# zhoubin-me/supertonic

Measured on AMD Instinct MI355X. Metric: audio-sec/sec (RTF^-1), 66M model, batch=128 per GPU, higher is better.
Workload: dtype bf16

## Files before the change

### include/stn.h

```cpp
#ifndef STN_H
#define STN_H
#include <stddef.h>
#include <stdint.h>

#include "stn_arch.h"

#ifdef __cplusplus
extern "C" {
#endif

#define STN_OK 0
#define STN_ERR_INVALID (-1)
#define STN_ERR_DEVICE (-2)
#define STN_ERR_STATE (-3)
#define STN_ERR_UNSUPPORTED (-4)
#define STN_ERR_IO (-5)

#define STN_DTYPE_F32 0
#define STN_DTYPE_BF16 1
#define STN_DTYPE_F16 2

typedef struct stn_handle stn_handle;

typedef struct stn_config {
// ... 133 lines not shown
int stn_set_loudness(stn_handle* h, int on, float target_lufs, float ceiling_dbfs);
int stn_get_loudness(const stn_handle* h, int* on, float* target_lufs, float* ceiling_dbfs);
int stn_batch_loudness(stn_handle* h, float* lufs, float* peak, float* gain);
int stn_op_loudness(stn_handle* h, int hz, int rows, int W, const float* x, const int64_t* n_or_null, float* lufs, float* peak);
int stn_kweighting_filter(int hz, double* shelf_b3, double* shelf_a3, double* hp_b3, double* hp_a3);
int stn_op_loudness_ex(stn_handle* h, int hz, int rows, int W, const float* x, const int64_t* n_or_null, int on, float target_lufs,
                       float ceiling_dbfs, int x_misalign, float* st_end, float* st_start, float* pk, float* pa, float* pb, float* lufs,
                       float* peak, float* gain, char* form, size_t form_cap);
int stn_loudness_table(int hz, float* coef10, float* mpow, size_t cap, int* hop);

int stn_batch_loudness_range(stn_handle* h, float* m_max, float* s_max, float* lra, int32_t* n_st);
int stn_batch_join_loudness_range(stn_handle* h, const stn_join* j, float* m_max, float* s_max, float* lra, int32_t* n_st);
int stn_op_loudness_range(stn_handle* h, int hz, int rows, int W, const float* x, const int64_t* n_or_null, float* m_max, float* s_max,
                          float* lra, int32_t* n_st);
int stn_loudness_range_rule(int hop, int64_t nseg, const double* seg, double* m_max, double* s_max, double* lra, int32_t* n_st);

int stn_set_silence_trim(stn_handle* h, int on, float top_db, float keep_ms, float fade_ms);
int stn_get_silence_trim(const stn_handle* h, int* on, float* top_db, float* keep_ms, float* fade_ms);
int stn_batch_silence_edges(stn_handle* h, int64_t* start, int64_t* end);
int stn_op_silence_edges(stn_handle* h, int hz, int rows, int W, const float* x, const int64_t* n_or_null, float top_db, float keep_ms,
                         int64_t* start, int64_t* end);
int stn_op_silence_trim(stn_handle* h, int hz, int rows, int W, const float* x, const int64_t* n_or_null, float top_db, float keep_ms,
                        float fade_ms, const float* gain_or_null, int enc, void* y, int64_t* start, int64_t* end);
int stn_silence_fade_window(int hz, float fade_ms, float* w, int64_t cap, int64_t* n);
int stn_dbg_batch_set_wav(stn_handle* h, const float* wav);
int64_t stn_dbg_span_uploads(const stn_handle* h);

int stn_set_pause_limit(stn_handle* h, int on, float max_pause_ms);
int stn_get_pause_limit(const stn_handle* h, int* on, float* max_pause_ms);
int stn_batch_pauses(stn_handle* h, int64_t* len, int32_t* n_cuts, int64_t* cuts_or_null, int cap_pairs);
int stn_op_pause_trim(stn_handle* h, int hz, int rows, int W, const float* x, const int64_t* n_or_null, float top_db, float keep_ms,
                      float fade_ms, float max_pause_ms, const float* gain_or_null, int enc, void* y, int64_t* start, int64_t* end,
                      int64_t* len, int32_t* n_cuts, int64_t* cuts_or_null, int cap_pairs);
int stn_pause_plan(int hz, int64_t n, const double* level, int64_t K, float top_db, float keep_ms, float max_pause_ms, int64_t* start,
                   int64_t* end, int64_t* cuts, int cap_pairs, int32_t* n_cuts);
const char* stn_pause_plan_error(void);
int stn_op_silence_edges_ex(stn_handle* h, int hz, int rows, int W, const float* x, const int64_t* n_or_null, float top_db, float keep_ms,
                            float fade_ms, float max_pause_ms, int x_misalign, float* pa, float* pb, double* lev, int64_t* start,
                            int64_t* end, int64_t* len, int32_t* n_cuts, int64_t* cuts_or_null, int cap_pairs, char* form, size_t form_cap);

int stn_set_limiter(stn_handle* h, int on, float lookahead_ms);
int stn_get_limiter(const stn_handle* h, int* on, float* lookahead_ms);
int stn_batch_limiter(stn_handle* h, float* reduction_db, int64_t* limited);
int stn_op_limiter(stn_handle* h, int hz, int rows, int W, const float* x, const int64_t* n_or_null, const float* gain_or_null,
                   float ceiling_dbfs, float lookahead_ms, float* y, float* s_or_null, float* reduction_db, int64_t* limited);
int stn_limiter_window(int hz, float lookahead_ms, float* w, int64_t cap, int64_t* n);

#define STN_PEAK_SAMPLE 0
#define STN_PEAK_TRUE 1
int stn_set_peak_mode(stn_handle* h, int mode);
int stn_get_peak_mode(const stn_handle* h);
int stn_true_peak_filter(float* taps_or_null, size_t cap, int* phases, int* taps_per_phase);
int stn_batch_true_peak(stn_handle* h, float* tp_in, float* tp_out, float* trim);
int stn_op_true_peak(stn_handle* h, int hz, int rows, int W, const float* x, const int64_t* n_or_null, const float* gain_or_null,
                     int x_misalign, float* tp, float* env_or_null, float* pk_or_null, char* form, size_t form_cap);
int stn_op_limiter_ex(stn_handle* h, int hz, int rows, int W, const float* x, const int64_t* n_or_null, const float* gain_or_null,
                      float ceiling_dbfs, float lookahead_ms, float* y, float* s_or_null, float* reduction_db, int64_t* limited,
                      int peak_mode, float* env_or_null, float* trim_or_null);

#define STN_FILT_HIGHPASS 0
#define STN_FILT_LOWPASS 1
#define STN_FILT_NOTCH 2
#define STN_FILT_PEAK 3
#define STN_FILT_LOWSHELF 4
#define STN_FILT_HIGHSHELF 5
#define STN_MAX_FILTERS 8
typedef struct stn_filter { int type; float freq_hz; float q; float gain_db; } stn_filter;
int stn_set_filters(stn_handle* h, int n, const stn_filter* f);
int stn_get_filters(const stn_handle* h, int* n, stn_filter* out);
int stn_op_filter(stn_handle* h, int hz, int rows, int W, const float* x, int n, const stn_filter* f, float* y);
int stn_op_filter_ex(stn_handle* h, int hz, int rows, int W, const float* x, int n, const stn_filter* f, int x_misalign, float* y,
                     float* st_end, float* st_start, int* guard_ok, char* form, size_t form_cap);
int stn_filter_coefs(const stn_filter* f, int rate_hz, double c[5], float c32[5]);
const char* stn_filter_error(int n, const stn_filter* f, int rate_hz);
int stn_filter_response(int n, const stn_filter* f, int rate_hz, int n_freq, const double* freq_hz, double* mag_db);
int stn_dbg_filter_geometry(int* chunk, int* wg_span, int* scan_tile_chunks, int* biquads_per_section);

typedef struct stn_compressor { float threshold_db, ratio, knee_db, attack_ms, release_ms, makeup_db; } stn_compressor;
int stn_set_compressor(stn_handle* h, int on, const stn_compressor* c);
int stn_get_compressor(const stn_handle* h, int* on, stn_compressor* out);
int stn_batch_compressor(stn_handle* h, float* max_reduction_db);
int stn_op_compressor(stn_handle* h, int hz, int rows, int W, const float* x, const stn_compressor* c, float* y);
int stn_op_compressor_ex(stn_handle* h, int hz, int rows, int W, const float* x, const stn_compressor* c, int x_misalign, int in_place,
                         float* y, float* gr_db, float* s1_end, float* s1_start, float* s2_end, float* s2_start, int* guard_ok, char* form,
                         size_t form_cap);
int stn_compressor_coefs(const stn_compressor* c, int rate_hz, double k[2], float k32[2]);
int stn_compressor_curve(const stn_compressor* c, int n, const double* in_db, double* out_db);
const char* stn_compressor_error(const stn_compressor* c, int rate_hz);

#define STN_DEESS_SPLIT 0
#define STN_DEESS_WIDE 1
typedef struct stn_deesser { float freq_hz, threshold_db, ratio, knee_db, attack_ms, release_ms, range_db; int mode; } stn_deesser;
int stn_set_deesser(stn_handle* h, int on, const stn_deesser* c);
int stn_get_deesser(const stn_handle* h, int* on, stn_deesser* out);
int stn_batch_deesser(stn_handle* h, float* max_reduction_db);
int stn_op_deesser(stn_handle* h, int hz, int rows, int W, const float* x, const stn_deesser* c, float* y);
int stn_op_deesser_ex(stn_handle* h, int hz, int rows, int W, const float* x, const stn_deesser* c, int x_misalign, int in_place, float* y,
                      float* band, float* gr_db, float* st_end, float* st_start, float* s1_end, float* s1_start, float* s2_end,
                      float* s2_start, int* guard_ok, char* form, size_t form_cap);
int stn_deesser_band(const stn_deesser* c, int rate_hz, double c10[10], float c32[10]);
int stn_deesser_coefs(const stn_deesser* c, int rate_hz, double k[2], float k32[2]);
const char* stn_deesser_error(const stn_deesser* c, int rate_hz);

typedef struct stn_expander { float threshold_db, ratio, knee_db, range_db, attack_ms, hold_ms, release_ms; } stn_expander;
int stn_set_expander(stn_handle* h, int on, const stn_expander* c);
int stn_get_expander(const stn_handle* h, int* on, stn_expander* out);
int stn_batch_expander(stn_handle* h, float* min_attenuation_db, int64_t* closed_samples);
int stn_op_expander(stn_handle* h, int hz, int rows, int W, const float* x, const stn_expander* c, float* y);
int stn_op_expander_ex(stn_handle* h, int hz, int rows, int W, const float* x, const stn_expander* c, int x_misalign, int in_place, float* y,
                       float* open_db, float* s1_end, float* s1_start, float* s2_end, float* s2_start, int* guard_ok, char* form,
                       size_t form_cap);
int stn_expander_coefs(const stn_expander* c, int rate_hz, double k[3], float k32[3], int64_t* hold_samples);
int stn_expander_curve(const stn_expander* c, int n, const double* in_db, double* out_db);
const char* stn_expander_error(const stn_expander* c, int rate_hz);

int stn_profile_enable(stn_handle* h, int on);
int stn_profile_reset(stn_handle* h);
int stn_profile_filter(stn_handle* h, const char* family_or_null);
int stn_profile_sample(stn_handle* h, int every);
int stn_launch_log_enable(stn_handle* h, int on);
int64_t stn_launch_log(stn_handle* h, char* out, size_t cap);
int stn_profile_count(stn_handle* h);
int stn_profile_get(stn_handle* h, int idx, char* name, size_t name_cap, double* total_ms, int64_t* launches,
                    double* flops, double* bytes);

int stn_dbg_xattn_hs_enable(stn_handle* h, int on);
int64_t stn_dbg_xattn_hs_stamps(stn_handle* h, unsigned long long* out, size_t cap);
int stn_dbg_fold_run_frames(const int32_t* latent_lengths, int B, int n_cu);

int stn_op_gemm(stn_handle* h, int dtype, int M, int N, int K, const float* A , const float* W ,
                const float* bias_or_null, int act , float* out );
int stn_op_gemm_ex(stn_handle* h, int dtype, int M, int N, int K, const float* A , const float* W , int mode, int act,
                   int out_dtype, int ldo, const float* bias_or_null, const float* gamma_or_null, const int32_t* len_or_null, int L,
                   const int32_t* row_b_or_null, const float* rowvec_or_null, int nseq, int nt, int tr, float* out, int64_t out_elems,
                   char* form, size_t form_cap);
int stn_dbg_gemm_form(int dtype, int M, int N, int K, int mode, int out_dtype, int ldo, int masked, int tr, char* out, size_t cap);
int stn_dbg_ffn_form(int dtype, int stage, int C, int I, int64_t M, int64_t gate_rows, int packed, int k, int max_dil, int mask,
                     int64_t min_rows, int64_t split_min_rows, int nt_hints, char* out, size_t cap);
int stn_op_gemm_bench(stn_handle* h, int dtype, int M, int N, int K, int mode, int iters, double* avg_ms);
int stn_op_gemm_phases(stn_handle* h, int dtype, int M, int N, int K, int mode, double* out6);
int stn_op_dwconv_ln(stn_handle* h, int dtype, int B, int L, int C, int k, int dil, const float* x,
                     const float* w , const float* bias, const float* ln_g, const float* ln_b, float* y);
int stn_op_dwconv_ln_ragged(stn_handle* h, int dtype, int B, int L, int C, int k, int dil, const float* x,
                            const float* w , const float* bias, const float* ln_g, const float* ln_b,
                            const int32_t* seqlen , float* y);
int stn_op_gemm_rows(stn_handle* h, int dtype, int M, int N, int K, const float* A, const float* W, const float* bias_or_null, int B,
                     const int32_t* rows, const int32_t* valid, int T, float* out, int64_t out_elems, char* form, size_t form_cap);
int stn_op_dwconv_ln_ex(stn_handle* h, int dtype, int B, int L, int C, int k, int dil, const float* x, int64_t x_rows,
                        const float* w_or_null , const float* bias_or_null, const float* ln_g, const float* ln_b,
                        const int32_t* seqlen_or_null, int packed, int ln_only, float* y, int64_t y_rows, char* form, size_t form_cap);
int stn_op_dwconv_ln_tail(stn_handle* h, int dtype, int B, int L, int C, int k, int dil, const float* x, int64_t x_rows,
                          const float* w , const float* bias, const float* ln_g, const float* ln_b, const int32_t* seqlen,
                          const float* tail , int T, int rf, float* y, int64_t y_rows, char* form, size_t form_cap);
int64_t stn_dbg_len_tables(int B, const int32_t* llen, int ve_rows, int with_pairs, int vo_form, int ccf, int T, int rf, int32_t* layout,
                           int32_t* out, int64_t out_n);
int stn_dbg_dwconv_ln_form(int dtype, int B, int L, int C, int k, int packed, char* out, size_t cap);
int stn_op_fold_ln(stn_handle* h, int dtype, int M, int C, int S, const float* part, const float* b2, const float* gamma,
                   const float* rowvec_or_null, const int32_t* row_b_or_null, int nseq, const float* ln_g, const float* ln_b, float* x,
                   float* y);
int stn_op_layout(stn_handle* h, int which, int dtype, const int32_t* p, int n_p, const float* a, int64_t a_n, const float* b, int64_t b_n,
                  const float* c, int64_t c_n, const int64_t* ids, int64_t ids_n, const int32_t* len, int packed, float* out, int64_t out_n,
                  float* out2, int64_t out2_n, int32_t* iout, int64_t iout_n);
int stn_op_attention(stn_handle* h, int dtype, int B, int Lq, int Lk, int H, int dh, const float* q, const float* k,
                     const float* v, const int32_t* qlen_or_null, const int32_t* klen_or_null, int rope_mode, float* o);
int stn_op_attention_ex(stn_handle* h, int dtype, int B, int Lq, int Lk, int H, int dh, const float* q, int64_t q_elems, int ldq,
                        int q_col, float* kv, int64_t kv_elems, int ldk, int k_col, int v_col, float* o, int64_t o_elems, int ldo,
                        const int32_t* qlen_or_null, const int32_t* klen_or_null, const int32_t* q_off_or_null,
                        const int32_t* k_off_or_null, int rope_mode, int k_rotated, int rot_groups, int rot_stride, int rot_col,
                        char* form, size_t form_cap);
int stn_op_xattn_hs(stn_handle* h, int dtype, int M, const float* xn, const float* Wq, const float* bq_or_null, const float* Wo,
                    const float* kv, int64_t kv_elems, int ldk, int k_col, int B, int L, int Lk, const int32_t* qlen,
                    const int32_t* klen_or_null, const int32_t* k_off_or_null, int rope_mode, int pairs_mode, int64_t part_stride,
                    float* part, int64_t part_elems, int32_t* pairs_out_or_null, char* form, size_t form_cap);
int stn_dbg_attn_form(int kind, int dtype, int B, int Lq, int Lk, int H, int dh, int ldq, int ldk, int misaligned, char* out, size_t cap);
int stn_op_ffn(stn_handle* h, int M, int C, int I, const float* xn , const float* W1, const float* b1, const float* W2,
               const float* b2_or_null, const float* gamma_or_null, const float* rowvec_or_null ,
               const int32_t* row_b_or_null , int nseq, float* x, int fused);
int stn_op_ffn_ex(stn_handle* h, int dtype, int M, int C, int I, const float* xn, int ldx, int64_t xn_elems, const float* W1, const float* b1,
                  const float* W2, const float* b2_or_null, const float* gamma_or_null, const int32_t* len_or_null, int L,
                  const int32_t* row_b_or_null, const float* rowvec_or_null, int rv_ld, int nseq, int mode, int split, float* x, int ldo,
                  int64_t x_elems, float* part_or_null, int64_t part_stride, int64_t part_elems, char* form, size_t form_cap);
int stn_op_ffn_bench(stn_handle* h, int M, int C, int I, int fused, int iters, double* out5);
int stn_op_fold_dwconv_ln(stn_handle* h, int B, int C, int k, int dil, int S, const int32_t* seqlen, const float* x, const float* part,
                          const float* b2_or_null, const float* gamma_or_null, const float* rowvec_or_null , const float* w ,
                          const float* bias, const float* ln_g, const float* ln_b, float* x_out, float* y);
int stn_op_fold_dwconv_ln_ex(stn_handle* h, int dtype, int B, int L, int C, int k, int dil, int S, int run_frames, const int32_t* seqlen,
                             const float* x_in, int64_t x_rows, const float* part, int64_t part_stride, int64_t part_elems,
                             const float* b2_or_null, const float* gamma_or_null, const float* rowvec_or_null, int rv_ld,
                             const float* w , const float* bias, const float* ln_g, const float* ln_b, float* x_out, int64_t x_out_rows,
                             float* y, int64_t y_rows, char* form, size_t form_cap);
int stn_dbg_fold_dwconv_ln_form(int dtype, int B, int L, int C, int k, int dil, int S, int has_rowvec, int run_frames, char* out, size_t cap);
int stn_op_block_bench(stn_handle* h, int B, int L, int C, int I, int k, int dil, int mode, int iters, double* out6);
int stn_op_randn(stn_handle* h, uint64_t seed, int B, int D, int L, const int64_t* utt_ids_or_null,
                 const int32_t* len_or_null, float* out);

const char* stn_version(void);
int stn_hip_versions(int* built, int* runtime);
int stn_device_count(void);
int stn_device_sync(int device);
int stn_ffn_fused_forms(int dtype, int C, int I);

#ifdef __cplusplus
}
#endif
#endif
```

### supertonic_amd/binding.py

```python
import ctypes
import os

import numpy as np

from .arch import StnArch

_HERE = os.path.dirname(os.path.abspath(__file__))
LIB_PATH = os.environ.get("STN_LIB") or os.path.join(_HERE, "libstn.so")
_LIB = None

F32, BF16, F16 = 0, 1, 2
_DTYPES = {"f32": F32, "fp32": F32, "float32": F32, "bf16": BF16, "f16": F16, "fp16": F16, "float16": F16, "half": F16,
           F32: F32, BF16: BF16, F16: F16}
ACT_NONE, ACT_GELU, ACT_SILU, ACT_GELU_TANH = 0, 1, 2, 3
EPI_STORE, EPI_RESID, EPI_STORE_T = 0, 1, 2
FFN_VOCODER, FFN_ESTIMATOR, FFN_TEXT = 1, 2, 4
LAYOUT_ROW_MAP, LAYOUT_NCL_TO_ROWS, LAYOUT_EULER_NCL, LAYOUT_UNPACK_ROWS, LAYOUT_EMBED, LAYOUT_MASKED_MEAN, LAYOUT_IM2COL, LAYOUT_VOCODER_IN = range(8)
LAYOUT_FILL_ROWS, LAYOUT_HS_PAIRS, LAYOUT_TRIM_LEN = 8, 9, 10
ENC_F32, ENC_PCM16, ENC_PCM24, ENC_MULAW, ENC_ALAW = 0, 1, 2, 3, 4
ENCODINGS = {"f32": ENC_F32, "pcm16": ENC_PCM16, "pcm24": ENC_PCM24, "mulaw": ENC_MULAW, "alaw": ENC_ALAW}
ENCODING_NAMES = {v: k for k, v in ENCODINGS.items()}
ENCODING_BYTES = {ENC_F32: 4, ENC_PCM16: 2, ENC_PCM24: 3, ENC_MULAW: 1, ENC_ALAW: 1}
ZERO_CODEWORD = {ENC_F32: 0, ENC_PCM16: 0, ENC_PCM24: 0, ENC_MULAW: 0xFF, ENC_ALAW: 0xD5}

# ... 367 lines not shown

class StnError(RuntimeError):
    def __init__(self, code, msg):
        super().__init__(f"stn error {code}: {msg}")
        self.code = code


class StnConfig(ctypes.Structure):
    _fields_ = [("device", ctypes.c_int32), ("dtype", ctypes.c_int32)]


_f32p = np.ctypeslib.ndpointer(np.float32, flags="C_CONTIGUOUS")
_i64p = np.ctypeslib.ndpointer(np.int64, flags="C_CONTIGUOUS")
_i32p = np.ctypeslib.ndpointer(np.int32, flags="C_CONTIGUOUS")


def runtime_info(L=None):
    import sys
    L = L or load()
    b, r = ctypes.c_int(), ctypes.c_int()
    L.stn_hip_versions(ctypes.byref(b), ctypes.byref(r))
    return {"hip_built": b.value, "hip_runtime": r.value, "torch_preloaded": "torch" in sys.modules, "lib": LIB_PATH}


def device_count():
    n = load().stn_device_count()
    if n < 0:
        raise StnError(n, "hipGetDeviceCount failed")
    return n


def device_sync(device=0):
    rc = load().stn_device_sync(int(device))
    if rc < 0:
        raise StnError(rc, "hipDeviceSynchronize failed")


def _check_runtime(L):
    import warnings
    info = runtime_info(L)
    b, r = info["hip_built"], info["hip_runtime"]
    if r > 0 and (b // 100000) != (r // 100000):
        warnings.warn(f"libstn.so was built against HIP {b // 10000000}.{b // 100000 % 100} but runs on HIP runtime {r // 10000000}.{r // 100000 % 100}"
                      + (" (PyTorch's bundled runtime was loaded first; set STN_NO_TORCH_PRELOAD=1 in processes that do not need torch)" if info["torch_preloaded"] else ""),
                      RuntimeWarning, stacklevel=3)


def load():
    global _LIB
    if _LIB is not None:
        return _LIB
    if not os.path.exists(LIB_PATH):
        raise FileNotFoundError(f"{LIB_PATH} not found: build it with `make` (hipcc --offload-arch=gfx950); "
                                "the engine has no fallback path")
    import sys
    if "torch" not in sys.modules and os.environ.get("STN_NO_TORCH_PRELOAD") != "1" and os.environ.get("STN_HOST_ONLY") != "1":
        import importlib.util
        if importlib.util.find_spec("torch") is not None:
            import torch
    L = ctypes.CDLL(LIB_PATH)
    if os.environ.get("STN_HOST_ONLY") == "1":
        _LIB = L
        return L
    vp, ci, cu64, cf = ctypes.c_void_p, ctypes.c_int, ctypes.c_uint64, ctypes.c_float
    L.stn_hip_versions.argtypes = [ctypes.POINTER(ci), ctypes.POINTER(ci)]
    L.stn_ffn_fused_forms.argtypes = [ci, ci, ci]
    L.stn_device_count.argtypes = []
    L.stn_device_sync.argtypes = [ci]
    _check_runtime(L)
    L.stn_version.restype = ctypes.c_char_p
    L.stn_create.argtypes = [ctypes.POINTER(StnConfig), ctypes.POINTER(vp)]
    L.stn_destroy.argtypes = [vp]
    L.stn_last_error.restype = ctypes.c_char_p
    L.stn_last_error.argtypes = [vp]
    L.stn_load_dir.argtypes = [vp, ctypes.c_char_p]
    L.stn_tensor_names.argtypes = [vp, ctypes.POINTER(StnArch), ctypes.c_char_p, ctypes.c_size_t]
    L.stn_load_synthetic.argtypes = [vp, ctypes.POINTER(StnArch), cu64]
    L.stn_get_arch.argtypes = [vp, ctypes.POINTER(StnArch)]
    L.stn_param_count.restype = ctypes.c_int64
    L.stn_param_count.argtypes = [vp]
    L.stn_duration.argtypes = [vp, ci, ci, _i64p, _f32p, _f32p, _f32p]
    L.stn_text_enc.argtypes = [vp, ci, ci, _i64p, _f32p, _f32p, _f32p]
    L.stn_vector_est.argtypes = [vp, ci, ci, ci] + [_f32p] * 8
    L.stn_vocoder.argtypes = [vp, ci, ci, _f32p, _f32p]
    L.stn_batch_upload.argtypes = [vp, ci, ci, _i64p, _f32p, _f32p, _f32p, vp, vp]
    L.stn_batch_set_noise.argtypes = [vp, _f32p, ci]
    L.stn_batch_run.argtypes = [vp, ci, cf, cu64]
    L.stn_set_graph_mode.argtypes = [vp, ci]
    L.stn_set_vocoder_mode.argtypes = [vp, ci]
    L.stn_set_row_layout.argtypes = [vp, ci]
    L.stn_set_fused_xattn.argtypes = [vp, ci]
    L.stn_set_shape_buckets.argtypes = [vp, ci]
    L.stn_set_duration_read.argtypes = [vp, ci]
    L.stn_set_gelu_form.argtypes = [vp, ci]
    L.stn_get_gelu_form.argtypes = [vp]
    L.stn_batch_ve_rows.argtypes = [vp]
    L.stn_batch_ve_rows.restype = ctypes.c_int64
    L.stn_batch_vo_rows.argtypes = [vp]
    L.stn_batch_vo_rows.restype = ctypes.c_int64
    L.stn_graph_replays.restype = ctypes.c_int64
    L.stn_graph_replays.argtypes = [vp]
    L.stn_graphs_cached.restype = ctypes.c_int64
    L.stn_graphs_cached.argtypes = [vp]
    L.stn_batch_dims.argtypes = [vp, ctypes.POINTER(ci), ctypes.POINTER(ci), ctypes.POINTER(ctypes.c_int64)]
    L.stn_batch_fetch.argtypes = [vp, vp, ctypes.c_size_t, vp]
    L.stn_batch_fetch_latent.argtypes = [vp, _f32p]
    L.stn_batch_fetch_pcm16.argtypes = [vp, vp, ctypes.c_size_t, vp]
    L.stn_batch_fetch_pcm16_begin.argtypes = [vp, ci]
    L.stn_batch_fetch_slot_dims.argtypes = [vp, ci, ctypes.POINTER(ci), ctypes.POINTER(ctypes.c_int64)]
    L.stn_batch_fetch_pcm16_end.argtypes = [vp, ci, ctypes.POINTER(vp), ctypes.POINTER(ctypes.c_size_t), vp]
    L.stn_host_alloc_pinned.restype = vp
    L.stn_host_alloc_pinned.argtypes = [ctypes.c_size_t]
    L.stn_host_free_pinned.argtypes = [vp]
    L.stn_batch_wav_device_ptr.argtypes = [vp, ctypes.POINTER(vp)]
    L.stn_sync.argtypes = [vp]
    L.stn_set_stream.argtypes = [vp, vp]
    L.stn_batch_copy_wav_device.argtypes = [vp, vp, ctypes.c_int64]
    L.stn_batch_copy_pcm16_device.argtypes = [vp, vp, ctypes.c_int64]
    L.stn_profile_filter.argtypes = [vp, ctypes.c_char_p]
    L.stn_profile_sample.argtypes = [vp, ci]
    L.stn_launch_log_enable.argtypes = [vp, ci]
    L.stn_dbg_xattn_hs_enable.argtypes = [vp, ci]
    L.stn_dbg_xattn_hs_stamps.argtypes = [vp, vp, ctypes.c_size_t]
    L.stn_dbg_xattn_hs_stamps.restype = ctypes.c_int64
    L.stn_dbg_fold_run_frames.argtypes = [vp, ctypes.c_int, ctypes.c_int]
    L.stn_dbg_fold_run_frames.restype = ctypes.c_int
    L.stn_dbg_gemm_form.argtypes = [ci, ci, ci, ci, ci, ci, ci, ci, ci, ctypes.c_char_p, ctypes.c_size_t]
    L.stn_dbg_gemm_form.restype = ctypes.c_int
    L.stn_dbg_attn_form.argtypes = [ci, ci, ci, ci, ci, ci, ci, ci, ci, ci, ctypes.c_char_p, ctypes.c_size_t]
    L.stn_dbg_attn_form.restype = ctypes.c_int
    L.stn_dbg_ffn_form.argtypes = [ci, ci, ci, ci, ctypes.c_int64, ctypes.c_int64, ci, ci, ci, ci, ctypes.c_int64, ctypes.c_int64, ci,
                                   ctypes.c_char_p, ctypes.c_size_t]
    L.stn_dbg_ffn_form.restype = ctypes.c_int
    L.stn_launch_log.argtypes = [vp, ctypes.c_char_p, ctypes.c_size_t]
    L.stn_launch_log.restype = ctypes.c_int64
    L.stn_profile_enable.argtypes = [vp, ci]
    L.stn_profile_reset.argtypes = [vp]
    L.stn_profile_count.argtypes = [vp]
    L.stn_profile_get.argtypes = [vp, ci, ctypes.c_char_p, ctypes.c_size_t, ctypes.POINTER(ctypes.c_double),
                                  ctypes.POINTER(ctypes.c_int64), ctypes.POINTER(ctypes.c_double),
                                  ctypes.POINTER(ctypes.c_double)]
    L.stn_op_gemm.argtypes = [vp, ci, ci, ci, ci, _f32p, _f32p, vp, ci, _f32p]
    L.stn_op_gemm_ex.argtypes = [vp, ci, ci, ci, ci, _f32p, _f32p, ci, ci, ci, ci, vp, vp, vp, ci, vp, vp, ci, ci, ci, _f32p,
                                 ctypes.c_int64, ctypes.c_char_p, ctypes.c_size_t]
    L.stn_op_gemm_bench.argtypes = [vp, ci, ci, ci, ci, ci, ci, ctypes.POINTER(ctypes.c_double)]
    L.stn_op_gemm_phases.argtypes = [vp, ci, ci, ci, ci, ci, ctypes.POINTER(ctypes.c_double)]
    L.stn_op_dwconv_ln.argtypes = [vp, ci, ci, ci, ci, ci, ci, _f32p, _f32p, _f32p, _f32p, _f32p, _f32p]
    L.stn_op_dwconv_ln_ragged.argtypes = [vp, ci, ci, ci, ci, ci, ci, _f32p, _f32p, _f32p, _f32p, _f32p, _i32p, _f32p]
    L.stn_op_attention.argtypes = [vp, ci, ci, ci, ci, ci, ci, _f32p, _f32p, _f32p, vp, vp, ci, _f32p]
    L.stn_op_gemm_rows.argtypes = [vp, ci, ci, ci, ci, _f32p, _f32p, vp, ci, _i32p, _i32p, ci, _f32p, ctypes.c_int64, ctypes.c_char_p, ctypes.c_size_t]
    L.stn_op_dwconv_ln_ex.argtypes = [vp, ci, ci, ci, ci, ci, ci, _f32p, ctypes.c_int64, vp, vp, _f32p, _f32p, vp, ci, ci, _f32p, ctypes.c_int64,
                                      ctypes.c_char_p, ctypes.c_size_t]
    L.stn_op_dwconv_ln_tail.argtypes = [vp, ci, ci, ci, ci, ci, ci, _f32p, ctypes.c_int64, _f32p, _f32p, _f32p, _f32p, _i32p, _f32p, ci, ci, _f32p,
                                        ctypes.c_int64, ctypes.c_char_p, ctypes.c_size_t]
    L.stn_dbg_resample_form.argtypes = [ci, ci, ctypes.c_int64, ctypes.c_char_p, ctypes.c_size_t]
    L.stn_dbg_resample_form.restype = ctypes.c_int
    L.stn_dbg_dwconv_ln_form.argtypes = [ci, ci, ci, ci, ci, ci, ctypes.c_char_p, ctypes.c_size_t]
    L.stn_dbg_dwconv_ln_form.restype = ctypes.c_int
    L.stn_dbg_len_tables.argtypes = [ci, _i32p, ci, ci, ci, ci, ci, ci, _i32p, ctypes.c_void_p, ctypes.c_int64]
    L.stn_dbg_len_tables.restype = ctypes.c_int64
    L.stn_op_fold_ln.argtypes = [vp, ci, ci, ci, ci, _f32p, _f32p, _f32p, vp, vp, ci, _f32p, _f32p, _f32p, _f32p]
    L.stn_op_layout.argtypes = [vp, ci, ci, _i32p, ci, vp, ctypes.c_int64, vp, ctypes.c_int64, vp, ctypes.c_int64, vp, ctypes.c_int64, vp, ci,
                                vp, ctypes.c_int64, vp, ctypes.c_int64, vp, ctypes.c_int64]
    L.stn_op_attention_ex.argtypes = [vp, ci, ci, ci, ci, ci, ci, _f32p, ctypes.c_int64, ci, ci, _f32p, ctypes.c_int64, ci, ci, ci,
                                      _f32p, ctypes.c_int64, ci, vp, vp, vp, vp, ci, ci, ci, ci, ci, ctypes.c_char_p, ctypes.c_size_t]
    L.stn_op_xattn_hs.argtypes = [vp, ci, ci, _f32p, _f32p, vp, _f32p, _f32p, ctypes.c_int64, ci, ci, ci, ci, ci, _i32p, vp, vp, ci, ci,
                                  ctypes.c_int64, _f32p, ctypes.c_int64, vp, ctypes.c_char_p, ctypes.c_size_t]
    L.stn_op_randn.argtypes = [vp, cu64, ci, ci, ci, vp, vp, _f32p]
    L.stn_op_ffn.argtypes = [vp, ci, ci, ci, _f32p, _f32p, _f32p, _f32p, vp, vp, vp, vp, ci, _f32p, ci]
    L.stn_op_ffn_ex.argtypes = [vp, ci, ci, ci, ci, _f32p, ci, ctypes.c_int64, _f32p, _f32p, _f32p, vp, vp, vp, ci, vp, vp, ci, ci, ci, ci, _f32p, ci,
                                ctypes.c_int64, vp, ctypes.c_int64, ctypes.c_int64, ctypes.c_char_p, ctypes.c_size_t]
    L.stn_op_ffn_bench.argtypes = [vp, ci, ci, ci, ci, ci, ctypes.POINTER(ctypes.c_double)]
    L.stn_set_fused_ffn.argtypes = [vp, ci]
    L.stn_set_fused_ffn_min_rows.argtypes = [vp, ctypes.c_int64, ctypes.c_int64]
    L.stn_op_fold_dwconv_ln.argtypes = [vp, ci, ci, ci, ci, ci, _i32p, _f32p, _f32p, vp, vp, vp, _f32p, _f32p, _f32p, _f32p, _f32p, _f32p]
    L.stn_op_fold_dwconv_ln_ex.argtypes = [vp, ci, ci, ci, ci, ci, ci, ci, ci, _i32p, _f32p, ctypes.c_int64, _f32p, ctypes.c_int64, ctypes.c_int64, vp, vp,
                                           vp, ci, _f32p, _f32p, _f32p, _f32p, _f32p, ctypes.c_int64, _f32p, ctypes.c_int64, ctypes.c_char_p,
                                           ctypes.c_size_t]
    L.stn_dbg_fold_dwconv_ln_form.argtypes = [ci, ci, ci, ci, ci, ci, ci, ci, ci, ctypes.c_char_p, ctypes.c_size_t]
    L.stn_dbg_fold_dwconv_ln_form.restype = ctypes.c_int
    L.stn_op_block_bench.argtypes = [vp, ci, ci, ci, ci, ci, ci, ci, ci, ctypes.POINTER(ctypes.c_double)]
    L.stn_group_create.argtypes = [ci, vp, ci, ctypes.POINTER(vp)]
    L.stn_group_destroy.argtypes = [vp]
    L.stn_group_last_error.restype = ctypes.c_char_p
    L.stn_group_last_error.argtypes = [vp]
    L.stn_group_size.argtypes = [vp]
    L.stn_group_uses_rccl.argtypes = [vp]
    L.stn_group_handle.restype = vp
    L.stn_group_handle.argtypes = [vp, ci]
    L.stn_group_load_synthetic.argtypes = [vp, ctypes.POINTER(StnArch), cu64]
    L.stn_group_load_dir.argtypes = [vp, ctypes.c_char_p]
    L.stn_group_deal.argtypes = [ci, _i32p, ci, _i32p, _i32p]
    L.stn_group_synthesize.argtypes = [vp, ci, ci, _i64p, _f32p, _f32p, _f32p, ci, cf, vp, cu64, ctypes.POINTER(ctypes.c_int64)]
    L.stn_group_fetch_pcm16.argtypes = [vp, vp, ctypes.c_size_t, vp]
    L.stn_set_output_rate.argtypes = [vp, ci]
    L.stn_get_output_rate.argtypes = [vp]
    L.stn_resample_filter.argtypes = [ci, ci, vp, ctypes.c_size_t, ctypes.POINTER(ci), ctypes.POINTER(ci)]
    L.stn_resample_error.argtypes = [ci, ci]
    L.stn_resample_error.restype = ctypes.c_char_p
    L.stn_op_resample.argtypes = [vp, ci, ci, ci, ci, _f32p, vp, vp]
    L.stn_group_set_output_rate.argtypes = [vp, ci]
    _f64p = np.ctypeslib.ndpointer(np.float64, flags="C_CONTIGUOUS")
    L.stn_set_loudness.argtypes = [vp, ci, cf, cf]
    L.stn_get_loudness.argtypes = [vp, ctypes.POINTER(ci), ctypes.POINTER(cf), ctypes.POINTER(cf)]
    L.stn_batch_loudness.argtypes = [vp, vp, vp, vp]
    L.stn_op_loudness.argtypes = [vp, ci, ci, ci, _f32p, vp, vp, vp]
    L.stn_kweighting_filter.argtypes = [ci, _f64p, _f64p, _f64p, _f64p]
    L.stn_op_loudness_ex.argtypes = [vp, ci, ci, ci, _f32p, vp, ci, cf, cf, ci, vp, vp, vp, vp, vp, vp, vp, vp, ctypes.c_char_p, ctypes.c_size_t]
    L.stn_loudness_table.argtypes = [ci, vp, vp, ctypes.c_size_t, ctypes.POINTER(ci)]
    L.stn_group_set_loudness.argtypes = [vp, ci, cf, cf]
    L.stn_batch_loudness_range.argtypes = [vp, vp, vp, vp, vp]
    L.stn_op_loudness_range.argtypes = [vp, ci, ci, ci, _f32p, vp, vp, vp, vp, vp]
    L.stn_set_silence_trim.argtypes = [vp, ci, cf, cf, cf]
    L.stn_get_silence_trim.argtypes = [vp, ctypes.POINTER(ci), ctypes.POINTER(cf), ctypes.POINTER(cf), ctypes.POINTER(cf)]
    L.stn_batch_silence_edges.argtypes = [vp, vp, vp]
    L.stn_op_silence_edges.argtypes = [vp, ci, ci, ci, _f32p, vp, cf, cf, vp, vp]
    L.stn_op_silence_trim.argtypes = [vp, ci, ci, ci, _f32p, vp, cf, cf, cf, vp, ci, vp, vp, vp]
    L.stn_silence_fade_window.argtypes = [ci, cf, vp, ctypes.c_int64, ctypes.POINTER(ctypes.c_int64)]
    L.stn_set_pause_limit.argtypes = [vp, ci, cf]
    L.stn_get_pause_limit.argtypes = [vp, ctypes.POINTER(ci), ctypes.POINTER(cf)]
    L.stn_batch_pauses.argtypes = [vp, vp, vp, vp, ci]
    L.stn_op_pause_trim.argtypes = [vp, ci, ci, ci, _f32p, vp, cf, cf, cf, cf, vp, ci, vp, vp, vp, vp, vp, vp, ci]
    L.stn_op_silence_edges_ex.argtypes = [vp, ci, ci, ci, _f32p, vp, cf, cf, cf, cf, ci, vp, vp, vp, vp, vp, vp, vp, vp, ci, ctypes.c_char_p,
                                          ctypes.c_size_t]
    L.stn_group_set_pause_limit.argtypes = [vp, ci, cf]
    L.stn_set_limiter.argtypes = [vp, ci, cf]
    L.stn_get_limiter.argtypes = [vp, ctypes.POINTER(ci), ctypes.POINTER(cf)]
    L.stn_batch_limiter.argtypes = [vp, vp, vp]
    L.stn_op_limiter.argtypes = [vp, ci, ci, ci, _f32p, vp, vp, cf, cf, vp, vp, vp, vp]
    L.stn_limiter_window.argtypes = [ci, cf, vp, ctypes.c_int64, ctypes.POINTER(ctypes.c_int64)]
    L.stn_group_set_limiter.argtypes = [vp, ci, cf]
    L.stn_set_peak_mode.argtypes = [vp, ci]
    L.stn_get_peak_mode.argtypes = [vp]
    L.stn_group_set_peak_mode.argtypes = [vp, ci]
    L.stn_true_peak_filter.argtypes = [vp, ctypes.c_size_t, ctypes.POINTER(ci), ctypes.POINTER(ci)]
    L.stn_batch_true_peak.argtypes = [vp, vp, vp, vp]
    L.stn_op_true_peak.argtypes = [vp, ci, ci, ci, _f32p, vp, vp, ci, vp, vp, vp, ctypes.c_char_p, ctypes.c_size_t]
    L.stn_op_limiter_ex.argtypes = [vp, ci, ci, ci, _f32p, vp, vp, cf, cf, vp, vp, vp, vp, ci, vp, vp]
    fp = ctypes.POINTER(StnFilter)
    L.stn_set_filters.argtypes = [vp, ci, fp]
    L.stn_get_filters.argtypes = [vp, ctypes.POINTER(ci), fp]
    L.stn_group_set_filters.argtypes = [vp, ci, fp]
    L.stn_op_filter.argtypes = [vp, ci, ci, ci, _f32p, ci, fp, _f32p]
    L.stn_op_filter_ex.argtypes = [vp, ci, ci, ci, _f32p, ci, fp, ci, _f32p, vp, vp, ctypes.POINTER(ci), ctypes.c_char_p, ctypes.c_size_t]
    L.stn_filter_error.argtypes = [ci, fp, ci]
    L.stn_filter_error.restype = ctypes.c_char_p
    L.stn_filter_coefs.argtypes = [fp, ci, _f64p, _f32p]
    L.stn_filter_response.argtypes = [ci, fp, ci, ci, _f64p, _f64p]
    L.stn_dbg_filter_geometry.argtypes = [ctypes.POINTER(ci)] * 4
    cpp = ctypes.POINTER(StnCompressor)
    L.stn_set_compressor.argtypes = [vp, ci, cpp]
    L.stn_get_compressor.argtypes = [vp, ctypes.POINTER(ci), cpp]
    L.stn_group_set_compressor.argtypes = [vp, ci, cpp]
    L.stn_batch_compressor.argtypes = [vp, vp]
    L.stn_op_compressor.argtypes = [vp, ci, ci, ci, _f32p, cpp, _f32p]
    L.stn_op_compressor_ex.argtypes = [vp, ci, ci, ci, _f32p, cpp, ci, ci, _f32p, vp, vp, vp, vp, vp, ctypes.POINTER(ci), ctypes.c_char_p, ctypes.c_size_t]
    L.stn_compressor_error.argtypes = [cpp, ci]
    L.stn_compressor_error.restype = ctypes.c_char_p
    L.stn_compressor_coefs.argtypes = [cpp, ci, _f64p, _f32p]
    L.stn_compressor_curve.argtypes = [cpp, ci, _f64p, _f64p]
    xpp = ctypes.POINTER(StnExpander)
    L.stn_set_expander.argtypes = [vp, ci, xpp]
    L.stn_get_expander.argtypes = [vp, ctypes.POINTER(ci), xpp]
    L.stn_group_set_expander.argtypes = [vp, ci, xpp]
    L.stn_batch_expander.argtypes = [vp, vp, vp]
    L.stn_op_expander.argtypes = [vp, ci, ci, ci, _f32p, xpp, _f32p]
    L.stn_op_expander_ex.argtypes = [vp, ci, ci, ci, _f32p, xpp, ci, ci, _f32p, vp, vp, vp, vp, vp, ctypes.POINTER(ci), ctypes.c_char_p, ctypes.c_size_t]
    L.stn_expander_error.argtypes = [xpp, ci]
    L.stn_expander_error.restype = ctypes.c_char_p
    L.stn_expander_coefs.argtypes = [xpp, ci, _f64p, _f32p, ctypes.POINTER(ctypes.c_int64)]
    L.stn_expander_curve.argtypes = [xpp, ci, _f64p, _f64p]
    dsp = ctypes.POINTER(StnDeesser)
    L.stn_set_deesser.argtypes = [vp, ci, dsp]
    L.stn_get_deesser.argtypes = [vp, ctypes.POINTER(ci), dsp]
    L.stn_group_set_deesser.argtypes = [vp, ci, dsp]
    L.stn_batch_deesser.argtypes = [vp, vp]
    L.stn_op_deesser.argtypes = [vp, ci, ci, ci, _f32p, dsp, _f32p]
    L.stn_op_deesser_ex.argtypes = [vp, ci, ci, ci, _f32p, dsp, ci, ci, _f32p] + [vp] * 8 + [ctypes.POINTER(ci), ctypes.c_char_p, ctypes.c_size_t]
    L.stn_deesser_error.argtypes = [dsp, ci]
    L.stn_deesser_error.restype = ctypes.c_char_p
    L.stn_deesser_band.argtypes = [dsp, ci, _f64p, _f32p]
    L.stn_deesser_coefs.argtypes = [dsp, ci, _f64p, _f32p]
    L.stn_dbg_batch_set_wav.argtypes = [vp, _f32p]
    L.stn_dbg_span_uploads.argtypes = [vp]
    L.stn_dbg_span_uploads.restype = ctypes.c_int64
    L.stn_encoding_bytes.argtypes = [ci]
    L.stn_batch_fetch_encoded.argtypes = [vp, ci, vp, ctypes.c_size_t, vp]
    L.stn_batch_copy_encoded_device.argtypes = [vp, ci, vp, ctypes.c_int64]
    L.stn_batch_fetch_encoded_begin.argtypes = [vp, ci, ci]
    L.stn_batch_fetch_encoded_end.argtypes = [vp, ci, ctypes.POINTER(vp), ctypes.POINTER(ctypes.c_size_t), vp]
    L.stn_op_encode.argtypes = [vp, ci, ci, ci, _f32p, vp]
    L.stn_set_dither.argtypes = [vp, ci, cu64]
    L.stn_get_dither.argtypes = [vp, ctypes.POINTER(cu64)]
    L.stn_group_set_dither.argtypes = [vp, ci, cu64]
    L.stn_op_encode_ex.argtypes = [vp, ci, ci, ci, _f32p, ci, vp, vp, ci, cu64, ctypes.c_int64, vp]
    L.stn_set_pitch.argtypes = [vp, cf]
    L.stn_get_pitch.argtypes = [vp, ctypes.POINTER(cf), ctypes.POINTER(ci), ctypes.POINTER(ci)]
    L.stn_group_set_pitch.argtypes = [vp, cf]
    L.stn_op_time_stretch.argtypes = [vp, ci, ci, ci, _f32p, vp, ci, ci, vp, vp, vp]
    L.stn_op_pitch.argtypes = [vp, ci, ci, ci, _f32p, vp, cf, vp]
    L.stn_set_pitch_mode.argtypes = [vp, ci]
    L.stn_get_pitch_mode.argtypes = [vp]
    L.stn_group_set_pitch_mode.argtypes = [vp, ci]
    L.stn_op_formant.argtypes = [vp, ci, ci, ci, _f32p, _f32p, vp, vp]
    L.stn_op_formant_ex.argtypes = [vp, ci, ci, ci, _f32p, _f32p, vp, vp, vp, vp, vp, vp, vp, ctypes.POINTER(ci)]
    L.stn_op_pitch_ex.argtypes = [vp, ci, ci, ci, _f32p, vp, cf, ci, vp]
# ... 1384 lines not shown
        return res, form.value.decode()

    def op_gemm_bench(self, M, N, K, mode=0, iters=20, dtype=None):
        ms = ctypes.c_double()
        self._ck(self._lib.stn_op_gemm_bench(self._h, self.dtype if dtype is None else _DTYPES[dtype], M, N, K, mode,
                                             iters, ctypes.byref(ms)))
        return ms.value

    def op_ffn(self, xn, W1, b1, W2, b2, gamma, x, rowvec=None, row_b=None, fused=True):
        M, C = xn.shape
        I = W1.shape[0]
        out = np.array(x, dtype=np.float32, order="C", copy=True)
        _, b2p = _opt(b2, np.float32)
        b2a = _opt(b2, np.float32)[0]
        ga, gp = _opt(gamma, np.float32)
        rva, rvp = _opt(rowvec, np.float32)
        rba, rbp = _opt(row_b, np.int32)
        b2p = b2a.ctypes.data if b2a is not None else None
        self._ck(self._lib.stn_op_ffn(self._h, M, C, I, _c(xn, np.float32), _c(W1, np.float32), _c(b1, np.float32), _c(W2, np.float32),
                                      b2p, gp, rvp, rbp, 0 if rva is None else rva.shape[0], out, int(fused)))
        return out

    def op_ffn_ex(self, xn, W1, b1, W2, x, mode=1, b2=None, gamma=None, len=None, L=None, row_b=None, rowvec=None, split=0, part=None,
                  part_stride=0, M=None, dtype=None):
        xn = _c(xn, np.float32)
        I, C = W1.shape
        M = xn.shape[0] if M is None else int(M)
        x_r = np.array(x, dtype=np.float32, order="C", copy=True)
        p_r = None if part is None else np.array(part, dtype=np.float32, order="C", copy=True)
        nseq = 0
        for v in (len, rowvec):
            if v is not None:
                nseq = max(nseq, np.asarray(v).shape[0])
        if row_b is not None and rowvec is None:
            nseq = max(nseq, int(np.max(row_b)) + 1)
        _b, bp = _opt(b2, np.float32)
        _g, gp = _opt(gamma, np.float32)
        _l, lp = _opt(len, np.int32)
        _r, rp = _opt(row_b, np.int32)
        _v, vp_ = _opt(rowvec, np.float32)
        form = ctypes.create_string_buffer(32)
        self._ck(self._lib.stn_op_ffn_ex(self._h, self.dtype if dtype is None else _DTYPES[dtype], M, C, I, xn.reshape(-1), xn.shape[1], xn.size,
                                         _c(W1, np.float32), _c(b1, np.float32), _c(W2, np.float32), bp, gp, lp, int(M if L is None else L), rp, vp_,
                                         C if _v is None else _v.shape[1], nseq, int(mode), int(split), x_r.reshape(-1), x_r.shape[1], x_r.size,
                                         None if p_r is None else p_r.ctypes.data, int(part_stride), 0 if p_r is None else p_r.size, form,
                                         ctypes.sizeof(form)))
        return x_r, p_r, form.value.decode()

    def op_ffn_bench(self, M, C, I, fused=True, iters=20):
        out = (ctypes.c_double * 5)()
        self._ck(self._lib.stn_op_ffn_bench(self._h, M, C, I, int(fused), iters, out))
        return dict(ms=out[0], first_stage=out[1], tile_loop=out[2], epilogue=out[3], workgroups=int(out[4]))

    def op_fold_dwconv_ln(self, seqlen, x, part, b2, gamma, rowvec, w, bias, g, b, k, dil):
        seqlen = np.ascontiguousarray(seqlen, np.int32)
        S, M, C = part.shape
        xo = np.empty((M, C), np.float32)
        y = np.empty((M, C), np.float32)
        b2a, _ = _opt(b2, np.float32)
        ga, _ = _opt(gamma, np.float32)
        rva, _ = _opt(rowvec, np.float32)
        p = lambda a: None if a is None else a.ctypes.data
        self._ck(self._lib.stn_op_fold_dwconv_ln(self._h, len(seqlen), C, k, dil, S, seqlen, _c(x, np.float32), _c(part, np.float32), p(b2a), p(ga), p(rva),
                                                 _c(w, np.float32), _c(bias, np.float32), _c(g, np.float32), _c(b, np.float32), xo, y))
        return xo, y

    def op_fold_dwconv_ln_ex(self, seqlen, L, x_in, part, part_stride, S, b2, gamma, rowvec, w, bias, g, b, dil, x_out, y, run_frames=0, dtype=None):
        seqlen = _c(seqlen, np.int32)
        x_in = _c(x_in, np.float32)
        part = _c(part, np.float32).reshape(-1)
        xo = np.array(x_out, dtype=np.float32, order="C", copy=True)
        yo = np.array(y, dtype=np.float32, order="C", copy=True)
        C = x_in.shape[1]
        w = _c(w, np.float32)
        _b2, b2p = _opt(b2, np.float32)
        _g, gp = _opt(gamma, np.float32)
        _v, vp_ = _opt(rowvec, np.float32)
        form = ctypes.create_string_buffer(96)
        self._ck(self._lib.stn_op_fold_dwconv_ln_ex(self._h, self.dtype if dtype is None else _DTYPES[dtype], len(seqlen), int(L), C, w.shape[1], int(dil),
                                                    int(S), int(run_frames), seqlen, x_in.reshape(-1), x_in.shape[0], part, int(part_stride), part.size,
                                                    b2p, gp, vp_, C if _v is None else _v.shape[1], w, _c(bias, np.float32), _c(g, np.float32),
                                                    _c(b, np.float32), xo.reshape(-1), xo.shape[0], yo.reshape(-1), yo.shape[0], form, ctypes.sizeof(form)))
        return xo, yo, form.value.decode()

    def op_block_bench(self, B, L, C, I, k, dil, mode, iters=20):
        out = (ctypes.c_double * 6)()
        self._ck(self._lib.stn_op_block_bench(self._h, B, L, C, I, k, dil, mode, iters, out))
        return dict(ms=out[0], conv_ms=out[1], fold_phase1=out[2], fold_barrier=out[3], fold_phase2=out[4], fold_span=out[5])

    def set_fused_ffn_min_rows(self, k4_rows=-1, split_rows=-1):
        self._ck(self._lib.stn_set_fused_ffn_min_rows(self._h, int(k4_rows), int(split_rows)))

    def op_gemm_phases(self, M, N, K, mode=0, dtype=None):
        out = (ctypes.c_double * 6)()
        self._ck(self._lib.stn_op_gemm_phases(self._h, self.dtype if dtype is None else _DTYPES[dtype], M, N, K, mode, out))
        return dict(first_stage=out[0], k_loop=out[1], epilogue=out[2], grid_span=out[3], entry_spread=out[4], workgroups=int(out[5]))

    def op_dwconv_ln(self, x, w, bias, g, b, dil, dtype=None, seqlen=None):
        B, L, C = x.shape
        k = w.shape[1]
        y = np.empty((B, L, C), np.float32)
        if seqlen is not None:
            self._ck(self._lib.stn_op_dwconv_ln_ragged(self._h, self.dtype if dtype is None else _DTYPES[dtype], B, L, C, k,
                                                       dil, _c(x, np.float32), _c(w, np.float32), _c(bias, np.float32),
                                                       _c(g, np.float32), _c(b, np.float32), _c(seqlen, np.int32), y))
            return y
        self._ck(self._lib.stn_op_dwconv_ln(self._h, self.dtype if dtype is None else _DTYPES[dtype], B, L, C, k, dil,
                                            _c(x, np.float32), _c(w, np.float32), _c(bias, np.float32),
                                            _c(g, np.float32), _c(b, np.float32), y))
        return y

    def op_gemm_rows(self, A, W, out, rows, valid, T, bias=None, dtype=None):
        A = _c(A, np.float32)
        W = _c(W, np.float32)
        rows = _c(rows, np.int32)
        valid = _c(valid, np.int32)
        o_r = np.array(out, dtype=np.float32, order="C", copy=True)
        _b, bp = _opt(bias, np.float32)
        form = ctypes.create_string_buffer(96)
        self._ck(self._lib.stn_op_gemm_rows(self._h, self.dtype if dtype is None else _DTYPES[dtype], A.shape[0], W.shape[0], A.shape[1],
                                            A.reshape(-1), W.reshape(-1), bp, len(rows), rows, valid, int(T), o_r.reshape(-1), o_r.size, form,
                                            ctypes.sizeof(form)))
        return o_r, form.value.decode()

    def op_dwconv_ln_ex(self, x, w, bias, g, b, dil, out, B, L, seqlen=None, packed=False, ln_only=False, dtype=None):
        x = _c(x, np.float32)
        o_r = np.array(out, dtype=np.float32, order="C", copy=True)
        C = x.shape[1]
        _w, wp = _opt(w, np.float32)
        _b, bp = _opt(bias, np.float32)
        _l, lp = _opt(seqlen, np.int32)
        form = ctypes.create_string_buffer(32)
        self._ck(self._lib.stn_op_dwconv_ln_ex(self._h, self.dtype if dtype is None else _DTYPES[dtype], int(B), int(L), C,
                                               1 if _w is None else _w.shape[1], int(dil), x.reshape(-1), x.shape[0], wp, bp, _c(g, np.float32),
                                               _c(b, np.float32), lp, int(bool(packed)), int(bool(ln_only)), o_r.reshape(-1), o_r.shape[0], form,
                                               ctypes.sizeof(form)))
        return o_r, form.value.decode()

    def op_dwconv_ln_tail(self, x, w, bias, g, b, dil, out, L, seqlen, tail, T, dtype=None):
        x = _c(x, np.float32)
        tail = _c(tail, np.float32)
        o_r = np.array(out, dtype=np.float32, order="C", copy=True)
        C = x.shape[1]
        w = _c(w, np.float32)
        seqlen = _c(seqlen, np.int32)
        assert tail.ndim == 2 and tail.shape[1] == C and tail.shape[0] >= 1
        form = ctypes.create_string_buffer(32)
        self._ck(self._lib.stn_op_dwconv_ln_tail(self._h, self.dtype if dtype is None else _DTYPES[dtype], len(seqlen), int(L), C, w.shape[1],
                                                 int(dil), x.reshape(-1), x.shape[0], w, _c(bias, np.float32), _c(g, np.float32),
                                                 _c(b, np.float32), seqlen, tail.reshape(-1), int(T), tail.shape[0] - 1, o_r.reshape(-1),
                                                 o_r.shape[0], form, ctypes.sizeof(form)))
        return o_r, form.value.decode()

    def op_fold_ln(self, x, part, b2, gamma, g, b, rowvec=None, row_b=None, dtype=None):
        x_r = np.array(x, dtype=np.float32, order="C", copy=True)
        M, C = x_r.shape
        part = _c(part, np.float32)
        y = np.empty((M, C), np.float32)
        _v, vp_ = _opt(rowvec, np.float32)
        _r, rp = _opt(row_b, np.int32)
        self._ck(self._lib.stn_op_fold_ln(self._h, self.dtype if dtype is None else _DTYPES[dtype], M, C, part.shape[0], part.reshape(-1),
                                          _c(b2, np.float32), _c(gamma, np.float32), vp_, rp, 0 if _v is None else _v.shape[0],
                                          _c(g, np.float32), _c(b, np.float32), x_r, y))
        return x_r, y

    def op_layout(self, which, p, a=None, b=None, c=None, ids=None, length=None, packed=False, out=None, out2=None, iout=None, dtype="f32"):
        def f32(v):
            return (None, None, 0) if v is None else (lambda arr: (arr, arr.ctypes.data, arr.size))(_c(v, np.float32))
        pa = _c(p, np.int32)
        _a, ap, an = f32(a)
        _b, bp, bn = f32(b)
        _cc, cp, cn = f32(c)
        _i, ip = _opt(ids, np.int64)
        _l, lp = _opt(length, np.int32)
        o1 = None if out is None else np.array(out, dtype=np.float32, order="C", copy=True)
        o2 = None if out2 is None else np.array(out2, dtype=np.float32, order="C", copy=True)
        io = None if iout is None else np.array(iout, dtype=np.int32, order="C", copy=True)
        ptr = lambda v: (None, 0) if v is None else (v.ctypes.data, v.size)
        self._ck(self._lib.stn_op_layout(self._h, int(which), _DTYPES[dtype], pa, len(pa), ap, an, bp, bn, cp, cn, ip, 0 if _i is None else _i.size,
                                         lp, int(bool(packed)), *ptr(o1), *ptr(o2), *ptr(io)))
        return o1, o2, io

    def op_attention(self, q, k, v, H, qlen=None, klen=None, rope_mode=-1, dtype=None):
        B, Lq, C = q.shape
        Lk = k.shape[1]
        o = np.empty((B, Lq, C), np.float32)
        _q, qp = _opt(qlen, np.int32)
        _k, kp = _opt(klen, np.int32)
        self._ck(self._lib.stn_op_attention(self._h, self.dtype if dtype is None else _DTYPES[dtype], B, Lq, Lk, H,
                                            C // H, _c(q, np.float32), _c(k, np.float32), _c(v, np.float32), qp, kp,
                                            rope_mode, o))
        return o

    def op_attention_ex(self, q, kv, out, B, Lq, Lk, H, dh, q_col=0, k_col=0, v_col=None, qlen=None, klen=None, q_off=None, k_off=None,
                        rope_mode=-1, k_rotated=False, rot_groups=1, rot_stride=0, rot_col=None, dtype=None):
        q = _c(q, np.float32)
        kv_r = np.array(kv, dtype=np.float32, order="C", copy=True)
        o_r = np.array(out, dtype=np.float32, order="C", copy=True)
        _a, qlp = _opt(qlen, np.int32)
        _b, klp = _opt(klen, np.int32)
        _d, qop = _opt(q_off, np.int32)
        _e, kop = _opt(k_off, np.int32)
        form = ctypes.create_string_buffer(64)
        self._ck(self._lib.stn_op_attention_ex(self._h, self.dtype if dtype is None else _DTYPES[dtype], int(B), int(Lq), int(Lk), int(H), int(dh),
                                               q.reshape(-1), q.size, q.shape[1], int(q_col), kv_r.reshape(-1), kv_r.size, kv_r.shape[1],
                                               int(k_col), int(k_col + H * dh if v_col is None else v_col), o_r.reshape(-1), o_r.size,
                                               o_r.shape[1], qlp, klp, qop, kop, int(rope_mode), int(bool(k_rotated)), int(rot_groups),
                                               int(rot_stride), int(k_col if rot_col is None else rot_col), form, ctypes.sizeof(form)))
        return o_r, kv_r, form.value.decode()

    def op_xattn_hs(self, xn, Wq, bq, Wo, kv, part, part_stride, B, L, Lk, qlen, k_col=0, klen=None, k_off=None, rope_mode=-1,
                    pairs=False, dtype=None):
        xn = _c(xn, np.float32)
        kv = _c(kv, np.float32)
        part_r = np.array(part, dtype=np.float32, order="C", copy=True).reshape(-1)
        _b, bqp = _opt(bq, np.float32)
        _k, klp = _opt(klen, np.int32)
        _o, kop = _opt(k_off, np.int32)
        pr = np.full(2 * ((B + 1) // 2), -7, np.int32) if pairs else None
        form = ctypes.create_string_buffer(64)
        self._ck(self._lib.stn_op_xattn_hs(self._h, self.dtype if dtype is None else _DTYPES[dtype], xn.shape[0], xn.reshape(-1),
                                           _c(Wq, np.float32), bqp, _c(Wo, np.float32), kv.reshape(-1), kv.size, kv.shape[1], int(k_col),
                                           int(B), int(L), int(Lk), _c(qlen, np.int32), klp, kop, int(rope_mode), int(bool(pairs)),
                                           int(part_stride), part_r, part_r.size, None if pr is None else pr.ctypes.data, form,
                                           ctypes.sizeof(form)))
        return part_r, pr, form.value.decode()

    def op_randn(self, seed, B, D, L, utt_ids=None, length=None):
        out = np.empty((B, D, L), np.float32)
        _u, up = _opt(utt_ids, np.int64)
        _l, lp = _opt(length, np.int32)
        self._ck(self._lib.stn_op_randn(self._h, seed, B, D, L, up, lp, out))
        return out


def pinned_array(shape, dtype):
    L = load()
    dt = np.dtype(dtype)
    n = int(np.prod(shape)) * dt.itemsize
    p = L.stn_host_alloc_pinned(n)
    if not p:
        raise MemoryError("stn_host_alloc_pinned failed")
    buf = (ctypes.c_char * n).from_address(p)
    arr = np.frombuffer(buf, dtype=dt).reshape(shape)
    import weakref
    weakref.finalize(buf, L.stn_host_free_pinned, ctypes.c_void_p(p))
    return arr
```

### supertonic_amd/csrc/api.cpp

```cpp
#include "../../include/stn.h"

#include <algorithm>
#include <complex>
#include <cstdio>
#include <cstring>
#include <fstream>
#include <string>

#include "engine.hpp"
#include "host/json_min.hpp"
#include "host/graph_bind.hpp"
#include "host/onnx_reader.hpp"

#include <map>
#include <sstream>

struct stn_handle {
    stn::Engine* eng = nullptr;
    std::string err;
    std::vector<std::pair<std::string, stn::KernelStat>> prof;
};

static thread_local std::string g_create_err;

// ... 799 lines not shown
}
int stn_batch_loudness_range(stn_handle* h, float* m_max, float* s_max, float* lra, int32_t* n_st) {
    STN_TRY(h, { need_batch(h); h->eng->batch_loudness_range(m_max, s_max, lra, n_st); })
}
int stn_batch_join_loudness_range(stn_handle* h, const stn_join* j, float* m_max, float* s_max, float* lra, int32_t* n_st) {
    STN_TRY(h, { need(j != nullptr, "join is null"); need_batch(h); h->eng->batch_join_loudness_range(j, m_max, s_max, lra, n_st); })
}
int stn_op_loudness_range(stn_handle* h, int hz, int rows, int W, const float* x, const int64_t* n, float* m_max, float* s_max, float* lra,
                          int32_t* n_st) {
    STN_TRY(h, { need(rows > 0 && rows <= 65535 && W > 0 && x, "stn_op_loudness_range: bad argument (1 <= rows <= 65535, W >= 1, x)");
                 h->eng->op_loudness_range(hz, rows, W, x, n, m_max, s_max, lra, n_st); })
}
int stn_op_join(stn_handle* h, int hz, int rows, int W, const float* x, const int64_t* n, const stn_join* j, int enc, int loudness_on, float target_lufs,
                float ceiling_dbfs, void* y, float* prog_lufs, float* prog_peak, float* prog_gain) {
    STN_TRY(h, { need(rows > 0 && rows <= 65535 && W > 0 && x && n && j && y, "stn_op_join: bad argument (1 <= rows <= 65535, W >= 1, x, n, j and y)");
                 h->eng->op_join(hz, rows, W, x, n, j, enc, loudness_on != 0, target_lufs, ceiling_dbfs, y, prog_lufs, prog_peak, prog_gain); })
}
int stn_batch_copy_wav_device(stn_handle* h, void* dst, int64_t stride) {
    STN_TRY(h, { need(dst != nullptr, "dst is null"); h->eng->batch_copy_wav_device(static_cast<float*>(dst), stride); })
}

int stn_profile_enable(stn_handle* h, int on) { STN_TRY(h, { h->eng->profile_enable(on != 0); }) }
int stn_launch_log_enable(stn_handle* h, int on) { STN_TRY(h, { h->eng->launch_log_enable(on != 0); }) }
int64_t stn_launch_log(stn_handle* h, char* out, size_t cap) {
    if (!h) return STN_ERR_INVALID;
    try {
        const std::string s = h->eng->launch_log();
        if (out && cap > s.size()) std::memcpy(out, s.c_str(), s.size() + 1);
        return (int64_t)s.size();
    } catch (const std::exception& e) { h->err = e.what(); return STN_ERR_STATE; }
}
int stn_dbg_xattn_hs_enable(stn_handle* h, int on) { STN_TRY(h, { h->eng->hs_stamps_enable(on != 0); }) }
int stn_dbg_fold_run_frames(const int32_t* latent_lengths, int B, int n_cu) {
    if (!latent_lengths || B < 1 || n_cu < 1) return STN_ERR_INVALID;
    return stn::fold_run_frames(latent_lengths, B, n_cu);
}
int64_t stn_dbg_xattn_hs_stamps(stn_handle* h, unsigned long long* out, size_t cap) {
    if (!h) return STN_ERR_INVALID;
    try { return h->eng->hs_stamps_fetch(out, cap); } catch (const std::exception& e) { h->err = e.what(); return STN_ERR_STATE; }
}
int stn_profile_sample(stn_handle* h, int every) { STN_TRY(h, { h->eng->profile_sample(every); }) }
int stn_profile_filter(stn_handle* h, const char* fam) { STN_TRY(h, { h->eng->profile_filter(fam ? fam : ""); }) }
int stn_profile_reset(stn_handle* h) { STN_TRY(h, { h->eng->profile_reset(); h->prof.clear(); }) }
int stn_profile_count(stn_handle* h) {
    if (!h) return STN_ERR_INVALID;
    try { h->prof = h->eng->profile_collect(); } catch (const std::exception& e) { h->err = e.what(); return STN_ERR_DEVICE; }
    return (int)h->prof.size();
}
int stn_profile_get(stn_handle* h, int idx, char* name, size_t cap, double* ms, int64_t* launches, double* flops, double* bytes) {
    if (!h || idx < 0 || idx >= (int)h->prof.size()) return STN_ERR_INVALID;
    const auto& p = h->prof[idx];
    if (name && cap) { std::snprintf(name, cap, "%s", p.first.c_str()); }
    if (ms) *ms = p.second.ms;
    if (launches) *launches = p.second.launches;
    if (flops) *flops = p.second.flops;
    if (bytes) *bytes = p.second.bytes;
    return STN_OK;
}

int stn_op_gemm(stn_handle* h, int dtype, int M, int N, int K, const float* A, const float* W, const float* bias, int act, float* out) {
    STN_TRY(h, { need(M > 0 && N > 0 && K > 0 && A && W && out, "stn_op_gemm: bad argument");
                 need(K % (dtype != STN_DTYPE_F32 ? 8 : 4) == 0, "stn_op_gemm: K must be a multiple of 8 (bf16) / 4 (f32)");
                 h->eng->op_gemm(dtype, M, N, K, A, W, bias, act, out); })
}
int stn_op_gemm_ex(stn_handle* h, int dtype, int M, int N, int K, const float* A, const float* W, int mode, int act, int out_dtype, int ldo,
                   const float* bias, const float* gamma, const int32_t* len, int L, const int32_t* row_b, const float* rowvec, int nseq, int nt,
                   int tr, float* out, int64_t out_elems, char* form, size_t form_cap) {
    STN_TRY(h, { need(M > 0 && N > 0 && K > 0 && A && W && out && L >= 1, "stn_op_gemm_ex: bad argument");
                 need(dtype == STN_DTYPE_F32 || dtype == STN_DTYPE_BF16 || dtype == STN_DTYPE_F16, "stn_op_gemm_ex: unknown dtype");
                 need(K % (dtype != STN_DTYPE_F32 ? 8 : 4) == 0, "stn_op_gemm_ex: K must be a multiple of 8 (16-bit) / 4 (f32)");
                 need(mode == stn::EPI_STORE || mode == stn::EPI_RESID || mode == stn::EPI_STORE_T, "stn_op_gemm_ex: mode must be 0, 1 or 2");
                 need(act >= stn::ACT_NONE && act <= stn::ACT_GELU_TANH, "stn_op_gemm_ex: unknown activation");
                 need(out_dtype == STN_DTYPE_F32 || (mode == stn::EPI_STORE && out_dtype == dtype), "stn_op_gemm_ex: out_dtype must be f32 or the engine's dtype (store only)");
                 need(nt == 0 || nt == 1, "stn_op_gemm_ex: nt must be 0 or 1");
                 need(tr >= -1 && tr <= 1, "stn_op_gemm_ex: tr must be -1, 0 or 1");
                 need(!(len && row_b), "stn_op_gemm_ex: len and row_b exclude each other");
                 const int64_t seqs = ((int64_t)M + L - 1) / L;
                 if (mode == stn::EPI_STORE_T) {
                     need(!row_b && nseq >= seqs && out_elems >= seqs * N * L, "stn_op_gemm_ex: mode 2 needs nseq >= ceil(M/L), out_elems >= ceil(M/L)*N*L, no row_b");
                 } else {
                     need(ldo >= N && out_elems >= (int64_t)M * ldo, "stn_op_gemm_ex: needs ldo >= N and out_elems >= M*ldo");
                 }
                 if (len || (rowvec && !row_b)) need(nseq >= seqs, "stn_op_gemm_ex: len / rowvec by m / L need nseq >= ceil(M/L)");
                 if (rowvec || len || row_b) need(nseq > 0, "stn_op_gemm_ex: nseq must be > 0");
                 if (len) for (int b = 0; b < nseq; ++b) need(len[b] >= 0 && len[b] <= L, "stn_op_gemm_ex: len out of [0, L]");
                 if (row_b) for (int m = 0; m < M; ++m) need(row_b[m] >= 0 && row_b[m] < nseq, "stn_op_gemm_ex: row_b out of [0, nseq)");
                 const std::string f = h->eng->op_gemm_ex(dtype, M, N, K, A, W, mode, act, out_dtype, ldo, bias, gamma, len, L, row_b, rowvec,
                                                          nseq, nt, tr, out, out_elems);
                 if (form && form_cap) std::snprintf(form, form_cap, "%s", f.c_str()); })
}
int stn_dbg_gemm_form(int dtype, int M, int N, int K, int mode, int out_dtype, int ldo, int masked, int tr, char* out, size_t cap) {
    if (M < 1 || N < 1 || K < 1 || (dtype != STN_DTYPE_F32 && dtype != STN_DTYPE_BF16 && dtype != STN_DTYPE_F16) || tr < -1 || tr > 1)
        return STN_ERR_INVALID;
    static const int dummy_len[4] = {};
    stn::Epilogue e;
    e.mode = mode; e.out_dtype = out_dtype; e.ldo = ldo; e.len = masked ? dummy_len : nullptr; e.tr_force = tr;
    std::string f;
    try { f = stn::gemm_form(dtype, M, N, K, K, K, e, nullptr, nullptr).str(); } catch (const std::exception&) { return STN_ERR_INVALID; }
    if (out && cap > f.size()) std::memcpy(out, f.c_str(), f.size() + 1);
    return (int)f.size();
}
int stn_dbg_ffn_form(int dtype, int stage, int C, int I, int64_t M, int64_t gate_rows, int packed, int k, int max_dil, int mask,
                     int64_t min_rows, int64_t split_min_rows, int nt_hints, char* out, size_t cap) {
    if (C < 1 || I < 1 || M < 1 || k < 1 || max_dil < 1 || (stage != stn::FFN_VOCODER && stage != stn::FFN_ESTIMATOR && stage != stn::FFN_TEXT) ||
        (dtype != STN_DTYPE_F32 && dtype != STN_DTYPE_BF16 && dtype != STN_DTYPE_F16))
        return STN_ERR_INVALID;
    const std::string f = stn::ffn_form(dtype, stage, C, I, M, gate_rows, packed != 0, k, max_dil, mask, min_rows, split_min_rows, nt_hints != 0).str();
    if (out && cap > f.size()) std::memcpy(out, f.c_str(), f.size() + 1);
    return (int)f.size();
}
int stn_op_gemm_bench(stn_handle* h, int dtype, int M, int N, int K, int mode, int iters, double* avg_ms) {
    STN_TRY(h, { need(M > 0 && N > 0 && K > 0 && iters > 0 && avg_ms, "stn_op_gemm_bench: bad argument");
                 need(K % (dtype != STN_DTYPE_F32 ? 8 : 4) == 0, "K must be a multiple of 8 (bf16) / 4 (f32)");
                 *avg_ms = h->eng->op_gemm_bench(dtype, M, N, K, mode, iters); })
}
int stn_op_gemm_phases(stn_handle* h, int dtype, int M, int N, int K, int mode, double* out6) {
    STN_TRY(h, { need(M > 0 && N > 0 && K > 0 && out6, "stn_op_gemm_phases: bad argument");
                 need(K % (dtype != STN_DTYPE_F32 ? 8 : 4) == 0, "K must be a multiple of 8 (bf16) / 4 (f32)");
                 h->eng->op_gemm_phases(dtype, M, N, K, mode, out6); })
}
int stn_op_dwconv_ln(stn_handle* h, int dtype, int B, int L, int C, int k, int dil, const float* x, const float* w,
                     const float* bias, const float* g, const float* b, float* y) {
    STN_TRY(h, { need(B > 0 && L > 0 && C > 0 && C % 4 == 0 && C <= 1024 && k > 0 && (k & 1) && dil > 0 && x && w && bias && g && b && y,
                      "stn_op_dwconv_ln: bad argument");
                 h->eng->op_dwconv_ln(dtype, B, L, C, k, dil, x, w, bias, g, b, y); })
}
int stn_op_dwconv_ln_ragged(stn_handle* h, int dtype, int B, int L, int C, int k, int dil, const float* x, const float* w,
                            const float* bias, const float* g, const float* b, const int32_t* seqlen, float* y) {
    STN_TRY(h, { need(B > 0 && L > 0 && C > 0 && C % 4 == 0 && C <= 1024 && k > 0 && (k & 1) && dil > 0 && x && w && bias && g && b && y && seqlen,
                      "stn_op_dwconv_ln_ragged: bad argument");
                 for (int i = 0; i < B; ++i) need(seqlen[i] >= 0 && seqlen[i] <= L, "stn_op_dwconv_ln_ragged: seqlen out of [0, L]");
                 h->eng->op_dwconv_ln(dtype, B, L, C, k, dil, x, w, bias, g, b, y, seqlen); })
}
static void gemm_rows_checked(stn_handle* h, int dtype, int M, int N, int K, const float* A, const float* W, const float* bias, int B,
                              const int32_t* rows, const int32_t* valid, int T, float* out, int64_t out_elems, char* form, size_t form_cap) {
    need(M > 0 && N > 0 && K > 0 && A && W && out && rows && valid && B > 0 && B <= 1024 && T > 0, "stn_op_gemm_rows: bad argument");
    need(dtype == STN_DTYPE_F32 || dtype == STN_DTYPE_BF16 || dtype == STN_DTYPE_F16, "stn_op_gemm_rows: unknown dtype");
    need(K % (dtype != STN_DTYPE_F32 ? 8 : 4) == 0, "stn_op_gemm_rows: K must be a multiple of 8 (16-bit) / 4 (f32)");
    int64_t tot = 0;
    for (int b = 0; b < B; ++b) {
        need(rows[b] >= 0 && rows[b] <= T && valid[b] >= 0 && valid[b] <= rows[b], "stn_op_gemm_rows: needs 0 <= valid[b] <= rows[b] <= T");
        tot += rows[b];
    }
    need(tot <= M && out_elems >= (int64_t)B * T * N, "stn_op_gemm_rows: needs sum rows <= M and out_elems >= B*T*N");
    const std::string f = h->eng->op_gemm_rows(dtype, M, N, K, A, W, bias, B, rows, valid, T, out, out_elems);
    if (form && form_cap) std::snprintf(form, form_cap, "%s", f.c_str());
}
int stn_op_gemm_rows(stn_handle* h, int dtype, int M, int N, int K, const float* A, const float* W, const float* bias, int B, const int32_t* rows,
                     const int32_t* valid, int T, float* out, int64_t out_elems, char* form, size_t form_cap) {
    STN_TRY(h, gemm_rows_checked(h, dtype, M, N, K, A, W, bias, B, rows, valid, T, out, out_elems, form, form_cap))
}
static void dwconv_ln_ex_checked(stn_handle* h, int dtype, int B, int L, int C, int k, int dil, const float* x, int64_t x_rows, const float* w,
                                 const float* bias, const float* g, const float* b, const int32_t* seqlen, int packed, int ln_only, float* y,
                                 int64_t y_rows, char* form, size_t form_cap) {
    need(B > 0 && L > 0 && C > 0 && C % 4 == 0 && C <= 1024 && k > 0 && (k & 1) && dil > 0 && x && g && b && y && x_rows > 0 && y_rows > 0,
         "stn_op_dwconv_ln_ex: bad argument");
    need(dtype == STN_DTYPE_F32 || dtype == STN_DTYPE_BF16 || dtype == STN_DTYPE_F16, "stn_op_dwconv_ln_ex: unknown dtype");
    need(ln_only || (w && bias), "stn_op_dwconv_ln_ex: the conv needs w and bias");
    need(!(packed && ln_only), "stn_op_dwconv_ln_ex: ln_only takes no packed layout");
    need(!packed || (seqlen && B <= 1024), "stn_op_dwconv_ln_ex: packed rows need seqlen and B <= 1024");
    int64_t rows = (int64_t)B * L;
    if (seqlen && !ln_only) {
        int64_t tot = 0;
        for (int i = 0; i < B; ++i) { need(seqlen[i] >= 0 && seqlen[i] <= L, "stn_op_dwconv_ln_ex: seqlen out of [0, L]"); tot += seqlen[i]; }
        if (packed) rows = tot;
    }
    need(x_rows >= rows && y_rows >= rows, "stn_op_dwconv_ln_ex: x / y hold fewer rows than the launch addresses");
    const std::string f = h->eng->op_dwconv_ln_ex(dtype, B, L, C, k, dil, x, x_rows, w, bias, g, b, ln_only ? nullptr : seqlen, packed, ln_only, y, y_rows);
    if (form && form_cap) std::snprintf(form, form_cap, "%s", f.c_str());
}
int stn_op_dwconv_ln_ex(stn_handle* h, int dtype, int B, int L, int C, int k, int dil, const float* x, int64_t x_rows, const float* w,
                        const float* bias, const float* g, const float* b, const int32_t* seqlen, int packed, int ln_only, float* y,
                        int64_t y_rows, char* form, size_t form_cap) {
    STN_TRY(h, dwconv_ln_ex_checked(h, dtype, B, L, C, k, dil, x, x_rows, w, bias, g, b, seqlen, packed, ln_only, y, y_rows, form, form_cap))
}
static void dwconv_ln_tail_checked(stn_handle* h, int dtype, int B, int L, int C, int k, int dil, const float* x, int64_t x_rows, const float* w,
                                   const float* bias, const float* g, const float* b, const int32_t* seqlen, const float* tail, int T, int rf,
                                   float* y, int64_t y_rows, char* form, size_t form_cap) {
    need(B > 0 && B <= 1024 && L > 0 && C > 0 && C % 4 == 0 && C <= 512 && (k == 5 || k == 7) && dil > 0 && x && w && bias && g && b && y && seqlen &&
             x_rows > 0 && y_rows > 0,
         "stn_op_dwconv_ln_tail: bad argument");
    need(dtype == STN_DTYPE_F32 || dtype == STN_DTYPE_BF16 || dtype == STN_DTYPE_F16, "stn_op_dwconv_ln_tail: unknown dtype");
    need(tail && rf >= 0 && T >= L, "stn_op_dwconv_ln_tail: needs a tail table of rf + 1 >= 1 rows and T >= L");
    int64_t rows = 0;
    for (int i = 0; i < B; ++i) { need(seqlen[i] >= 0 && seqlen[i] <= L, "stn_op_dwconv_ln_tail: seqlen out of [0, L]"); rows += seqlen[i]; }
    need(x_rows >= rows && y_rows >= rows, "stn_op_dwconv_ln_tail: x / y hold fewer rows than the launch addresses");
    const std::string f = h->eng->op_dwconv_ln_ex(dtype, B, L, C, k, dil, x, x_rows, w, bias, g, b, seqlen, 1, 0, y, y_rows, tail, T, rf);
    if (form && form_cap) std::snprintf(form, form_cap, "%s", f.c_str());
}
int stn_op_dwconv_ln_tail(stn_handle* h, int dtype, int B, int L, int C, int k, int dil, const float* x, int64_t x_rows, const float* w,
                          const float* bias, const float* g, const float* b, const int32_t* seqlen, const float* tail, int T, int rf, float* y,
                          int64_t y_rows, char* form, size_t form_cap) {
    STN_TRY(h, dwconv_ln_tail_checked(h, dtype, B, L, C, k, dil, x, x_rows, w, bias, g, b, seqlen, tail, T, rf, y, y_rows, form, form_cap))
}
int64_t stn_dbg_len_tables(int B, const int32_t* llen, int ve_rows, int with_pairs, int vo_form, int ccf, int T, int rf, int32_t* layout,
                           int32_t* out, int64_t out_n) {
    if (B < 1 || B > 1024 || !llen || ve_rows < 0 || vo_form < stn::LEN_VO_NONE || vo_form > stn::LEN_VO_SCALED || ccf < 1 || T < 0 || rf < 0) return STN_ERR_INVALID;
    int64_t tot = 0;
    for (int b = 0; b < B; ++b) {
        if (llen[b] < 0 || llen[b] > (1 << 20)) return STN_ERR_INVALID;
        tot += llen[b];
    }
    if (ve_rows > 0 && tot > ve_rows) return STN_ERR_INVALID;
    if (with_pairs && ve_rows == 0) return STN_ERR_INVALID;
    const stn::LenTables t = stn::len_tables_layout(B, ve_rows, with_pairs != 0, vo_form);
    if (layout) {
        const int v[9] = {t.seed, t.llen, t.ve_off, t.ve_row_b, t.pairs, t.vo_n, t.vo_valid, t.vo_off, t.total};
        std::memcpy(layout, v, sizeof v);
    }
    if (out) {
        if (out_n < t.total) return STN_ERR_INVALID;
        stn::len_tables_build(t, llen, B, ve_rows, with_pairs != 0, vo_form, ccf, T, rf, out);
    }
    return t.total;
}
int stn_dbg_dwconv_ln_form(int dtype, int B, int L, int C, int k, int packed, char* out, size_t cap) {
    if (B < 1 || L < 1 || C < 1 || k < 1 || !(k & 1) || (dtype != STN_DTYPE_F32 && dtype != STN_DTYPE_BF16 && dtype != STN_DTYPE_F16)) return STN_ERR_INVALID;
    std::string f;
    try { f = stn::dwconv_ln_form(dtype, B, L, C, k, packed != 0).str(); } catch (const std::exception&) { return STN_ERR_INVALID; }
    if (out && cap > f.size()) std::memcpy(out, f.c_str(), f.size() + 1);
    return (int)f.size();
}
int stn_op_fold_ln(stn_handle* h, int dtype, int M, int C, int S, const float* part, const float* b2, const float* gamma, const float* rowvec,
                   const int32_t* row_b, int nseq, const float* g, const float* b, float* x, float* y) {
    STN_TRY(h, { need(M > 0 && C > 0 && C % 4 == 0 && C <= 1024 && (S == 4 || S == 8 || S == 12 || S == 24) && part && b2 && gamma && g && b && x && y,
                      "stn_op_fold_ln: bad argument");
                 need(dtype == STN_DTYPE_BF16 || dtype == STN_DTYPE_F16, "stn_op_fold_ln: a 16-bit format needed");
                 need(!rowvec || nseq > 0, "stn_op_fold_ln: rowvec needs nseq > 0");
                 if (rowvec && row_b) for (int m = 0; m < M; ++m) need(row_b[m] >= 0 && row_b[m] < nseq, "stn_op_fold_ln: row_b out of range");
                 h->eng->op_fold_ln(dtype, M, C, S, part, b2, gamma, rowvec, row_b, nseq, g, b, x, y); })
}
int stn_op_layout(stn_handle* h, int which, int dtype, const int32_t* p, int n_p, const float* a, int64_t a_n, const float* b, int64_t b_n,
                  const float* c, int64_t c_n, const int64_t* ids, int64_t ids_n, const int32_t* len, int packed, float* out, int64_t out_n,
                  float* out2, int64_t out2_n, int32_t* iout, int64_t iout_n) {
    static const int n_params[11] = {3, 4, 5, 3, 4, 3, 6, 6, 5, 1, 5};
    STN_TRY(h, { need(which >= 0 && which < 11 && p && n_p == n_params[which], "stn_op_layout: unknown kernel or parameter count");
                 need(dtype == STN_DTYPE_F32 || dtype == STN_DTYPE_BF16 || dtype == STN_DTYPE_F16, "stn_op_layout: unknown dtype");
                 need(a_n >= 0 && b_n >= 0 && c_n >= 0 && ids_n >= 0 && out_n >= 0 && out2_n >= 0 && iout_n >= 0 && (a || !a_n) && (b || !b_n) && (c || !c_n) &&
                          (ids || !ids_n) && (out || !out_n) && (out2 || !out2_n) && (iout || !iout_n),
                      "stn_op_layout: a buffer without a pointer");
                 h->eng->op_layout(which, dtype, p, a, a_n, b, b_n, c, c_n, ids, ids_n, len, packed, out, out_n, out2, out2_n, iout, iout_n); })
}
int stn_op_attention(stn_handle* h, int dtype, int B, int Lq, int Lk, int H, int dh, const float* q, const float* k,
                     const float* v, const int32_t* qlen, const int32_t* klen, int rope_mode, float* o) {
    STN_TRY(h, { need(B > 0 && Lq > 0 && Lk > 0 && H > 0 && dh >= 8 && dh % 8 == 0 && dh <= 96 && q && k && v && o,
                      "stn_op_attention: bad argument");
                 h->eng->op_attention(dtype, B, Lq, Lk, H, dh, q, k, v, qlen, klen, rope_mode, o); })
}
static void attention_ex_checked(stn_handle* h, int dtype, int B, int Lq, int Lk, int H, int dh, const float* q, int64_t q_elems, int ldq,
                                 int q_col, float* kv, int64_t kv_elems, int ldk, int k_col, int v_col, float* o, int64_t o_elems, int ldo,
                                 const int32_t* qlen, const int32_t* klen, const int32_t* q_off, const int32_t* k_off, int rope_mode,
                                 int k_rotated, int rot_groups, int rot_stride, int rot_col, char* form, size_t form_cap) {
    need(B > 0 && Lq > 0 && Lk > 0 && H > 0 && dh >= 8 && dh % 8 == 0 && dh <= 96 && q && kv && o, "stn_op_attention_ex: bad argument");
    need(dtype == STN_DTYPE_F32 || dtype == STN_DTYPE_BF16 || dtype == STN_DTYPE_F16, "stn_op_attention_ex: unknown dtype");
    need(rope_mode >= -1 && rope_mode <= 1, "stn_op_attention_ex: rope_mode must be -1, 0 or 1");
    const int64_t C = (int64_t)H * dh;
    need(ldq > 0 && ldk > 0 && ldo >= C && q_col >= 0 && k_col >= 0 && v_col >= 0 && q_col + C <= ldq && k_col + C <= ldk && v_col + C <= ldk,
         "stn_op_attention_ex: the heads must lie inside the rows (col + H*dh <= ld, ldo >= H*dh)");
    need((q_off == nullptr || qlen) && (k_off == nullptr || klen), "stn_op_attention_ex: packed rows need their lengths");
    const int64_t qrows = q_elems / ldq, krows = kv_elems / ldk, orows = o_elems / ldo;
    for (int b = 0; b < B; ++b) {
        need(!qlen || qlen[b] >= 0, "stn_op_attention_ex: qlen < 0");
        need(!klen || klen[b] >= 0, "stn_op_attention_ex: klen < 0");
        if (q_off)
            need(qlen[b] <= Lq && q_off[b] >= 0 && (int64_t)q_off[b] + qlen[b] <= std::min(qrows, orows),
                 "stn_op_attention_ex: packed query rows outside q / o (or qlen > Lq)");
        if (k_off) need(k_off[b] >= 0 && (int64_t)k_off[b] + std::min(klen[b], Lk) <= krows, "stn_op_attention_ex: packed key rows outside kv");
    }
    if (!q_off) need((int64_t)B * Lq <= std::min(qrows, orows), "stn_op_attention_ex: q / o hold fewer than B*Lq rows");
    if (!k_off) need((int64_t)B * Lk <= krows, "stn_op_attention_ex: kv holds fewer than B*Lk rows");
    if (k_rotated)
        need(rot_groups >= 1 && rot_stride >= 0 && rot_col >= 0 && rot_col + (int64_t)(rot_groups - 1) * rot_stride + C <= ldk,
             "stn_op_attention_ex: the rotated groups must lie inside the kv rows");
    const std::string f = h->eng->op_attention_ex(dtype, B, Lq, Lk, H, dh, q, q_elems, ldq, q_col, kv, kv_elems, ldk, k_col, v_col, o, o_elems,
                                                  ldo, qlen, klen, q_off, k_off, rope_mode, k_rotated, rot_groups, rot_stride, rot_col);
    if (form && form_cap) std::snprintf(form, form_cap, "%s", f.c_str());
}
int stn_op_attention_ex(stn_handle* h, int dtype, int B, int Lq, int Lk, int H, int dh, const float* q, int64_t q_elems, int ldq,
                        int q_col, float* kv, int64_t kv_elems, int ldk, int k_col, int v_col, float* o, int64_t o_elems, int ldo,
                        const int32_t* qlen, const int32_t* klen, const int32_t* q_off, const int32_t* k_off, int rope_mode, int k_rotated,
                        int rot_groups, int rot_stride, int rot_col, char* form, size_t form_cap) {
    STN_TRY(h, attention_ex_checked(h, dtype, B, Lq, Lk, H, dh, q, q_elems, ldq, q_col, kv, kv_elems, ldk, k_col, v_col, o, o_elems, ldo,
                                    qlen, klen, q_off, k_off, rope_mode, k_rotated, rot_groups, rot_stride, rot_col, form, form_cap))
}
static void xattn_hs_checked(stn_handle* h, int dtype, int M, const float* xn, const float* Wq, const float* bq, const float* Wo, const float* kv,
                             int64_t kv_elems, int ldk, int k_col, int B, int L, int Lk, const int32_t* qlen, const int32_t* klen,
                             const int32_t* k_off, int rope_mode, int pairs_mode, int64_t part_stride, float* part, int64_t part_elems,
                             int32_t* pairs_out, char* form, size_t form_cap) {
    const int C = 384;
    need(M > 0 && B > 0 && B <= 1024 && L > 0 && Lk > 0 && xn && Wq && Wo && kv && qlen && part, "stn_op_xattn_hs: bad argument");
    need(stn::xattn_hs_supported(dtype, C, 4, L, Lk, ldk), "stn_op_xattn_hs: unsupported dtype or shape (xattn_hs_supported)");
    need(rope_mode >= -1 && rope_mode <= 1 && (pairs_mode == 0 || pairs_mode == 1), "stn_op_xattn_hs: rope_mode -1..1, pairs_mode 0 or 1");
    need(k_col >= 0 && k_col % 8 == 0 && k_col + 2 * C <= ldk, "stn_op_xattn_hs: K and V (k_col .. k_col + 768) must lie inside the rows, k_col % 8 == 0");
    need(k_off == nullptr || klen, "stn_op_xattn_hs: packed keys need klen");
    need(part_stride >= (int64_t)M * C && part_elems >= 3 * part_stride + (int64_t)M * C,
         "stn_op_xattn_hs: part must hold 4 heads of M*384 values part_stride apart");
    int64_t rows = 0;
    const int64_t krows = kv_elems / ldk;
    for (int b = 0; b < B; ++b) {
        need(qlen[b] >= 0 && qlen[b] <= L, "stn_op_xattn_hs: qlen out of [0, L]");
        rows += qlen[b];
        need(!klen || klen[b] >= 0, "stn_op_xattn_hs: klen < 0");
        if (k_off) need(k_off[b] >= 0 && (int64_t)k_off[b] + std::min(klen[b], Lk) <= krows, "stn_op_xattn_hs: packed key rows outside kv");
    }
    need(rows <= M, "stn_op_xattn_hs: sum qlen > M");
    if (!k_off) need((int64_t)B * Lk <= krows, "stn_op_xattn_hs: kv holds fewer than B*Lk rows");
    const std::string f = h->eng->op_xattn_hs(dtype, M, xn, Wq, bq, Wo, kv, kv_elems, ldk, k_col, B, L, Lk, qlen, klen, k_off, rope_mode,
                                              pairs_mode, part_stride, part, part_elems, pairs_out);
    if (form && form_cap) std::snprintf(form, form_cap, "%s", f.c_str());
}
int stn_op_xattn_hs(stn_handle* h, int dtype, int M, const float* xn, const float* Wq, const float* bq, const float* Wo, const float* kv,
                    int64_t kv_elems, int ldk, int k_col, int B, int L, int Lk, const int32_t* qlen, const int32_t* klen, const int32_t* k_off,
                    int rope_mode, int pairs_mode, int64_t part_stride, float* part, int64_t part_elems, int32_t* pairs_out, char* form,
                    size_t form_cap) {
    STN_TRY(h, xattn_hs_checked(h, dtype, M, xn, Wq, bq, Wo, kv, kv_elems, ldk, k_col, B, L, Lk, qlen, klen, k_off, rope_mode, pairs_mode,
                                part_stride, part, part_elems, pairs_out, form, form_cap))
}
int stn_dbg_attn_form(int kind, int dtype, int B, int Lq, int Lk, int H, int dh, int ldq, int ldk, int misaligned, char* out, size_t cap) {
    if (B < 1 || Lq < 1 || Lk < 1 || H < 1 || (dtype != STN_DTYPE_F32 && dtype != STN_DTYPE_BF16 && dtype != STN_DTYPE_F16) || (kind != 0 && kind != 1))
        return STN_ERR_INVALID;
    std::string f;
    try {
        if (kind == 0) {
            auto ptr = [&](int bit) { return reinterpret_cast<const void*>((uintptr_t)(misaligned & bit ? 4 : 0)); };
            f = stn::attn_form(dtype, B, Lq, Lk, H, dh, ldq, ldk, ptr(1), ptr(2), ptr(4)).str();
        } else {
            f = stn::xattn_hs_form(dtype, H * dh, H, B, Lq, Lk, ldk).str();
        }
    } catch (const std::exception&) { return STN_ERR_INVALID; }
    if (out && cap > f.size()) std::memcpy(out, f.c_str(), f.size() + 1);
    return (int)f.size();
}
int stn_op_ffn(stn_handle* h, int M, int C, int I, const float* xn, const float* W1, const float* b1, const float* W2, const float* b2,
               const float* gamma, const float* rowvec, const int32_t* row_b, int nseq, float* x, int fused) {
    STN_TRY(h, { need(M > 0 && C > 0 && I > 0 && C % 8 == 0 && I % 8 == 0 && xn && W1 && b1 && W2 && x, "stn_op_ffn: bad argument");
                 need(!rowvec || nseq > 0, "stn_op_ffn: rowvec needs nseq > 0");
                 if (rowvec && row_b) for (int m = 0; m < M; ++m) need(row_b[m] >= 0 && row_b[m] < nseq, "stn_op_ffn: row_b out of range");
                 need(fused >= 0 && fused <= 2, "stn_op_ffn: mode must be 0 (two launches), 1 (K4) or 2 (K4-split + fold)");
                 h->eng->op_ffn(M, C, I, xn, W1, b1, W2, b2, gamma, rowvec, row_b, nseq, x, fused); })
}
static void ffn_ex_checked(stn_handle* h, int dtype, int M, int C, int I, const float* xn, int ldx, int64_t xn_elems, const float* W1, const float* b1,
                           const float* W2, const float* b2, const float* gamma, const int32_t* len, int L, const int32_t* row_b, const float* rowvec,
                           int rv_ld, int nseq, int mode, int split, float* x, int ldo, int64_t x_elems, float* part, int64_t part_stride,
                           int64_t part_elems, char* form, size_t form_cap) {
    need(M > 0 && C > 0 && I > 0 && C % 8 == 0 && I % 8 == 0 && xn && W1 && b1 && W2 && x && L >= 1, "stn_op_ffn_ex: bad argument");
    need((dtype == STN_DTYPE_BF16 || dtype == STN_DTYPE_F16) && dtype == h->eng->dtype(), "stn_op_ffn_ex: dtype must be the 16-bit format of the engine");
// ... 91 lines not shown
```

### supertonic_amd/csrc/engine.hpp

```cpp
#pragma once
#include <cmath>
#include <hip/hip_runtime.h>

#include <algorithm>
#include <cstdint>
#include <functional>
#include <initializer_list>
#include <iterator>
#include <stdexcept>
#include <string>
#include <unordered_map>
#include <vector>

#include "../../include/stn_arch.h"
#include "host/len_tables.hpp"
#include "host/join_plan.hpp"
#include "host/pause_plan.hpp"
#include "host/formant.hpp"
#include "host/pitch.hpp"
#include "kernels.hpp"

namespace stn {

#define STN_HIP(expr)                                                                                          \
// ... 279 lines not shown
    struct FormantProbe {
        float *ax = nullptr, *cy = nullptr;
        double *g = nullptr, *ex = nullptr, *ey = nullptr;
        bool guard_ok = false;
    };
    void op_formant(int hz, int rows, int W, const float* x, const float* y, const int64_t* n, float* out, FormantProbe* probe = nullptr);
    void op_pitch_ex(int hz, int rows, int W, const float* x, const int64_t* n, float semitones, int mode, float* y);
    void op_encode_ex(int enc, int rows, int W, const float* x, int x_misalign, const float* gain, const int64_t* row_id, int mode, uint64_t seed,
                      int64_t dst_stride, void* y);
    JoinPlan batch_join_plan(const stn_join* j);
    void batch_fetch_joined(const stn_join* j, int enc, void* dst, size_t capacity_bytes, int64_t* prog_len, float* prog_dur);
    void batch_fetch_joined_begin(int slot, const stn_join* j, int enc);
    void batch_copy_joined_device(const stn_join* j, int enc, void* dst, int64_t dst_stride);
    void batch_join_loudness(const stn_join* j, float* lufs, float* peak, float* gain);
    void op_join(int hz, int rows, int W, const float* x, const int64_t* n, const stn_join* j, int enc, bool loudness_on, float target_lufs,
                 float ceiling_dbfs, void* y, float* prog_lufs, float* prog_peak, float* prog_gain);

    void set_output_rate(int hz);
    int output_rate() const { return resample_on() ? out_hz_ : a_.sample_rate; }
    bool resample_on() const { return out_hz_ != 0 && out_hz_ != a_.sample_rate; }
    int64_t out_len(int64_t W) const;
    void op_resample(int in_hz, int out_hz, int rows, int W, const float* x, float* y, int16_t* pcm);

    void set_loudness(bool on, float target_lufs, float ceiling_dbfs);
    bool loudness_on() const { return lo_on_; }
    void get_loudness(int* on, float* target_lufs, float* ceiling_dbfs) const;
    void batch_loudness(float* lufs, float* peak, float* gain);
    void op_loudness(int hz, int rows, int W, const float* x, const int64_t* n, float* lufs, float* peak);
    struct LoProbe {
        int x_misalign = 0;
        float *st_end = nullptr, *st_start = nullptr, *pk = nullptr, *pa = nullptr, *pb = nullptr;
        const char* form = "";
    };
    void op_loudness_ex(int hz, int rows, int W, const float* x, const int64_t* n, bool on, float target, float ceiling, LoProbe& probe,
                        float* lufs, float* peak, float* gain);
    void batch_loudness_range(float* m_max, float* s_max, float* lra, int32_t* n_st);
    void batch_join_loudness_range(const stn_join* j, float* m_max, float* s_max, float* lra, int32_t* n_st);
    void op_loudness_range(int hz, int rows, int W, const float* x, const int64_t* n, float* m_max, float* s_max, float* lra, int32_t* n_st);

    void set_silence_trim(bool on, float top_db, float keep_ms, float fade_ms);
    bool silence_trim_on() const { return st_on_; }
    void get_silence_trim(int* on, float* top_db, float* keep_ms, float* fade_ms) const;
    void batch_silence_edges(int64_t* start, int64_t* end);
    void op_silence_edges(int hz, int rows, int W, const float* x, const int64_t* n, float top_db, float keep_ms, int64_t* start, int64_t* end);
    void op_silence_trim(int hz, int rows, int W, const float* x, const int64_t* n, float top_db, float keep_ms, float fade_ms, const float* gain,
                         int enc, void* y, int64_t* start, int64_t* end);
    void set_pause_limit(bool on, float max_pause_ms);
    bool pause_limit_active() const { return pl_on_ && st_on_; }
    void get_pause_limit(int* on, float* max_pause_ms) const;
    void batch_pauses(int64_t* len, int32_t* n_cuts, int64_t* cuts, int cap_pairs);
    void op_pause_trim(int hz, int rows, int W, const float* x, const int64_t* n, float top_db, float keep_ms, float fade_ms, float max_pause_ms,
                       const float* gain, int enc, void* y, int64_t* start, int64_t* end, int64_t* len, int32_t* n_cuts, int64_t* cuts, int cap_pairs);
    struct EdProbe {
        int x_misalign = 0;
        float *pa = nullptr, *pb = nullptr;
        double* lev = nullptr;
        const char* form = "";
    };
    void op_silence_edges_ex(int hz, int rows, int W, const float* x, const int64_t* n, float top_db, float keep_ms, float fade_ms, float max_pause_ms,
                             EdProbe& probe, int64_t* start, int64_t* end, int64_t* len, int32_t* n_cuts, int64_t* cuts, int cap_pairs);
    void dbg_batch_set_wav(const float* wav);
    int64_t span_uploads() const { return sp_uploads_; }

    void set_limiter(bool on, float lookahead_ms);
    bool limiter_active() const { return lm_on_ && lo_on_; }
    void get_limiter(int* on, float* lookahead_ms) const;
    void batch_limiter(float* reduction_db, int64_t* limited);
    void op_limiter(int hz, int rows, int W, const float* x, const int64_t* n, const float* gain, float ceiling_dbfs, float lookahead_ms, float* y,
                    float* s, float* reduction_db, int64_t* limited);
    void op_limiter_ex(int hz, int rows, int W, const float* x, const int64_t* n, const float* gain, float ceiling_dbfs, float lookahead_ms, float* y,
                       float* s, float* reduction_db, int64_t* limited, int peak_mode, float* env, float* trim);

    void set_peak_mode(int mode);
    int peak_mode() const { return pk_true_ ? 1 : 0; }
    void batch_true_peak(float* tp_in, float* tp_out, float* trim);
    const char* op_true_peak(int hz, int rows, int W, const float* x, const int64_t* n, const float* gain, int x_misalign, float* tp, float* env,
                             float* pk);

    void set_filters(int n, const stn_filter* f);
    bool filter_on() const { return !fl_set_.empty(); }
    const std::vector<stn_filter>& filters() const { return fl_set_; }
    struct FlProbe {
        int x_misalign = 0;
        float *st_end = nullptr, *st_start = nullptr;
        bool guard_ok = false;
        const char* form = "";
    };
    void op_filter(int hz, int rows, int W, const float* x, int n, const stn_filter* f, float* y, FlProbe* probe);

    void set_compressor(bool on, const stn_compressor* c);
    bool compressor_on() const { return cp_.on; }
    const stn_compressor& compressor() const { return cp_.set; }
    void batch_compressor(float* max_reduction_db);
    struct CpProbe {
        int x_misalign = 0, in_place = 0;
        float *gr = nullptr, *s1_end = nullptr, *s1_start = nullptr, *s2_end = nullptr, *s2_start = nullptr;
        bool guard_ok = false;
        const char* form = "";
    };
    void op_compressor(int hz, int rows, int W, const float* x, const stn_compressor& c, float* y, CpProbe* probe);

    void set_deesser(bool on, const stn_deesser* c);
    bool deesser_on() const { return ds_.on; }
    const stn_deesser& deesser() const { return ds_.set; }
    void batch_deesser(float* max_reduction_db);
    struct DsProbe {
        int x_misalign = 0, in_place = 0;
        float *band = nullptr, *gr = nullptr, *st_end = nullptr, *st_start = nullptr;
        float *s1_end = nullptr, *s1_start = nullptr, *s2_end = nullptr, *s2_start = nullptr;
        bool guard_ok = false;
        const char* form = "";
    };
    void op_deesser(int hz, int rows, int W, const float* x, const stn_deesser& c, float* y, DsProbe* probe);

    void set_expander(bool on, const stn_expander* c);
    bool expander_on() const { return xp_.on; }
    const stn_expander& expander() const { return xp_.set; }
    void batch_expander(float* min_attenuation_db, int64_t* closed_samples);
    struct XpProbe {
        int x_misalign = 0, in_place = 0;
        float *open = nullptr, *s1_end = nullptr, *s1_start = nullptr, *s2_end = nullptr, *s2_start = nullptr;
        bool guard_ok = false;
        const char* form = "";
    };
    void op_expander(int hz, int rows, int W, const float* x, const stn_expander& c, float* y, XpProbe* probe);

    void profile_enable(bool on) { if (on != prof_on_) profile_reset(); prof_on_ = on; }
    void launch_log_enable(bool on);
    std::string launch_log() const;
    void profile_sample(int every) { prof_every_ = every < 1 ? 1 : every; prof_seen_ = 0; }
    void profile_filter(const std::string& family) { if (family != prof_filter_) profile_reset(); prof_filter_ = family; }
    void profile_reset();
    std::vector<std::pair<std::string, KernelStat>> profile_collect();

    void op_gemm(int dtype, int M, int N, int K, const float* A, const float* W, const float* bias, int act, float* out);
    std::string op_gemm_ex(int dtype, int M, int N, int K, const float* A, const float* W, int mode, int act, int out_dtype, int ldo,
                           const float* bias, const float* gamma, const int* len, int L, const int* row_b, const float* rowvec, int nseq,
                           int nt, int tr, float* out, int64_t out_elems);
    std::string op_attention_ex(int dtype, int B, int Lq, int Lk, int H, int dh, const float* q, int64_t q_elems, int ldq, int q_col,
                                float* kv, int64_t kv_elems, int ldk, int k_col, int v_col, float* o, int64_t o_elems, int ldo,
                                const int* qlen, const int* klen, const int* q_off, const int* k_off, int rope_mode, int k_rotated,
                                int rot_groups, int rot_stride, int rot_col);
    std::string op_xattn_hs(int dtype, int M, const float* xn, const float* Wq, const float* bq, const float* Wo, const float* kv,
                            int64_t kv_elems, int ldk, int k_col, int B, int L, int Lk, const int* qlen, const int* klen, const int* k_off,
                            int rope_mode, int pairs_mode, int64_t part_stride, float* part, int64_t part_elems, int* pairs_out);
    void op_attention(int dtype, int B, int Lq, int Lk, int H, int dh, const float* q, const float* k, const float* v,
                      const int* qlen, const int* klen, int rope_mode, float* o);
    std::string op_gemm_rows(int dtype, int M, int N, int K, const float* A, const float* W, const float* bias, int B, const int* rows,
                             const int* valid, int T, float* out, int64_t out_elems);
    void op_dwconv_ln(int dtype, int B, int L, int C, int k, int dil, const float* x, const float* w, const float* bias,
                      const float* g, const float* b, float* y, const int* seqlen = nullptr );
    std::string op_dwconv_ln_ex(int dtype, int B, int L, int C, int k, int dil, const float* x, int64_t x_rows, const float* w, const float* bias,
                                const float* g, const float* b, const int* seqlen, int packed, int ln_only, float* y, int64_t y_rows,
                                const float* tail = nullptr, int T = 0, int rf = 0);
    void op_fold_ln(int dtype, int M, int C, int S, const float* part, const float* b2, const float* gamma, const float* rowvec, const int* row_b,
                    int nseq, const float* g, const float* b, float* x, float* y);
    void op_layout(int which, int dtype, const int* p, const float* a, int64_t a_n, const float* b, int64_t b_n, const float* c, int64_t c_n,
                   const int64_t* ids, int64_t ids_n, const int* len, int packed, float* out, int64_t out_n, float* out2, int64_t out2_n, int* iout,
                   int64_t iout_n);
    double op_gemm_bench(int dtype, int M, int N, int K, int mode, int iters);
    void op_gemm_phases(int dtype, int M, int N, int K, int mode, double* out6);
    void op_randn(uint64_t seed, int B, int D, int L, const int64_t* utt_ids, const int* len, float* out);
    void op_ffn(int M, int C, int I, const float* xn, const float* W1, const float* b1, const float* W2, const float* b2, const float* gamma,
                const float* rowvec , const int* row_b , int nseq, float* x, int mode);
    std::string op_ffn_ex(int M, int C, int I, const float* xn, int ldx, int64_t xn_elems, const float* W1, const float* b1, const float* W2,
                          const float* b2, const float* gamma, const int* len, int L, const int* row_b, const float* rowvec, int rv_ld, int nseq,
                          int mode, int split, float* x, int ldo, int64_t x_elems, float* part, int64_t part_stride, int64_t part_elems);
    void op_fold_dwconv_ln(int B, int C, int k, int dil, int S, const int* seqlen, const float* x, const float* part, const float* b2,
                           const float* gamma, const float* rowvec , const float* w , const float* bias,
                           const float* g, const float* b, float* x_out, float* y);
    std::string op_fold_dwconv_ln_ex(int dtype, int B, int L, int C, int k, int dil, int S, int run_frames, const int* seqlen, const float* x_in,
                                     int64_t x_rows, const float* part, int64_t part_stride, int64_t part_elems, const float* b2, const float* gamma,
                                     const float* rowvec, int rv_ld, const float* w, const float* bias, const float* g, const float* b, float* x_out,
                                     int64_t x_out_rows, float* y, int64_t y_rows);
    void op_ffn_bench(int M, int C, int I, int mode, int iters, double* out5);
    void op_block_bench(int B, int L, int C, int I, int k, int dil, int mode, int iters, double* out6);

    Arena& arena() { return ar_; }

   private:
    DevTensor& tensor(const std::string& name);
    const float* vecf(const std::string& name) { return tensor(name).f32; }
    Linear linear(const std::string& prefix);
    LNorm lnorm(const std::string& prefix);
    ConvNeXt convnext_w(const std::string& prefix);
    Attn attn_w(const std::string& prefix, bool self);
    void free_weights();
    using RawSource = std::function<std::vector<float>(const std::string& name, int kind, int rows, int cols, float gain)>;
    void load_weights(const stn_arch& a, const RawSource& src, std::vector<std::string>* names_only);

    size_t act_bytes(int64_t n) const { return (size_t)n * (is_half(dt_) ? 2 : 4); }
    void* act_alloc(int64_t n) { return ar_.alloc(act_bytes(n)); }
    float* f32_alloc(int64_t n) { return static_cast<float*>(ar_.alloc((size_t)n * 4)); }
    void gemm(const char* tag, int dt, const void* A, int lda, const Linear& w, int M, Epilogue e);
    struct FoldState {
        float* x = nullptr;
        float* x_alt = nullptr;
        void* part = nullptr;
        int64_t part_stride = 0;
        bool pending = false;
        FoldArgs fold;
    };
    FfnForm ffn_plan(int stage, int C, int I, int64_t M, int64_t gate_rows, bool packed, int k, int max_dil) const {
        return ffn_form(dt_, stage, C, I, M, gate_rows, packed, k, max_dil, fused_ffn_, ffn_min_rows_, ffn_split_min_rows_, nt_hints_);
    }
    FoldArgs ffn_launch(const FfnForm& f, int C, const FfnArgs& a, const Linear& w1, const Linear& w2);
    static FoldArgs ffn_pending(const FfnForm& f, const FfnArgs& a) {
        return FoldArgs{a.part, f.split, a.part_stride, a.b2, a.gamma, a.rowvec, a.rv_ld, a.row_b};
    }
    struct FfnOp { FfnForm f; Linear w1, w2; FfnArgs a; };
    FfnOp op_ffn_setup(const char* op, int mode, int M, int C, int I, const float* W1, const float* W2, int split = 0);
    void convnext(const ConvNeXt& p, const FfnForm& f, float* x, int B, int L, int C, int hid, int k, int dil, const int* len,
                  const int* conv_len = nullptr, const float* rowvec = nullptr, int rv_ld = 0, const Ragged* rg = nullptr, FoldState* fs = nullptr,
                  const DwconvTail& tl = DwconvTail() );
    void fold_layernorm(FoldState& fs, int64_t M, int C, const LNorm& ln, void* xn, const char* tag);
    void attn_block(const Attn& p, float* x, int B, int Lq, int C, int H, const void* ctx, int Lk, const int* qlen,
                    const int* klen, int rope_mode, bool self, const Ragged* qrg = nullptr);
    void* to_act(const float* src, int64_t n);

    struct ProfSpan { std::string tag; hipEvent_t a, b; double flops, bytes; };
    void prof_begin(const char* tag, double flops, double bytes);
    void prof_end();
    class StageSpan {
       public:
        StageSpan(Engine& e, const char* stage, const char* tag, double flops, double bytes) : e_(e), prev_(e.stage_) {
            e_.stage_ = stage;
            begin(tag, flops, bytes);
        }
        ~StageSpan() { end(); e_.stage_ = prev_; }
        StageSpan(const StageSpan&) = delete;
        StageSpan& operator=(const StageSpan&) = delete;
        void next(const char* tag, double flops, double bytes) { end(); begin(tag, flops, bytes); }

       private:
        void begin(const char* tag, double flops, double bytes) { if ((begun_ = e_.prof_on_)) e_.prof_begin(tag, flops, bytes); }
        void end() { if (begun_) e_.prof_end(); begun_ = false; }
        Engine& e_;
        const char* prev_;
        bool begun_ = false;
    };

    int device_, dt_;
    int n_cu_ = 256;
    hipStream_t s_ = nullptr, own_s_ = nullptr;
    const char* stage_ = "";
    std::string prof_filter_;
    std::string log_family_;
    int prof_every_ = 1;
    uint64_t prof_seen_ = 0;
    bool prof_active_ = false;
    stn_arch a_{};
    bool loaded_ = false;
    int64_t params_ = 0;
    std::unordered_map<std::string, DevTensor> w_;
    std::vector<void*> owned_;
    Arena ar_;
    Batch bt_;
    std::vector<void*> batch_owned_;
    std::vector<void*> batch_retired_;
    template <typename T> void ensure(T*& p, size_t& cap, size_t need);
    std::vector<float> reported_dur_;
    uint64_t drains_ = 0;
    std::vector<int64_t> out_spans(int64_t W, int hz) const;
    struct BatchSpans {
        RowSpans dev;
        std::vector<int64_t> host;
        uint64_t seq = 0, drains = ~0ull; int hz = 0; int64_t W = 0;
    };
    const BatchSpans& batch_spans(int hz, int64_t W);
    BatchSpans sp_[2];
    DevBuf sp_buf_;
    int64_t sp_uploads_ = 0;
    RowSpans op_spans(int rows, int W, std::vector<int64_t> n);
    std::vector<int64_t> op_sp_;
    void enqueue_after_duration(int total_step, const std::function<void()>& take_text_rows);
    struct GraphKey {
        int B = 0, Lt = 0, L = 0, steps = 0; bool noise = false, ragged = false; int xattn = 0; int ffn = 0; int rows = 0, vrows = 0, trows = 0; int vform = 0;
        uint64_t gen = 0, wgen = 0; const void* p0 = nullptr; const void* p1 = nullptr; const void* pin = nullptr; hipStream_t s = nullptr;
        bool operator==(const GraphKey& o) const {
            return B == o.B && Lt == o.Lt && L == o.L && steps == o.steps && noise == o.noise && ragged == o.ragged && xattn == o.xattn && ffn == o.ffn &&
                   rows == o.rows && vrows == o.vrows && vform == o.vform && trows == o.trows && gen == o.gen && wgen == o.wgen && p0 == o.p0 && p1 == o.p1 && pin == o.pin && s == o.s;
        }
    };
    struct GraphEntry { GraphKey key; hipGraph_t graph = nullptr, graph2 = nullptr; hipGraphExec_t exec = nullptr, exec2 = nullptr; uint64_t last_use = 0; };
    static constexpr size_t kGraphCache = 8, kWarmKeys = 16;
    std::vector<GraphEntry> graphs_;
    std::vector<GraphKey> warm_keys_;
    uint64_t graph_clock_ = 0, wgen_ = 0;
    void drop_graphs();
    bool graph_on_ = true;
    bool vo_ragged_ = false;
    bool packed_ve_ = true;
    bool nt_hints_ = true;
    hipStream_t dp_s_ = nullptr, te_s_ = nullptr;
    Arena dp_ar_, te_ar_;
    hipEvent_t ev_te_ = nullptr, ev_copied_ = nullptr, ev_dp_ = nullptr;
    std::function<void()> text_gate_;
    bool copied_valid_ = false;
    int64_t ffn_min_rows_ = 18432;
    int64_t ffn_split_min_rows_ = 1;
    int fused_ffn_ = 9;
    bool shape_buckets_ = false;
    bool dur_read_always_ = false;
    int gelu_act_ = ACT_GELU;
    int fused_xattn_ = 1;
    int64_t last_ve_rows_ = 0, last_vo_rows_ = 0;
    struct VoConsts {
// ... 190 lines not shown
```

### supertonic_amd/csrc/engine_ops.cpp

```cpp
#include "engine.hpp"
#include "engine_internal.hpp"

#include <algorithm>
#include <cmath>
#include <cstdio>
#include <cstring>

namespace stn {
using detail::up;

void Engine::op_gemm(int dtype, int M, int N, int K, const float* A, const float* W, const float* bias, int act, float* out) {
    STN_HIP(hipSetDevice(device_));
    ar_.reset();
    float* dA = up(ar_, s_, A, (size_t)M * K);
    float* dW = up(ar_, s_, W, (size_t)N * K);
    float* dB = bias ? up(ar_, s_, bias, (size_t)N) : nullptr;
    float* dO = f32_alloc((size_t)M * N);
    const void* pa = dA;
    const void* pw = dW;
    if (is_half(dtype)) {
        void* a16 = ar_.alloc((size_t)M * K * 2);
        void* w16 = ar_.alloc((size_t)N * K * 2);
        launch_cast(s_, dtype, dA, (int64_t)M * K, a16);
        launch_cast(s_, dtype, dW, (int64_t)N * K, w16);
// ... 382 lines not shown
    STN_HIP(hipEventRecord(a, s_));
    for (int i = 0; i < iters; ++i) run(nullptr);
    STN_HIP(hipEventRecord(b, s_));
    STN_HIP(hipEventSynchronize(b));
    float ms = 0.f;
    STN_HIP(hipEventElapsedTime(&ms, a, b));
    (void)hipEventDestroy(a); (void)hipEventDestroy(b);
    out5[0] = ms / iters;
    if (op.f.kind != FFN_GEMMS) {
        STN_HIP(hipMemsetAsync(ts, 0, sizeof(unsigned long long) * 4 * (size_t)nwg, s_));
        run(ts);
        std::vector<unsigned long long> h((size_t)4 * nwg);
        STN_HIP(hipMemcpyAsync(h.data(), ts, sizeof(unsigned long long) * h.size(), hipMemcpyDeviceToHost, s_));
        sync();
        double s1 = 0, s2 = 0, s3 = 0;
        int live = 0;
        for (int w = 0; w < nwg; ++w) {
            if (!h[4 * w + 3]) continue;
            ++live;
            s1 += (double)(h[4 * w + 1] - h[4 * w]); s2 += (double)(h[4 * w + 2] - h[4 * w + 1]); s3 += (double)(h[4 * w + 3] - h[4 * w + 2]);
        }
        if (live) { out5[1] = s1 / live; out5[2] = s2 / live; out5[3] = s3 / live; }
        out5[4] = live;
    }
    STN_HIP(hipGetLastError());
    sync();
}

void Engine::op_fold_dwconv_ln(int B, int C, int k, int dil, int S, const int* seqlen, const float* x, const float* part, const float* b2,
                               const float* gamma, const float* rowvec, const float* w, const float* bias, const float* g, const float* b,
                               float* x_out, float* y) {
    if (!is_half(dt_)) throw std::invalid_argument("op_fold_dwconv_ln: 16-bit engines only");
    int L = 0;
    int64_t M = 0;
    for (int i = 0; i < B; ++i) { M += seqlen[i]; L = std::max(L, seqlen[i]); }
    std::fill(x_out, x_out + M * C, 0.f);
    std::fill(y, y + M * C, 0.f);
    op_fold_dwconv_ln_ex(dt_, B, L, C, k, dil, S, 0, seqlen, x, M, part, M * C, M * C * S, b2, gamma, rowvec, C, w, bias, g, b, x_out, M, y, M);
}

void Engine::op_block_bench(int B, int L, int C, int I, int k, int dil, int mode, int iters, double* out2) {
    STN_HIP(hipSetDevice(device_));
    ar_.reset();
    for (int i = 0; i < 6; ++i) out2[i] = 0.0;
    const int64_t M = (int64_t)B * L;
    float* wr = f32_alloc((int64_t)I * C);
    launch_randn_masked(s_, 12, nullptr, 1, I, C, nullptr, wr);
    launch_scale(s_, wr, I * C, 0.05f);
    FfnOp op = op_ffn_setup("op_block_bench", mode, (int)M, C, I, wr, wr);
    std::vector<int> len(B, L), off(B + 1);
    for (int i = 0; i <= B; ++i) off[i] = i * L;
    const int* dlen = up(ar_, s_, len.data(), (size_t)B);
    const int* doff = up(ar_, s_, off.data(), (size_t)B + 1);
    float* xa = f32_alloc(M * C);
    float* xb = f32_alloc(M * C);
    launch_randn_masked(s_, 11, nullptr, 1, (int)M, C, nullptr, xa);
    float* d_b1 = f32_alloc(I);
    float* d_b2 = f32_alloc(C);
    float* d_g = f32_alloc(C);
    float* d_one = f32_alloc(C);
    float* dwt = f32_alloc((int64_t)k * C);
    launch_fill(s_, d_b1, I, 0.01f); launch_fill(s_, d_b2, C, 0.01f); launch_fill(s_, d_g, C, 0.01f); launch_fill(s_, d_one, C, 1.f);
    launch_fill(s_, dwt, k * C, 1.f / k);
    void* xn = act_alloc(M * C);
    op.a.xn = xn; op.a.b1 = d_b1; op.a.b2 = d_b2; op.a.gamma = d_g;
    const bool split = op.f.kind == FFN_K4_SPLIT;
    if (split) STN_HIP(hipMemsetAsync(op.a.part, 0, (size_t)op.a.part_stride * op.f.split * 2, s_));
    FoldArgs fo = ffn_pending(op.f, op.a);
    auto conv = [&]() {
        if (split) { launch_fold_dwconv_ln(s_, dt_, xa, xb, B, L, C, fo, dwt, d_b2, k, dil, d_one, d_b2, 1e-6f, xn, dlen, doff); std::swap(xa, xb); }
        else launch_dwconv_ln(s_, dt_, xa, B, L, C, dwt, d_b2, k, dil, d_one, d_b2, 1e-6f, xn, dlen, doff);
    };
    auto block = [&]() { conv(); op.a.x = xa; ffn_launch(op.f, C, op.a, op.w1, op.w2); };
    hipEvent_t a, b;
    STN_HIP(hipEventCreate(&a)); STN_HIP(hipEventCreate(&b));
    for (int which = 0; which < 2; ++which) {
        for (int i = 0; i < 3; ++i) { if (which) conv(); else block(); }
        STN_HIP(hipEventRecord(a, s_));
        for (int i = 0; i < iters; ++i) { if (which) conv(); else block(); }
        STN_HIP(hipEventRecord(b, s_));
        STN_HIP(hipEventSynchronize(b));
        float ms = 0.f;
        STN_HIP(hipEventElapsedTime(&ms, a, b));
        out2[which] = ms / iters;
    }
    (void)hipEventDestroy(a); (void)hipEventDestroy(b);
    if (split) {
        const int nwg = B * ((L + 7) / 8);
        unsigned long long* ts = static_cast<unsigned long long*>(ar_.alloc(sizeof(unsigned long long) * 4 * (size_t)nwg));
        STN_HIP(hipMemsetAsync(ts, 0, sizeof(unsigned long long) * 4 * (size_t)nwg, s_));
        fo.ts = ts;
        conv();
        fo.ts = nullptr;
        std::vector<unsigned long long> h((size_t)4 * nwg);
        STN_HIP(hipMemcpyAsync(h.data(), ts, sizeof(unsigned long long) * h.size(), hipMemcpyDeviceToHost, s_));
        sync();
        double p1 = 0, p2 = 0, p3 = 0; int live = 0;
        unsigned long long tmin = ~0ull, tmax = 0;
        for (int w = 0; w < nwg; ++w) {
            if (!h[4 * w + 3]) continue;
            ++live;
            p1 += (double)(h[4 * w + 1] - h[4 * w]); p2 += (double)(h[4 * w + 2] - h[4 * w + 1]); p3 += (double)(h[4 * w + 3] - h[4 * w + 2]);
            tmin = std::min(tmin, h[4 * w]); tmax = std::max(tmax, h[4 * w + 3]);
        }
        if (live) { out2[2] = p1 / live; out2[3] = p2 / live; out2[4] = p3 / live; out2[5] = (double)(tmax - tmin); }
    }
    STN_HIP(hipGetLastError());
    sync();
}

static void down_as(Arena& ar, hipStream_t s, int dtype, const void* d, float* h, size_t n) {
    const float* src = static_cast<const float*>(d);
    if (is_half(dtype)) {
        float* w = static_cast<float*>(ar.alloc(n * 4));
        launch_half_to_f32(s, dtype, d, (int64_t)n, w);
        src = w;
    }
    STN_HIP(hipMemcpyAsync(h, src, n * 4, hipMemcpyDeviceToHost, s));
}

std::string Engine::op_ffn_ex(int M, int C, int I, const float* xn, int ldx, int64_t xn_elems, const float* W1, const float* b1, const float* W2,
                              const float* b2, const float* gamma, const int* len, int L, const int* row_b, const float* rowvec, int rv_ld, int nseq,
                              int mode, int split, float* x, int ldo, int64_t x_elems, float* part, int64_t part_stride, int64_t part_elems) {
    STN_HIP(hipSetDevice(device_));
    ar_.reset();
    float* d_w1 = up(ar_, s_, W1, (size_t)I * C);
    float* d_w2 = up(ar_, s_, W2, (size_t)C * I);
    FfnOp op = op_ffn_setup("op_ffn_ex", mode, M, C, I, d_w1, d_w2, split);
    FfnArgs& fa = op.a;
    fa.xn = up_as(ar_, s_, dt_, xn, (size_t)xn_elems); fa.ldx = ldx;
    float* d_x = up(ar_, s_, x, (size_t)x_elems);
    fa.x = d_x; fa.ldo = ldo;
    fa.b1 = up(ar_, s_, b1, (size_t)I);
    fa.b2 = b2 ? up(ar_, s_, b2, (size_t)C) : nullptr;
    fa.gamma = gamma ? up(ar_, s_, gamma, (size_t)C) : nullptr;
    fa.rowvec = rowvec ? up(ar_, s_, rowvec, (size_t)nseq * rv_ld) : nullptr; fa.rv_ld = rv_ld;
    fa.row_b = row_b ? up(ar_, s_, row_b, (size_t)M) : nullptr;
    fa.len = len ? up(ar_, s_, len, (size_t)nseq) : nullptr; fa.L = L;
    void* d_part = nullptr;
    if (op.f.kind == FFN_K4_SPLIT) {
        d_part = up_as(ar_, s_, dt_, part, (size_t)part_elems);
        fa.part = d_part; fa.part_stride = part_stride;
    }
    ffn_launch(op.f, C, fa, op.w1, op.w2);
    STN_HIP(hipGetLastError());
    STN_HIP(hipMemcpyAsync(x, d_x, sizeof(float) * (size_t)x_elems, hipMemcpyDeviceToHost, s_));
    if (d_part) down_as(ar_, s_, dt_, d_part, part, (size_t)part_elems);
    sync();
    return op.f.str();
}

std::string Engine::op_dwconv_ln_ex(int dtype, int B, int L, int C, int k, int dil, const float* x, int64_t x_rows, const float* w,
                                    const float* bias, const float* g, const float* b, const int* seqlen, int packed, int ln_only, float* y,
                                    int64_t y_rows, const float* tail, int T, int rf) {
    STN_HIP(hipSetDevice(device_));
    ar_.reset();
    const int* dlen = seqlen ? up(ar_, s_, seqlen, (size_t)B) : nullptr;
    float* dx = up(ar_, s_, x, (size_t)x_rows * C);
    float* dg = up(ar_, s_, g, (size_t)C);
    float* dbt = up(ar_, s_, b, (size_t)C);
    void* dy = up_as(ar_, s_, dtype, y, (size_t)y_rows * C);
    std::string form = "layernorm";
    if (ln_only) {
        launch_layernorm(s_, dtype, dx, (int64_t)B * L, C, dg, dbt, 1e-6f, dy);
    } else {
        std::vector<float> wt((size_t)C * k);
        for (int c = 0; c < C; ++c) for (int j = 0; j < k; ++j) wt[(size_t)j * C + c] = w[(size_t)c * k + j];
        float* dw = up(ar_, s_, wt.data(), wt.size());
        float* db = up(ar_, s_, bias, (size_t)C);
        int* off = nullptr;
        if (packed) {
            off = static_cast<int*>(ar_.alloc(sizeof(int) * (size_t)(B + 1)));
            launch_row_map(s_, dlen, B, off, nullptr);
        }
        DwconvTail tl;
        if (tail) { tl.tail = up(ar_, s_, tail, (size_t)(rf + 1) * C); tl.T = T; tl.rf = rf; }
        form = dwconv_ln_form(dtype, B, L, C, k, packed != 0).str();
        launch_dwconv_ln(s_, dtype, dx, B, L, C, dw, db, k, dil, dg, dbt, 1e-6f, dy, dlen, off, tl);
    }
    STN_HIP(hipGetLastError());
    down_as(ar_, s_, dtype, dy, y, (size_t)y_rows * C);
    sync();
    return form;
}

void Engine::op_fold_ln(int dtype, int M, int C, int S, const float* part, const float* b2, const float* gamma, const float* rowvec,
                        const int* row_b, int nseq, const float* g, const float* b, float* x, float* y) {
    STN_HIP(hipSetDevice(device_));
    ar_.reset();
    const size_t n = (size_t)M * C;
    FoldArgs fo;
    fo.part = up_as(ar_, s_, dtype, part, n * S); fo.S = S; fo.part_stride = (int64_t)n;
    fo.b2 = up(ar_, s_, b2, (size_t)C); fo.gamma = up(ar_, s_, gamma, (size_t)C);
    fo.rowvec = rowvec ? up(ar_, s_, rowvec, (size_t)nseq * C) : nullptr; fo.rv_ld = C;
    fo.row_b = (rowvec && row_b) ? up(ar_, s_, row_b, (size_t)M) : nullptr;
    float* dx = up(ar_, s_, x, n);
    float* dg = up(ar_, s_, g, (size_t)C);
    float* dbt = up(ar_, s_, b, (size_t)C);
    void* dy = ar_.alloc(n * 2);
    launch_fold_ln(s_, dtype, dx, M, C, fo, dg, dbt, 1e-6f, dy);
    STN_HIP(hipGetLastError());
    STN_HIP(hipMemcpyAsync(x, dx, n * 4, hipMemcpyDeviceToHost, s_));
    down_as(ar_, s_, dtype, dy, y, n);
    sync();
}

std::string Engine::op_fold_dwconv_ln_ex(int dtype, int B, int L, int C, int k, int dil, int S, int run_frames, const int* seqlen, const float* x_in,
                                         int64_t x_rows, const float* part, int64_t part_stride, int64_t part_elems, const float* b2, const float* gamma,
                                         const float* rowvec, int rv_ld, const float* w, const float* bias, const float* g, const float* b, float* x_out,
                                         int64_t x_out_rows, float* y, int64_t y_rows) {
    STN_HIP(hipSetDevice(device_));
    ar_.reset();
    std::vector<float> wt((size_t)C * k);
    for (int c = 0; c < C; ++c) for (int j = 0; j < k; ++j) wt[(size_t)j * C + c] = w[(size_t)c * k + j];
    const int* dlen = up(ar_, s_, seqlen, (size_t)B);
    int* doff = static_cast<int*>(ar_.alloc(sizeof(int) * (size_t)(B + 1)));
    launch_row_map(s_, dlen, B, doff, nullptr);
    float* dx = up(ar_, s_, x_in, (size_t)x_rows * C);
    float* dxo = up(ar_, s_, x_out, (size_t)x_out_rows * C);
    void* dy = up_as(ar_, s_, dtype, y, (size_t)y_rows * C);
    float* dw = up(ar_, s_, wt.data(), wt.size());
    float* db = up(ar_, s_, bias, (size_t)C);
    float* dg = up(ar_, s_, g, (size_t)C);
    float* dbt = up(ar_, s_, b, (size_t)C);
    FoldArgs fo;
    fo.part = up_as(ar_, s_, dtype, part, (size_t)part_elems); fo.S = S; fo.part_stride = part_stride;
    if (b2) fo.b2 = up(ar_, s_, b2, (size_t)C);
    else { float* z = f32_alloc(C); launch_fill(s_, z, C, 0.f); fo.b2 = z; }
    if (gamma) fo.gamma = up(ar_, s_, gamma, (size_t)C);
    else { float* o = f32_alloc(C); launch_fill(s_, o, C, 1.f); fo.gamma = o; }
    fo.rowvec = rowvec ? up(ar_, s_, rowvec, (size_t)B * rv_ld) : nullptr; fo.rv_ld = rowvec ? rv_ld : C;
    fo.run_frames = run_frames;
    const std::string form = fold_dwconv_ln_form(dtype, B, L, C, k, dil, S, rowvec != nullptr, run_frames).str();
    launch_fold_dwconv_ln(s_, dtype, dx, dxo, B, L, C, fo, dw, db, k, dil, dg, dbt, 1e-6f, dy, dlen, doff);
    STN_HIP(hipGetLastError());
    STN_HIP(hipMemcpyAsync(x_out, dxo, sizeof(float) * (size_t)x_out_rows * C, hipMemcpyDeviceToHost, s_));
    down_as(ar_, s_, dtype, dy, y, (size_t)y_rows * C);
    sync();
    return form;
}

void Engine::op_layout(int which, int dtype, const int* p, const float* a, int64_t a_n, const float* b, int64_t b_n, const float* c, int64_t c_n,
                       const int64_t* ids, int64_t ids_n, const int* len, int packed, float* out, int64_t out_n, float* out2, int64_t out2_n,
                       int* iout, int64_t iout_n) {
    STN_HIP(hipSetDevice(device_));
    ar_.reset();
    auto need = [](bool ok, const char* what) { if (!ok) throw std::invalid_argument(std::string("stn_op_layout: ") + what); };
    auto rows_needed = [&](int B, int rows_per_seq) -> int64_t {
        if (!packed) return (int64_t)B * rows_per_seq;
        int64_t t = 0;
        for (int i = 0; i < B; ++i) t += len[i];
        return t;
    };
    auto check_len = [&](int B, int hi, bool required) {
        need(B > 0 && B <= 1024, "1 <= B <= 1024");
        need(len || !(required || packed), "lengths needed");
        if (len) for (int i = 0; i < B; ++i) need(len[i] >= 0 && len[i] <= hi, "a length outside [0, rows per sequence]");
    };
    auto row_off = [&](const int* dlen, int B) -> int* {
        if (!packed) return nullptr;
        int* off = static_cast<int*>(ar_.alloc(sizeof(int) * (size_t)(B + 1)));
        launch_row_map(s_, dlen, B, off, nullptr);
        return off;
    };
    switch (which) {
    case 0: {
        const int B = p[0], rows_padded = p[1], with_b = p[2];
        need(B > 0 && len && iout && rows_padded >= 0, "row_map: B > 0, lengths and iout needed");
        if (B > 1024) { launch_row_map(s_, nullptr, B, nullptr, nullptr); return; }
        int64_t tot = 0;
        for (int i = 0; i < B; ++i) { need(len[i] >= 0 && len[i] < (1 << 20), "row_map: length out of range"); tot += len[i]; }
        need(iout_n >= B + 1 + (with_b ? std::max<int64_t>(tot, rows_padded) : 0), "row_map: iout too small");
        const int* dlen = up(ar_, s_, len, (size_t)B);
        int* d = up(ar_, s_, iout, (size_t)iout_n);
        launch_row_map(s_, dlen, B, d, with_b ? d + B + 1 : nullptr, rows_padded);
        STN_HIP(hipMemcpyAsync(iout, d, (size_t)iout_n * 4, hipMemcpyDeviceToHost, s_));
        break;
    }
    case 1: {
        const int B = p[0], C = p[1], L = p[2], ldo = p[3];
        need(C > 0 && L > 0 && ldo >= C && a && out, "ncl_to_rows: bad shape");
        check_len(B, L, false);
        need(a_n >= (int64_t)B * C * L && out_n >= rows_needed(B, L) * ldo, "ncl_to_rows: buffer too small");
        const int* dlen = len ? up(ar_, s_, len, (size_t)B) : nullptr;
        float* da = up(ar_, s_, a, (size_t)a_n);
        void* d = up_as(ar_, s_, dtype, out, (size_t)out_n);
        launch_ncl_to_rows(s_, dtype, da, B, C, L, d, ldo, dlen, row_off(dlen, B));
        down_as(ar_, s_, dtype, d, out, (size_t)out_n);
        break;
    }
    case 2: {
        const int B = p[0], D = p[1], L = p[2], with_z = p[3], ldz = p[4];
        need(D > 0 && L > 0 && a && b && c && out && (!with_z || (out2 && ldz >= D)), "euler_ncl: bad shape");
        check_len(B, L, false);
        const int64_t vr = rows_needed(B, L);
        need(a_n >= (int64_t)B * D * L && out_n >= (int64_t)B * D * L && c_n >= B && b_n >= vr * D && (!with_z || out2_n >= vr * ldz), "euler_ncl: buffer too small");
        const int* dlen = len ? up(ar_, s_, len, (size_t)B) : nullptr;
        float* dp = up(ar_, s_, a, (size_t)a_n);
        float* dv = up(ar_, s_, b, (size_t)b_n);
        float* ddt = up(ar_, s_, c, (size_t)c_n);
        float* d = up(ar_, s_, out, (size_t)out_n);
        void* dz = with_z ? up_as(ar_, s_, dtype, out2, (size_t)out2_n) : nullptr;
        launch_euler_ncl(s_, dp, dv, ddt, dlen, B, D, L, d, row_off(dlen, B), dz, dtype, ldz);
        STN_HIP(hipMemcpyAsync(out, d, (size_t)out_n * 4, hipMemcpyDeviceToHost, s_));
        if (dz) down_as(ar_, s_, dtype, dz, out2, (size_t)out2_n);
        break;
    }
    case 3: {
        const int B = p[0], T = p[1], W = p[2];
        need(T > 0 && W > 0 && W % 4 == 0 && a && out, "unpack_rows: bad shape");
        packed = 1;
        check_len(B, T, true);
        need(a_n >= rows_needed(B, T) * W && a_n > 0 && out_n >= (int64_t)B * T * W, "unpack_rows: buffer too small");
        const int* dlen = up(ar_, s_, len, (size_t)B);
        float* da = up(ar_, s_, a, (size_t)a_n);
        float* d = up(ar_, s_, out, (size_t)out_n);
        launch_unpack_rows(s_, da, dlen, row_off(dlen, B), B, T, W, d);
        STN_HIP(hipMemcpyAsync(out, d, (size_t)out_n * 4, hipMemcpyDeviceToHost, s_));
        break;
    }
    case 4: {
        const int vocab = p[0], B = p[1], L = p[2], C = p[3];
        need(vocab > 0 && L > 0 && C > 0 && C % 4 == 0 && ids && a && out, "embed: bad shape");
        check_len(B, L, true);
        need(ids_n >= (int64_t)B * L && a_n >= (int64_t)vocab * C && out_n >= rows_needed(B, L) * C, "embed: buffer too small");
        const int* dlen = up(ar_, s_, len, (size_t)B);
        int64_t* di = up(ar_, s_, ids, (size_t)ids_n);
        float* da = up(ar_, s_, a, (size_t)a_n);
        float* d = up(ar_, s_, out, (size_t)out_n);
        launch_embed(s_, di, da, vocab, B, L, C, dlen, d, row_off(dlen, B));
        STN_HIP(hipMemcpyAsync(out, d, (size_t)out_n * 4, hipMemcpyDeviceToHost, s_));
// ... 95 lines not shown
```

### supertonic_amd/csrc/kernels.hpp

```cpp
#pragma once
#include <hip/hip_runtime.h>
#include <hip/hip_ext.h>
#include <stdint.h>
#include <stdio.h>
#include <stdlib.h>

#include <stdexcept>
#include <type_traits>
#include <utility>
#include <vector>
#include <string>

#include "dither.hpp"

namespace stn {

struct LaunchEvents { hipEvent_t start = nullptr, stop = nullptr; };
inline thread_local LaunchEvents g_launch_ev;
struct LaunchLog {
    bool on = false;
    const char* family = "-";
    std::vector<std::pair<std::string, const char*>> entries;
    void add(const char* kexpr) { if (entries.size() < 200000) entries.emplace_back(family, kexpr); }
};
// ... 3 lines not shown
        if (::stn::g_launch_log.on) ::stn::g_launch_log.add(#kernel);                                                   \
        if (::stn::g_launch_ev.start) {                                                                                 \
            const ::stn::LaunchEvents ev_ = ::stn::g_launch_ev;                                                         \
            ::stn::g_launch_ev = ::stn::LaunchEvents{};                                                                 \
            hipExtLaunchKernelGGL(kernel, grid, block, lds, stream, ev_.start, ev_.stop, 0, __VA_ARGS__);               \
        } else {                                                                                                        \
            hipLaunchKernelGGL(kernel, grid, block, lds, stream, __VA_ARGS__);                                          \
        }                                                                                                               \
    } while (0)

struct PerDeviceOnce {
    bool done[64] = {};
    bool need() { int d = 0; (void)hipGetDevice(&d); d &= 63; if (done[d]) return false; done[d] = true; return true; }
};

inline void stn_check_hip(hipError_t e, const char* what) {
    if (e != hipSuccess) throw std::runtime_error(std::string("HIP error: ") + what + " failed: " + hipGetErrorString(e));
}


enum DType : int { F32 = 0, BF16 = 1, F16 = 2 };
__host__ __device__ inline bool is_half(int dt) { return dt == BF16 || dt == F16; }
typedef _Float16 f16_t;
template <typename Fn>
inline void with_out_type(int dtype, Fn&& fn) {
    if (dtype == F16) fn(static_cast<f16_t*>(nullptr));
    else if (dtype == BF16) fn(static_cast<uint16_t*>(nullptr));
    else fn(static_cast<float*>(nullptr));
}
template <typename Fn>
inline void with_half_type(int dtype, Fn&& fn) {
    if (dtype == F16) fn(static_cast<f16_t*>(nullptr));
    else fn(static_cast<uint16_t*>(nullptr));
}
enum ActFn : int { ACT_NONE = 0, ACT_GELU = 1, ACT_SILU = 2, ACT_GELU_TANH = 3 };

enum EpiMode : int {
    EPI_STORE = 0,
    EPI_RESID = 1,
    EPI_STORE_T = 2,
};

struct Epilogue {
    int mode = EPI_STORE;
    int act = ACT_NONE;
    int out_dtype = F32;
    const float* bias = nullptr;
    void* out = nullptr;
    int ldo = 0;
    const float* gamma = nullptr;
    float* resid = nullptr;
    const int* len = nullptr;
    int L = 1;
    const int* row_b = nullptr;
    const float* rowvec = nullptr;
    int rv_ld = 0;
    const int* map_off = nullptr;
    const int* map_valid = nullptr;
    int map_B = 0, map_T = 0;
    int ksplit = 1;
    int nt = 0;
    int tr_epilogue = 0;
    int tr_force = -1;
    unsigned long long* ts = nullptr;
};

enum GemmKernel : int { GK_TILED = 0, GK_RING_VEC = 1, GK_RING = 2, GK_REG = 3 };
enum GemmEpiForm : int { GE_LANE = 0, GE_SLAB = 1, GE_TR = 2 };
constexpr int GEMM_CFG_F32_64 = 19, GEMM_CFG_F32_128 = 20;
struct GemmForm {
    int dtype = F32, mode = EPI_STORE;
    int kernel = GK_REG;
    int cfg = 0;
    int bm = 128, bn = 128, wm = 2, wn = 2, nstage = 2, ks = 64, esz = 2;
    int epi = GE_LANE;
    int tr_epilogue = 0;
    int split = 1;
    std::string str() const;
};
GemmForm gemm_form(int dtype, int M, int N, int K, int lda, int ldw, const Epilogue& e, const void* A, const void* W, bool allow_split = true);
void launch_gemm_form(hipStream_t s, const GemmForm& f, const void* A, int lda, const void* W, int ldw, int M, int N, int K,
                      const Epilogue& e, float* workspace);
bool gemm_form_maps_rows(const GemmForm& f);
void launch_gemm(hipStream_t s, int dtype, const void* A, int lda, const void* W, int ldw, int M, int N, int K,
                 const Epilogue& e);
int gemm_splitk_factor(int dtype, int M, int N, int K, const Epilogue& e);
void launch_gemm_splitk(hipStream_t s, int dtype, const void* A, int lda, const void* W, int ldw, int M, int N, int K, const Epilogue& e,
                        int S, float* workspace);

struct FfnArgs {
    const void* xn = nullptr; int ldx = 0;
    const void* wseq = nullptr;
    const float* b1 = nullptr;
    const float* b2 = nullptr;
    const float* gamma = nullptr;
    float* x = nullptr; int ldo = 0;
    int M = 0, I = 0;
    const int* row_b = nullptr;
    const float* rowvec = nullptr; int rv_ld = 0;
    const int* len = nullptr; int L = 1;
    unsigned long long* ts = nullptr;
    int split = 1;
    void* part = nullptr;
    int64_t part_stride = 0;
};
bool ffn_fused_supported(int dtype, int C, int I);
int ffn_split_factor(int dtype, int C, int I);
constexpr int FFN_SPLITS[] = {4, 8, 12};
bool ffn_split_valid(int dtype, int C, int I, int S);
int ffn_split_choose(int dtype, int C, int I, int64_t M);
inline int64_t ffn_split_rows(int64_t M) { return (M + 127) / 128 * 128; }
enum FfnKind : int { FFN_GEMMS = 0, FFN_K4 = 1, FFN_K4_SPLIT = 2 };
enum FfnStage : int { FFN_VOCODER = 1, FFN_ESTIMATOR = 2, FFN_TEXT = 4 };
struct FfnForm {
    int kind = FFN_GEMMS, split = 1;
    bool nt = false;
    std::string str() const;
};
FfnForm ffn_form(int dtype, int stage, int C, int I, int64_t M, int64_t gate_rows, bool packed, int k, int max_dil, int mask, int64_t min_rows,
                 int64_t split_min_rows, bool nt_hints);
__host__ __device__ constexpr inline int ffn_lds_side_offset(int C, int I) { return (4 * C * 64 + (I + 2 * C) * 4 + 1023) & ~1023; }
__host__ __device__ constexpr inline bool ffn_lds_has_side(int C) { return C == 384; }
void launch_ffn_fused(hipStream_t s, int dtype, int C, const FfnArgs& a);
struct FoldArgs {
    const void* part = nullptr; int S = 0; int64_t part_stride = 0;
    const float* b2 = nullptr;
    const float* gamma = nullptr;
    const float* rowvec = nullptr; int rv_ld = 0;
    const int* row_b = nullptr;
    unsigned long long* ts = nullptr;
    int run_frames = 0;
};
int fold_run_frames(const int* lengths, int B, int n_cu);
void launch_fold_ln(hipStream_t s, int act_dtype, float* x, int64_t M, int C, const FoldArgs& f, const float* g, const float* b, float eps, void* y);
bool fold_dwconv_ln_supported(int C, int k, int dil);
struct FoldDwconvLnForm {
    int act_dtype = BF16, K = 5, nslot = 3, S = 4, U = 1, run = 32, cps = 1;
    bool rv = false;
    unsigned grid = 0;
    size_t lds = 0;
    std::string str() const;
};
FoldDwconvLnForm fold_dwconv_ln_form(int act_dtype, int B, int L, int C, int k, int dil, int S, bool has_rowvec, int run_frames);
void launch_fold_dwconv_ln(hipStream_t s, int act_dtype, const float* x_in, float* x_out, int B, int L, int C, const FoldArgs& f, const float* w_t,
                           const float* bias, int k, int dil, const float* ln_g, const float* ln_b, float eps, void* y, const int* seqlen,
                           const int* row_off);
void launch_repack_frag_acc(hipStream_t s, const void* W, int N, int K, void* Wf);
void launch_ffn_pack(hipStream_t s, const void* W1, const void* W2, int C, int I, void* tmp, void* wseq, int S = 1);

struct DwconvTail {
    const float* tail = nullptr;
    int T = 0, rf = 0;
};
void launch_dwconv_ln(hipStream_t s, int out_dtype, const float* x, int B, int L, int C, const float* w_t,
                      const float* bias, int k, int dil, const float* ln_g, const float* ln_b, float eps, void* y,
                      const int* seqlen = nullptr, const int* row_off = nullptr, const DwconvTail& tl = DwconvTail());
enum DwconvLnKernel : int { DW_V3 = 0, DW_V2 = 1, DW_GENERIC = 2 };
struct DwconvLnForm {
    int out_dtype = F32;
    int kernel = DW_GENERIC;
    int K = 0, R = 1;
    bool occ4 = false;
    std::string str() const;
};
DwconvLnForm dwconv_ln_form(int out_dtype, int B, int L, int C, int k, bool packed);
bool dwconv_ln_supports_packed(int C, int k);
void launch_row_map(hipStream_t s, const int* len, int B, int* row_off , int* row_b ,
                    int rows_padded = 0 );
constexpr int LN_NI = 4;
void check_ln_shape(int C);
void launch_layernorm(hipStream_t s, int out_dtype, const float* x, int64_t M, int C, const float* g, const float* b,
                      float eps, void* y);

enum AttnVec : int { ATTN_VEC_Q = 1, ATTN_VEC_K = 2, ATTN_VEC_V = 4 };
struct AttnForm {
    int dtype = F32;
    bool mfma = false;
    int dh = 0;
    int kc = 0, nch = 0;
    int tpr = 8, vec = 0;
    size_t lds = 0;
    std::string str() const;
};
AttnForm attn_form(int dtype, int B, int Lq, int Lk, int H, int dh, int ldq, int ldk, const void* q, const void* k, const void* v);
void launch_attention(hipStream_t s, int dtype, const void* q, int ldq, const void* k, const void* v, int ldk, void* o,
                      int ldo, int B, int Lq, int Lk, int H, int dh, const int* qlen, const int* klen, int rope_mode,
                      float rope_base, float rope_gamma, bool k_rotated = false,
                      const int* q_off = nullptr ,
                      const int* k_off = nullptr );
void launch_repack_frag(hipStream_t s, const void* W, int N, int K, void* Wf);
bool xattn_hs_supported(int dtype, int C, int H, int L, int Lk, int ldk);
void launch_xattn_hs(hipStream_t s, int dtype, const void* xn, int64_t M, const void* WqF, const float* bq, const void* kp, const void* vp, int ldk,
                     const void* WoA, void* part, int64_t part_stride, int B, int L, int Lk, const int* qlen, const int* klen,
                     const int* q_off, const int* k_off, int rope_mode, float rope_base, float rope_gamma, unsigned long long* ts = nullptr,
                     const int* pairs = nullptr );
struct XattnHsForm {
    bool f16 = false;
    int U = 1, kc = 32;
    size_t lds = 0;
    std::string str() const;
};
XattnHsForm xattn_hs_form(int dtype, int C, int H, int B, int L, int Lk, int ldk);
void launch_xattn_hs_pairs(hipStream_t s, const int* qlen, int B, int* pairs);
void launch_rope_rows(hipStream_t s, int dtype, void* x, int ld, int B, int L, const int* len, int groups, int group_stride,
                      int H, int dh, int rope_mode, float rope_base, float rope_gamma, const int* row_off = nullptr );

void launch_embed(hipStream_t s, const int64_t* ids, const float* emb, int vocab, int B, int L, int C, const int* len,
                  float* x, const int* row_off = nullptr );
void launch_mask_to_len(hipStream_t s, const float* mask, int B, int L, int* len);
void launch_ncl_to_rows(hipStream_t s, int out_dtype, const float* in, int B, int C, int L, void* out, int ld_out = 0,
                        const int* len = nullptr, const int* row_off = nullptr );
void launch_euler_ncl(hipStream_t s, const float* prev, const float* v, const float* dt, const int* len, int B, int D, int L, float* out,
                      const int* row_off = nullptr , void* z_rows = nullptr, int z_dtype = 0, int ldz = 0);
void launch_cast(hipStream_t s, int out_dtype, const float* in, int64_t n, void* out);
void launch_add_rowvec(hipStream_t s, float* x, const float* v, int ldv, int B, int L, int C, const int* len);
void launch_time_embed(hipStream_t s, const float* cur, const float* tot, int B, int dim, float scale, float* te);
void launch_scale_len(hipStream_t s, const int* len, int B, int factor, int* out);
void launch_vocoder_in(hipStream_t s, const float* latent, int B, int L, int ld, int ccf, const float* w ,
                       const float* bias, int C, int k, float* x, const int* seqlen = nullptr);
void launch_vocoder_im2col(hipStream_t s, int out_dtype, const float* latent, int B, int L, int ld, int ccf, int k, int kp, void* cols,
                           const int* seqlen = nullptr ,
                           const int* row_off = nullptr );
void launch_fill_rows(hipStream_t s, const int* valid, int B, int T, int W, int rf, const float* quiet, const float* edge, float* dst);
void launch_unpack_rows(hipStream_t s, const float* src, const int* len, const int* row_off, int B, int T, int W, float* dst);
void launch_trim_len(hipStream_t s, const int* len, int B, int ccf, int T, int rf, int* n_out, int* valid_out, bool tail_form = false);
void launch_unpack_rows_quiet(hipStream_t s, const float* src, const int* valid, const int* row_off, int B, int T, int W, int rf,
                              const float* quiet, const float* edge, float* dst);
void launch_masked_mean(hipStream_t s, int in_dtype, const void* x, int B, int L, int C, const int* len, float* pooled,
                        const int* row_off = nullptr );
void launch_softplus(hipStream_t s, float* x, int n);
void launch_scale(hipStream_t s, float* x, int n, float mul);
void launch_randn_masked(hipStream_t s, uint64_t seed, const int64_t* utt_ids, int B, int D, int L, const int* len,
                         float* xt, const unsigned long long* seed_dev = nullptr );
void launch_mask_ncl(hipStream_t s, float* x, int B, int D, int L, const int* len);
void launch_reciprocal(hipStream_t s, const float* in, int n, float* out);
void launch_bf16_to_f32(hipStream_t s, const uint16_t* in, int64_t n, float* out);
void launch_half_to_f32(hipStream_t s, int in_dtype, const void* in, int64_t n, float* out);
void launch_fill(hipStream_t s, float* x, int n, float v);
void launch_step_counters(hipStream_t s, float* tot , float* cur , float* dt , int B, int steps);
enum OutEnc : int { ENC_F32 = 0, ENC_PCM16 = 1, ENC_PCM24 = 2, ENC_MULAW = 3, ENC_ALAW = 4 };
constexpr int enc_bytes(int enc) {
    return enc == ENC_F32 ? 4 : enc == ENC_PCM16 ? 2 : enc == ENC_PCM24 ? 3 : (enc == ENC_MULAW || enc == ENC_ALAW) ? 1 : 0;
}
template <typename Fn>
inline void with_enc(int enc, const char* who, Fn&& fn) {
    switch (enc) {
        case ENC_F32: fn(std::integral_constant<int, ENC_F32>{}); break;
        case ENC_PCM16: fn(std::integral_constant<int, ENC_PCM16>{}); break;
        case ENC_PCM24: fn(std::integral_constant<int, ENC_PCM24>{}); break;
        case ENC_MULAW: fn(std::integral_constant<int, ENC_MULAW>{}); break;
        case ENC_ALAW: fn(std::integral_constant<int, ENC_ALAW>{}); break;
        default: throw std::invalid_argument(std::string(who) + ": unknown encoding " + std::to_string(enc));
    }
}
struct Dither {
    int mode = DITHER_OFF; uint64_t seed = 0; unsigned kind = DITHER_ROW; const int64_t* ids = nullptr;
    const int64_t* lim = nullptr; int64_t lim_stride = 1;
};
void launch_store_rows(hipStream_t s, const float* x, int64_t rows, int64_t W, const float* g, int enc, void* y, int64_t dst_stride, const Dither& d = {});
struct JoinSeg { int64_t dst, len, row; };
struct JoinProg { int64_t len; int32_t first, count; };
void launch_join_rows(hipStream_t s, const float* x, int64_t src_stride, const JoinSeg* seg, const JoinProg* prog, int G, int64_t Wj, const float* g,
                      int enc, void* y, int64_t dst_stride, const Dither& d = {});
struct JoinSegT { int64_t dst, len, row, src; int32_t fin, fout; };
void launch_join_trim_rows(hipStream_t s, const float* x, int64_t src_stride, const JoinSegT* seg, const JoinProg* prog, int G, int64_t Wj,
                           const float* g, const float* fade, int enc, void* y, int64_t dst_stride, const Dither& d = {});

constexpr int ED_CHUNK = 32;
constexpr int ED_WG = 256;
__host__ __device__ inline int64_t ed_chunks(int64_t W) { return (W + ED_CHUNK - 1) / ED_CHUNK; }
inline int edges_frame(int hz) { return (hz + 50) / 100; }
inline int64_t edges_frames(int64_t W, int hz) { const int F = edges_frame(hz); return (W + F - 1) / F; }
void launch_edges_frames(hipStream_t s, const float* x, int64_t rows, int64_t W, const int64_t* n, int hz, float* pa, float* pb);
void launch_edges_rows(hipStream_t s, int64_t rows, int64_t W, const int64_t* n, int hz, double top_db, int64_t keep, int64_t fd, const float* pa,
                       const float* pb, double* lev, int64_t* edges, JoinSegT* seg, JoinProg* prog);
const char* edges_staging_form(const float* x, int64_t W);
constexpr int PZ_MAX_CUTS = 255;
void launch_pause_rows(hipStream_t s, int64_t rows, int64_t W, const int64_t* n, int hz, double top_db, int64_t fd, int64_t Mp, int S, const double* lev,
                       const int64_t* edges, JoinSegT* seg, JoinProg* prog, int64_t* cuts);

struct ResampleTable {
    int in_hz = 0, out_hz = 0;
    int P = 0, Q = 0, T = 0, off = 0;
    std::vector<float> taps;
    float* dev = nullptr;
};
constexpr int RESAMPLE_MIN_HZ = 8000, RESAMPLE_MAX_HZ = 192000, RESAMPLE_MAX_P = 640;
inline int64_t resample_out_len(int64_t W, int P, int Q) { return (W * P + Q - 1) / Q; }
std::string resample_design(int in_hz, int out_hz, ResampleTable& f);
void resample_design_pq(int P, int Q, int in_hz, int out_hz, ResampleTable& f);
double bessel_i0(double x);
void launch_resample(hipStream_t s, const float* x, int64_t rows, int64_t W, const ResampleTable& f, int enc, void* y, int64_t dst_stride, int64_t cap = 0);
struct ResampleForm {
    int G = 1;
    bool lds = true;
    int64_t lds_bytes = 0;
    int64_t grid_x = 0;
    std::string str() const;
};
ResampleForm resample_form(int64_t W, const ResampleTable& f);

void launch_pitch_search(hipStream_t s, const float* x, int64_t rows, int64_t W, const int64_t* n, int H, int64_t M, int a, int b, int* delta, float* score);
void launch_pitch_ola(hipStream_t s, const float* x, int64_t rows, int64_t W, const int64_t* n, int H, int64_t M, int64_t Ws, int a, int b, const int* delta,
                      const float* win, float* y);

void launch_formant_lpc(hipStream_t s, const float* x, const float* y, int64_t rows, int64_t W, const int64_t* n, int H, int64_t F, int p, const float* win,
                        const double* lagw, float* ax, float* cy, double* g, double* ex, double* ey);
void launch_formant_filter(hipStream_t s, const float* y, int64_t rows, int64_t W, const int64_t* n, int H, int64_t F, int p, const float* win,
                           const float* ax, const float* cy, float* out);
// ... 92 lines not shown
```

### supertonic_amd/csrc/kernels_dwconv_ln.hip

```cpp
#include "kernels.hpp"
#include "kernels_dev.hpp"
#include "dev_env.hpp"

#include <type_traits>
#include <stdio.h>
#include <stdlib.h>

namespace stn {

template <typename OutT, bool CONV>
__global__ __launch_bounds__(256) void dwconv_ln_kernel(const float* __restrict__ x, int64_t M, int L, int C,
                                                        const float* __restrict__ w_t, const float* __restrict__ bias,
                                                        int k, int dil, const float* __restrict__ g,
                                                        const float* __restrict__ bt, float eps, OutT* __restrict__ y,
                                                        const int* __restrict__ seqlen) {
    const int lane = threadIdx.x & 63;
    const int64_t row = (int64_t)blockIdx.x * 4 + (threadIdx.x >> 6);
    if (row >= M) return;
    const int Lv = (CONV && seqlen) ? seqlen[row / L] : L;
    const bool live = !(CONV && (int)(row % L) >= Lv);
    const int C4 = C >> 2;
    const float4* x4 = reinterpret_cast<const float4*>(x);
    float4 h[LN_NI];
    if (CONV) {
        const int t = (int)(row % L);
        const int64_t base = row - t;
        const int half = (k - 1) >> 1;
        const float4* w4 = reinterpret_cast<const float4*>(w_t);
        const float4* b4 = reinterpret_cast<const float4*>(bias);
#pragma unroll
        for (int i = 0; i < LN_NI; ++i) {
            const int c4 = lane + 64 * i;
            h[i] = make_float4(0.f, 0.f, 0.f, 0.f);
            if (c4 < C4) {
                float4 a = b4[c4];
                for (int j = 0; j < k; ++j) {
                    const int tt = t + (j - half) * dil;
                    if (tt >= 0 && tt < Lv) {
                        const float4 xv = x4[(base + tt) * C4 + c4];
                        const float4 wv = w4[(int64_t)j * C4 + c4];
                        a.x = fmaf(wv.x, xv.x, a.x); a.y = fmaf(wv.y, xv.y, a.y);
                        a.z = fmaf(wv.z, xv.z, a.z); a.w = fmaf(wv.w, xv.w, a.w);
                    }
                }
                h[i] = a;
            }
        }
    } else {
#pragma unroll
        for (int i = 0; i < LN_NI; ++i) {
            const int c4 = lane + 64 * i;
            h[i] = make_float4(0.f, 0.f, 0.f, 0.f);
            if (c4 < C4) h[i] = x4[row * C4 + c4];
        }
    }
    float s = 0.f;
#pragma unroll
    for (int i = 0; i < LN_NI; ++i) s += (h[i].x + h[i].y) + (h[i].z + h[i].w);
    const float mean = wave_sum(s) / (float)C;
    float v = 0.f;
#pragma unroll
    for (int i = 0; i < LN_NI; ++i) {
        if (lane + 64 * i < C4) {
            const float dx = h[i].x - mean, dy = h[i].y - mean, dz = h[i].z - mean, dw = h[i].w - mean;
            v += (dx * dx + dy * dy) + (dz * dz + dw * dw);
        }
    }
    const float rstd = rsqrtf(wave_sum(v) / (float)C + eps);
    const float4* g4 = reinterpret_cast<const float4*>(g);
    const float4* bt4 = reinterpret_cast<const float4*>(bt);
#pragma unroll
    for (int i = 0; i < LN_NI; ++i) {
        const int c4 = lane + 64 * i;
        if (c4 < C4) {
            const float4 gg = g4[c4], bb = bt4[c4];
            store4(y + row * C + c4 * 4, live ? (h[i].x - mean) * rstd * gg.x + bb.x : 0.f, live ? (h[i].y - mean) * rstd * gg.y + bb.y : 0.f,
                   live ? (h[i].z - mean) * rstd * gg.z + bb.z : 0.f, live ? (h[i].w - mean) * rstd * gg.w + bb.w : 0.f);
        }
    }
}

template <typename OutT, int K, int R>
__global__ __launch_bounds__(256) void dwconv_ln_v2_kernel(const float* __restrict__ x, int64_t M, int L, int C,
                                                           const float* __restrict__ w_t, const float* __restrict__ bias,
                                                           int dil, const float* __restrict__ g,
                                                           const float* __restrict__ bt, float eps, OutT* __restrict__ y,
                                                           const int* __restrict__ seqlen) {
    const int lane = threadIdx.x & 63;
    const int64_t r0 = ((int64_t)blockIdx.x * 4 + (threadIdx.x >> 6)) * R;
    if (r0 >= M) return;
    const int C4 = C >> 2;
    constexpr int HALF = (K - 1) / 2;
    const float4* x4 = reinterpret_cast<const float4*>(x);
    const float4* w4 = reinterpret_cast<const float4*>(w_t);
    const float4* b4 = reinterpret_cast<const float4*>(bias);
    int tpos[R], lv[R];
    int64_t base[R];
    bool rowok[R];
#pragma unroll
    for (int r = 0; r < R; ++r) {
        const int64_t row = r0 + r < M ? r0 + r : M - 1;
        tpos[r] = (int)(row % L);
        base[r] = row - tpos[r];
        lv[r] = seqlen ? seqlen[row / L] : L;
        rowok[r] = r0 + r < M;
    }
    float4 h[R][2];
#pragma unroll
    for (int i = 0; i < 2; ++i) {
        const int c4 = lane + 64 * i;
        const bool act = c4 < C4;
        const int cc = act ? c4 : 0;
        float4 xv[R][K];
        float4 wv[K];
#pragma unroll
        for (int j = 0; j < K; ++j) wv[j] = w4[(int64_t)j * C4 + cc];
#pragma unroll
        for (int r = 0; r < R; ++r)
#pragma unroll
            for (int j = 0; j < K; ++j) {
                const int tt = tpos[r] + (j - HALF) * dil;
                const int tc = tt < 0 ? 0 : (tt >= L ? L - 1 : tt);
                xv[r][j] = x4[(base[r] + tc) * C4 + cc];
            }
        const float4 bv = b4[cc];
#pragma unroll
        for (int r = 0; r < R; ++r) {
            float4 a = bv;
#pragma unroll
            for (int j = 0; j < K; ++j) {
                const int tt = tpos[r] + (j - HALF) * dil;
                const bool keep = tt >= 0 && tt < lv[r];
                const float4 v = keep ? xv[r][j] : make_float4(0.f, 0.f, 0.f, 0.f);
                a.x = fmaf(wv[j].x, v.x, a.x); a.y = fmaf(wv[j].y, v.y, a.y);
                a.z = fmaf(wv[j].z, v.z, a.z); a.w = fmaf(wv[j].w, v.w, a.w);
            }
            h[r][i] = act ? a : make_float4(0.f, 0.f, 0.f, 0.f);
        }
    }
    const float4* g4 = reinterpret_cast<const float4*>(g);
    const float4* bt4 = reinterpret_cast<const float4*>(bt);
#pragma unroll
    for (int r = 0; r < R; ++r) {
        float s = (h[r][0].x + h[r][0].y) + (h[r][0].z + h[r][0].w) + (h[r][1].x + h[r][1].y) + (h[r][1].z + h[r][1].w);
        const float mean = wave_sum(s) / (float)C;
        float v = 0.f;
#pragma unroll
        for (int i = 0; i < 2; ++i)
            if (lane + 64 * i < C4) {
                const float dx = h[r][i].x - mean, dy = h[r][i].y - mean, dz = h[r][i].z - mean, dw = h[r][i].w - mean;
                v += (dx * dx + dy * dy) + (dz * dz + dw * dw);
            }
        const float rstd = rsqrtf(wave_sum(v) / (float)C + eps);
        if (!rowok[r]) continue;
        const bool live = tpos[r] < lv[r];
#pragma unroll
        for (int i = 0; i < 2; ++i) {
            const int c4 = lane + 64 * i;
            if (c4 < C4) {
                const float4 gg = g4[c4], bb = bt4[c4];
                store4(y + (r0 + r) * C + c4 * 4, live ? (h[r][i].x - mean) * rstd * gg.x + bb.x : 0.f, live ? (h[r][i].y - mean) * rstd * gg.y + bb.y : 0.f,
                       live ? (h[r][i].z - mean) * rstd * gg.z + bb.z : 0.f, live ? (h[r][i].w - mean) * rstd * gg.w + bb.w : 0.f);
            }
        }
    }
}

template <typename OutT, int K, int R, bool TAIL = false>
__device__ __forceinline__ void dwconv_ln_v3_body(const float* __restrict__ x, int nseq, int L, int C,
                                                           const float* __restrict__ w_t, const float* __restrict__ bias,
                                                           int dil, int wps , const float* __restrict__ g,
                                                           const float* __restrict__ bt, float eps, OutT* __restrict__ y,
                                                           const int* __restrict__ seqlen, const int* __restrict__ row_off, int xcd_runs,
                                                           const float* __restrict__ tail = nullptr, int T = 0, int rf = 0) {
    const int lane = threadIdx.x & 63;
    int bid = blockIdx.x;
    if (xcd_runs) {
        const int nb = gridDim.x, q = nb >> 3, rr = nb & 7, xcd = bid & 7, idx = bid >> 3;
        bid = xcd * q + (xcd < rr ? xcd : rr) + idx;
    }
    const int64_t wid = (int64_t)bid * 4 + (threadIdx.x >> 6);
    if (wid >= (int64_t)nseq * wps) return;
    const int b = (int)(wid / wps), rem = (int)(wid % wps);
    const int t0 = (rem / dil) * (R * dil) + (rem % dil);
    const int Lv = seqlen ? seqlen[b] : L;
    constexpr int HALF = (K - 1) / 2, NWIN = R + K - 1;
    const int C4 = C >> 2;
    const int64_t row0 = row_off ? (int64_t)row_off[b] : (int64_t)b * L;
    if (t0 >= Lv) {
        if (row_off) return;
#pragma unroll
        for (int r = 0; r < R; ++r) {
            const int t = t0 + r * dil;
            if (t >= L) break;
#pragma unroll
            for (int i = 0; i < 2; ++i)
                if (lane + 64 * i < C4) store4(y + (row0 + t) * C + (lane + 64 * i) * 4, 0.f, 0.f, 0.f, 0.f);
        }
        return;
    }
    const float4* x4 = reinterpret_cast<const float4*>(x) + row0 * C4;
    const float4* w4 = reinterpret_cast<const float4*>(w_t);
    const float4* b4 = reinterpret_cast<const float4*>(bias);
    float4 h[R][2];
#pragma unroll
    for (int i = 0; i < 2; ++i) {
        const int c4 = lane + 64 * i;
        const bool act = c4 < C4;
        const int cc = act ? c4 : 0;
        float4 win[NWIN], wv[K];
#pragma unroll
        for (int j = 0; j < K; ++j) wv[j] = w4[(int64_t)j * C4 + cc];
#pragma unroll
        for (int q = 0; q < NWIN; ++q) {
            const int tt = t0 + (q - HALF) * dil;
            const int hi_ = row_off ? Lv : L;
            const int tc = tt < 0 ? 0 : (tt >= hi_ ? hi_ - 1 : tt);
            if constexpr (TAIL) {
                const float4* src = x4 + (int64_t)tc * C4;
                bool keep = tt >= 0 && tt < Lv;
                if (tt >= Lv && tt < T) {
                    const int j = T - 1 - tt;
                    src = reinterpret_cast<const float4*>(tail) + (int64_t)(j < rf ? j : rf) * C4;
                    keep = true;
                }
                const float4 v = src[cc];
                win[q] = keep ? v : make_float4(0.f, 0.f, 0.f, 0.f);
            } else {
                const float4 v = x4[(int64_t)tc * C4 + cc];
                win[q] = (tt >= 0 && tt < Lv) ? v : make_float4(0.f, 0.f, 0.f, 0.f);
            }
        }
        const float4 bv = b4[cc];
#pragma unroll
        for (int r = 0; r < R; ++r) {
            float4 a = bv;
#pragma unroll
            for (int j = 0; j < K; ++j) {
                a.x = fmaf(wv[j].x, win[r + j].x, a.x); a.y = fmaf(wv[j].y, win[r + j].y, a.y);
                a.z = fmaf(wv[j].z, win[r + j].z, a.z); a.w = fmaf(wv[j].w, win[r + j].w, a.w);
            }
            h[r][i] = act ? a : make_float4(0.f, 0.f, 0.f, 0.f);
        }
    }
    const float4* g4 = reinterpret_cast<const float4*>(g);
    const float4* bt4 = reinterpret_cast<const float4*>(bt);
    float4 gg[2], bb[2];
#pragma unroll
    for (int i = 0; i < 2; ++i) {
        const int c4 = lane + 64 * i;
        gg[i] = g4[c4 < C4 ? c4 : 0];
        bb[i] = bt4[c4 < C4 ? c4 : 0];
    }
#pragma unroll
    for (int r = 0; r < R; ++r) {
        const int t = t0 + r * dil;
        const float s = (h[r][0].x + h[r][0].y) + (h[r][0].z + h[r][0].w) + (h[r][1].x + h[r][1].y) + (h[r][1].z + h[r][1].w);
        const float mean = wave_sum(s) / (float)C;
        float v = 0.f;
#pragma unroll
        for (int i = 0; i < 2; ++i)
            if (lane + 64 * i < C4) {
                const float dx = h[r][i].x - mean, dy = h[r][i].y - mean, dz = h[r][i].z - mean, dw = h[r][i].w - mean;
                v += (dx * dx + dy * dy) + (dz * dz + dw * dw);
            }
        const float rstd = rsqrtf(wave_sum(v) / (float)C + eps);
        if (t >= L) continue;
        if (t >= Lv) {
            if (row_off) continue;
#pragma unroll
            for (int i = 0; i < 2; ++i)
                if (lane + 64 * i < C4) store4(y + (row0 + t) * C + (lane + 64 * i) * 4, 0.f, 0.f, 0.f, 0.f);
            continue;
        }
#pragma unroll
        for (int i = 0; i < 2; ++i) {
            const int c4 = lane + 64 * i;
            if (c4 < C4)
                store4(y + (row0 + t) * C + c4 * 4, (h[r][i].x - mean) * rstd * gg[i].x + bb[i].x,
                       (h[r][i].y - mean) * rstd * gg[i].y + bb[i].y, (h[r][i].z - mean) * rstd * gg[i].z + bb[i].z,
                       (h[r][i].w - mean) * rstd * gg[i].w + bb[i].w);
        }
    }
}

template <typename OutT, int K, int R>
__global__ __launch_bounds__(256) void dwconv_ln_v3_kernel(const float* __restrict__ x, int nseq, int L, int C, const float* __restrict__ w_t,
                                                           const float* __restrict__ bias, int dil, int wps, const float* __restrict__ g, const float* __restrict__ bt,
                                                           float eps, OutT* __restrict__ y, const int* __restrict__ seqlen, const int* __restrict__ row_off, int xcd_runs) {
    dwconv_ln_v3_body<OutT, K, R>(x, nseq, L, C, w_t, bias, dil, wps, g, bt, eps, y, seqlen, row_off, xcd_runs);
}
template <typename OutT, int K, int R>
__global__ __launch_bounds__(256) __attribute__((amdgpu_waves_per_eu(4, 4))) void dwconv_ln_v3_occ4_kernel(
    const float* __restrict__ x, int nseq, int L, int C, const float* __restrict__ w_t, const float* __restrict__ bias, int dil, int wps,
    const float* __restrict__ g, const float* __restrict__ bt, float eps, OutT* __restrict__ y, const int* __restrict__ seqlen,
    const int* __restrict__ row_off, int xcd_runs) {
    dwconv_ln_v3_body<OutT, K, R>(x, nseq, L, C, w_t, bias, dil, wps, g, bt, eps, y, seqlen, row_off, xcd_runs);
}

template <typename OutT, int K, int R>
__global__ __launch_bounds__(256) void dwconv_ln_v3_tail_kernel(const float* __restrict__ x, int nseq, int L, int C, const float* __restrict__ w_t,
                                                                const float* __restrict__ bias, int dil, int wps, const float* __restrict__ g,
                                                                const float* __restrict__ bt, float eps, OutT* __restrict__ y,
                                                                const int* __restrict__ seqlen, const int* __restrict__ row_off, int xcd_runs,
                                                                const float* __restrict__ tail, int T, int rf) {
    dwconv_ln_v3_body<OutT, K, R, true>(x, nseq, L, C, w_t, bias, dil, wps, g, bt, eps, y, seqlen, row_off, xcd_runs, tail, T, rf);
}
template <typename OutT, int K, int R>
__global__ __launch_bounds__(256) __attribute__((amdgpu_waves_per_eu(4, 4))) void dwconv_ln_v3_tail_occ4_kernel(
    const float* __restrict__ x, int nseq, int L, int C, const float* __restrict__ w_t, const float* __restrict__ bias, int dil, int wps,
    const float* __restrict__ g, const float* __restrict__ bt, float eps, OutT* __restrict__ y, const int* __restrict__ seqlen,
    const int* __restrict__ row_off, int xcd_runs, const float* __restrict__ tail, int T, int rf) {
    dwconv_ln_v3_body<OutT, K, R, true>(x, nseq, L, C, w_t, bias, dil, wps, g, bt, eps, y, seqlen, row_off, xcd_runs, tail, T, rf);
}

template <typename OutT, int K, int R>
static void launch_dwconv_ln_v3_kr(hipStream_t s, bool occ4, const float* x, int nseq, int L, int C, const float* w_t, const float* bias,
                                   int dil, const float* g, const float* b, float eps, OutT* y, const int* seqlen, const int* row_off,
                                   const DwconvTail& tl) {
    const int wps = ((L + R * dil - 1) / (R * dil)) * dil;
    const int64_t nw = (int64_t)nseq * wps;
    static const int xcd_runs = [] { const char* e = stn::dev_env("STN_DWCONV_XCD"); return e ? atoi(e) : 1; }();
    if (tl.tail) {
        if constexpr (K == 7 && R == 4 && !std::is_same<OutT, f16_t>::value) {
            if (occ4) {
                STN_KLAUNCH((dwconv_ln_v3_tail_occ4_kernel<OutT, K, R>), dim3((unsigned)((nw + 3) / 4)), dim3(256), 0, s, x, nseq, L, C, w_t, bias,
                                   dil, wps, g, b, eps, y, seqlen, row_off, xcd_runs, tl.tail, tl.T, tl.rf);
                return;
            }
        }
        if (occ4) throw std::logic_error("dwconv_ln: no occ4 kernel for this form");
        STN_KLAUNCH((dwconv_ln_v3_tail_kernel<OutT, K, R>), dim3((unsigned)((nw + 3) / 4)), dim3(256), 0, s, x, nseq, L, C, w_t, bias,
                           dil, wps, g, b, eps, y, seqlen, row_off, xcd_runs, tl.tail, tl.T, tl.rf);
        return;
    }
    if constexpr (K == 7 && R == 4 && !std::is_same<OutT, f16_t>::value) {
        if (occ4) {
            STN_KLAUNCH((dwconv_ln_v3_occ4_kernel<OutT, K, R>), dim3((unsigned)((nw + 3) / 4)), dim3(256), 0, s, x, nseq, L, C, w_t, bias,
                               dil, wps, g, b, eps, y, seqlen, row_off, xcd_runs);
            return;
        }
    }
    if (occ4) throw std::logic_error("dwconv_ln: no occ4 kernel for this form");
    STN_KLAUNCH((dwconv_ln_v3_kernel<OutT, K, R>), dim3((unsigned)((nw + 3) / 4)), dim3(256), 0, s, x, nseq, L, C, w_t, bias,
                       dil, wps, g, b, eps, y, seqlen, row_off, xcd_runs);
}

void check_ln_shape(int C) {
    if (C % 4 || C > 4 * 64 * LN_NI) { char m_[256]; snprintf(m_, sizeof m_, "LayerNorm width %d unsupported (C %% 4 == 0, C <= 1024)", C); throw std::invalid_argument(m_); }
}

bool dwconv_ln_supports_packed(int C, int k) { return C <= 512 && C % 4 == 0 && (k == 5 || k == 7); }

std::string DwconvLnForm::str() const {
    if (kernel == DW_GENERIC) return "generic";
    char m_[32];
    if (kernel == DW_V2) snprintf(m_, sizeof m_, "v2<%d>", K);
    else snprintf(m_, sizeof m_, "%s<%d,%d>", occ4 ? "v3occ4" : "v3", K, R);
    return m_;
}

DwconvLnForm dwconv_ln_form(int out_dtype, int B, int L, int C, int k, bool packed) {
    check_ln_shape(C);
    if (packed && !dwconv_ln_supports_packed(C, k)) throw std::invalid_argument("packed dwconv_ln needs lengths, C <= 512, k in {5,7}");
    DwconvLnForm f;
    f.out_dtype = out_dtype == BF16 || out_dtype == F16 ? out_dtype : F32;
    f.K = k;
    if (C > 512 || (k != 5 && k != 7)) return f;
    const int64_t M = (int64_t)B * L;
    f.kernel = DW_V3;
    if (M >= 32768) {
        f.R = k == 5 ? 8 : 4;
    } else if (M >= 4096) {
        f.R = k == 5 ? (M < 16384 ? 2 : 4) : 4;
    } else if (packed) {
        f.R = k == 5 ? (M < 1024 ? 2 : 4) : 4;
    } else {
        f.kernel = DW_V2;
        f.R = 2;
    }
    f.occ4 = f.kernel == DW_V3 && f.K == 7 && f.R == 4 && f.out_dtype != F16;
    return f;
}

template <typename OutT>
static void launch_dwconv_ln_t(hipStream_t s, const DwconvLnForm& f, const float* x, int B, int L, int C, const float* w_t, const float* bias,
                               int k, int dil, const float* g, const float* b, float eps, OutT* y, const int* seqlen, const int* row_off,
                               const DwconvTail& tl) {
    const int64_t M = (int64_t)B * L;
    if (f.kernel == DW_V3) {
        if (f.K == 5 && f.R == 2) launch_dwconv_ln_v3_kr<OutT, 5, 2>(s, f.occ4, x, B, L, C, w_t, bias, dil, g, b, eps, y, seqlen, row_off, tl);
        else if (f.K == 5 && f.R == 4) launch_dwconv_ln_v3_kr<OutT, 5, 4>(s, f.occ4, x, B, L, C, w_t, bias, dil, g, b, eps, y, seqlen, row_off, tl);
        else if (f.K == 5 && f.R == 8) launch_dwconv_ln_v3_kr<OutT, 5, 8>(s, f.occ4, x, B, L, C, w_t, bias, dil, g, b, eps, y, seqlen, row_off, tl);
        else if (f.K == 7 && f.R == 4) launch_dwconv_ln_v3_kr<OutT, 7, 4>(s, f.occ4, x, B, L, C, w_t, bias, dil, g, b, eps, y, seqlen, row_off, tl);
        else throw std::logic_error("dwconv_ln: no v3 kernel for form " + f.str());
    } else if (f.kernel == DW_V2) {
        constexpr int R = 2;
        const dim3 grid((unsigned)((M + 4 * R - 1) / (4 * R)));
        if (f.K == 5) STN_KLAUNCH((dwconv_ln_v2_kernel<OutT, 5, R>), grid, dim3(256), 0, s, x, M, L, C, w_t, bias, dil, g, b, eps, y, seqlen);
        else if (f.K == 7) STN_KLAUNCH((dwconv_ln_v2_kernel<OutT, 7, R>), grid, dim3(256), 0, s, x, M, L, C, w_t, bias, dil, g, b, eps, y, seqlen);
        else throw std::logic_error("dwconv_ln: no v2 kernel for form " + f.str());
    } else {
        const dim3 grid((unsigned)((M + 3) / 4));
        STN_KLAUNCH((dwconv_ln_kernel<OutT, true>), grid, dim3(256), 0, s, x, M, L, C, w_t, bias, k, dil, g, b, eps, y, seqlen);
    }
}

void launch_dwconv_ln(hipStream_t s, int out_dtype, const float* x, int B, int L, int C, const float* w_t,
                      const float* bias, int k, int dil, const float* ln_g, const float* ln_b, float eps, void* y,
                      const int* seqlen, const int* row_off, const DwconvTail& tl) {
    check_ln_shape(C);
    if ((int64_t)B * L == 0) return;
    if (row_off && !seqlen) { throw std::invalid_argument("packed dwconv_ln needs lengths, C <= 512, k in {5,7}"); }
    if (tl.tail && (!row_off || tl.T < L || tl.rf < 0)) { throw std::invalid_argument("dwconv_ln: a tail table needs packed rows, T >= L and rf >= 0"); }
    const DwconvLnForm f = dwconv_ln_form(out_dtype, B, L, C, k, row_off != nullptr);
    with_out_type(f.out_dtype, [&](auto* tag) {
        using T = std::remove_pointer_t<decltype(tag)>;
        launch_dwconv_ln_t(s, f, x, B, L, C, w_t, bias, k, dil, ln_g, ln_b, eps, static_cast<T*>(y), seqlen, row_off, tl);
    });
}

void launch_layernorm(hipStream_t s, int out_dtype, const float* x, int64_t M, int C, const float* g, const float* b,
                      float eps, void* y) {
    check_ln_shape(C);
    if (M == 0) return;
    const dim3 grid((unsigned)((M + 3) / 4));
    with_out_type(out_dtype, [&](auto* tag) {
        using T = std::remove_pointer_t<decltype(tag)>;
        STN_KLAUNCH((dwconv_ln_kernel<T, false>), grid, dim3(256), 0, s, x, M, 1, C, nullptr, nullptr, 1, 1, g, b, eps, static_cast<T*>(y),
                    static_cast<const int*>(nullptr));
    });
}

}
```

Before: 48050.

## Make v3 dwconv+LN kernels grid-stride with LDS-staged weights and capped grid

```diff
diff --git a/include/stn.h b/include/stn.h
--- a/include/stn.h
+++ b/include/stn.h
@@ -309,6 +309,10 @@
 int stn_op_dwconv_ln_tail(stn_handle* h, int dtype, int B, int L, int C, int k, int dil, const float* x, int64_t x_rows,
                           const float* w , const float* bias, const float* ln_g, const float* ln_b, const int32_t* seqlen,
                           const float* tail , int T, int rf, float* y, int64_t y_rows, char* form, size_t form_cap);
+int stn_op_dwconv_ln_walk(stn_handle* h, int dtype, int B, int L, int C, int k, int dil, const float* x, int64_t x_rows,
+                          const float* w , const float* bias, const float* ln_g, const float* ln_b, const int32_t* seqlen_or_null,
+                          int packed, const float* tail_or_null , int T, int rf, int grid_cap, float* y, int64_t y_rows,
+                          char* form, size_t form_cap);
 int64_t stn_dbg_len_tables(int B, const int32_t* llen, int ve_rows, int with_pairs, int vo_form, int ccf, int T, int rf, int32_t* layout,
                            int32_t* out, int64_t out_n);
 int stn_dbg_dwconv_ln_form(int dtype, int B, int L, int C, int k, int packed, char* out, size_t cap);
diff --git a/supertonic_amd/binding.py b/supertonic_amd/binding.py
--- a/supertonic_amd/binding.py
+++ b/supertonic_amd/binding.py
@@ -543,6 +543,8 @@
     L.stn_op_dwconv_ln_ex.argtypes = [vp, ci, ci, ci, ci, ci, ci, _f32p, ctypes.c_int64, vp, vp, _f32p, _f32p, vp, ci, ci, _f32p, ctypes.c_int64,
                                       ctypes.c_char_p, ctypes.c_size_t]
     L.stn_op_dwconv_ln_tail.argtypes = [vp, ci, ci, ci, ci, ci, ci, _f32p, ctypes.c_int64, _f32p, _f32p, _f32p, _f32p, _i32p, _f32p, ci, ci, _f32p,
+                                        ctypes.c_int64, ctypes.c_char_p, ctypes.c_size_t]
+    L.stn_op_dwconv_ln_walk.argtypes = [vp, ci, ci, ci, ci, ci, ci, _f32p, ctypes.c_int64, _f32p, _f32p, _f32p, _f32p, vp, ci, vp, ci, ci, ci, _f32p,
                                         ctypes.c_int64, ctypes.c_char_p, ctypes.c_size_t]
     L.stn_dbg_resample_form.argtypes = [ci, ci, ctypes.c_int64, ctypes.c_char_p, ctypes.c_size_t]
     L.stn_dbg_resample_form.restype = ctypes.c_int
@@ -2233,6 +2235,21 @@
                                                  o_r.shape[0], form, ctypes.sizeof(form)))
         return o_r, form.value.decode()
 
+    def op_dwconv_ln_walk(self, x, w, bias, g, b, dil, out, B, L, grid_cap, seqlen=None, packed=False, tail=None, T=0, dtype=None):
+        x = _c(x, np.float32)
+        o_r = np.array(out, dtype=np.float32, order="C", copy=True)
+        C = x.shape[1]
+        w = _c(w, np.float32)
+        _l, lp = _opt(seqlen, np.int32)
+        _t, tp = _opt(None if tail is None else np.asarray(tail).reshape(-1), np.float32)
+        rf = 0 if tail is None else np.asarray(tail).shape[0] - 1
+        form = ctypes.create_string_buffer(32)
+        self._ck(self._lib.stn_op_dwconv_ln_walk(self._h, self.dtype if dtype is None else _DTYPES[dtype], int(B), int(L), C, w.shape[1], int(dil),
+                                                 x.reshape(-1), x.shape[0], w, _c(bias, np.float32), _c(g, np.float32), _c(b, np.float32), lp,
+                                                 int(bool(packed)), tp, int(T), int(rf), int(grid_cap), o_r.reshape(-1), o_r.shape[0], form,
+                                                 ctypes.sizeof(form)))
+        return o_r, form.value.decode()
+
     def op_fold_ln(self, x, part, b2, gamma, g, b, rowvec=None, row_b=None, dtype=None):
         x_r = np.array(x, dtype=np.float32, order="C", copy=True)
         M, C = x_r.shape
diff --git a/supertonic_amd/csrc/api.cpp b/supertonic_amd/csrc/api.cpp
--- a/supertonic_amd/csrc/api.cpp
+++ b/supertonic_amd/csrc/api.cpp
@@ -975,7 +975,7 @@
 }
 static void dwconv_ln_ex_checked(stn_handle* h, int dtype, int B, int L, int C, int k, int dil, const float* x, int64_t x_rows, const float* w,
                                  const float* bias, const float* g, const float* b, const int32_t* seqlen, int packed, int ln_only, float* y,
-                                 int64_t y_rows, char* form, size_t form_cap) {
+                                 int64_t y_rows, char* form, size_t form_cap, int grid_cap = 0) {
     need(B > 0 && L > 0 && C > 0 && C % 4 == 0 && C <= 1024 && k > 0 && (k & 1) && dil > 0 && x && g && b && y && x_rows > 0 && y_rows > 0,
          "stn_op_dwconv_ln_ex: bad argument");
     need(dtype == STN_DTYPE_F32 || dtype == STN_DTYPE_BF16 || dtype == STN_DTYPE_F16, "stn_op_dwconv_ln_ex: unknown dtype");
@@ -989,7 +989,7 @@
         if (packed) rows = tot;
     }
     need(x_rows >= rows && y_rows >= rows, "stn_op_dwconv_ln_ex: x / y hold fewer rows than the launch addresses");
-    const std::string f = h->eng->op_dwconv_ln_ex(dtype, B, L, C, k, dil, x, x_rows, w, bias, g, b, ln_only ? nullptr : seqlen, packed, ln_only, y, y_rows);
+    const std::string f = h->eng->op_dwconv_ln_ex(dtype, B, L, C, k, dil, x, x_rows, w, bias, g, b, ln_only ? nullptr : seqlen, packed, ln_only, y, y_rows, nullptr, 0, 0, grid_cap);
     if (form && form_cap) std::snprintf(form, form_cap, "%s", f.c_str());
 }
 int stn_op_dwconv_ln_ex(stn_handle* h, int dtype, int B, int L, int C, int k, int dil, const float* x, int64_t x_rows, const float* w,
@@ -999,7 +999,7 @@
 }
 static void dwconv_ln_tail_checked(stn_handle* h, int dtype, int B, int L, int C, int k, int dil, const float* x, int64_t x_rows, const float* w,
                                    const float* bias, const float* g, const float* b, const int32_t* seqlen, const float* tail, int T, int rf,
-                                   float* y, int64_t y_rows, char* form, size_t form_cap) {
+                                   float* y, int64_t y_rows, char* form, size_t form_cap, int grid_cap = 0) {
     need(B > 0 && B <= 1024 && L > 0 && C > 0 && C % 4 == 0 && C <= 512 && (k == 5 || k == 7) && dil > 0 && x && w && bias && g && b && y && seqlen &&
              x_rows > 0 && y_rows > 0,
          "stn_op_dwconv_ln_tail: bad argument");
@@ -1008,13 +1008,21 @@
     int64_t rows = 0;
     for (int i = 0; i < B; ++i) { need(seqlen[i] >= 0 && seqlen[i] <= L, "stn_op_dwconv_ln_tail: seqlen out of [0, L]"); rows += seqlen[i]; }
     need(x_rows >= rows && y_rows >= rows, "stn_op_dwconv_ln_tail: x / y hold fewer rows than the launch addresses");
-    const std::string f = h->eng->op_dwconv_ln_ex(dtype, B, L, C, k, dil, x, x_rows, w, bias, g, b, seqlen, 1, 0, y, y_rows, tail, T, rf);
+    const std::string f = h->eng->op_dwconv_ln_ex(dtype, B, L, C, k, dil, x, x_rows, w, bias, g, b, seqlen, 1, 0, y, y_rows, tail, T, rf, grid_cap);
     if (form && form_cap) std::snprintf(form, form_cap, "%s", f.c_str());
 }
 int stn_op_dwconv_ln_tail(stn_handle* h, int dtype, int B, int L, int C, int k, int dil, const float* x, int64_t x_rows, const float* w,
                           const float* bias, const float* g, const float* b, const int32_t* seqlen, const float* tail, int T, int rf, float* y,
                           int64_t y_rows, char* form, size_t form_cap) {
     STN_TRY(h, dwconv_ln_tail_checked(h, dtype, B, L, C, k, dil, x, x_rows, w, bias, g, b, seqlen, tail, T, rf, y, y_rows, form, form_cap))
+}
+int stn_op_dwconv_ln_walk(stn_handle* h, int dtype, int B, int L, int C, int k, int dil, const float* x, int64_t x_rows, const float* w,
+                          const float* bias, const float* g, const float* b, const int32_t* seqlen, int packed, const float* tail, int T, int rf,
+                          int grid_cap, float* y, int64_t y_rows, char* form, size_t form_cap) {
+    STN_TRY(h, { need(grid_cap >= 1, "stn_op_dwconv_ln_walk: grid_cap must be >= 1");
+                 need(!tail || packed, "stn_op_dwconv_ln_walk: a tail table needs packed rows");
+                 if (tail) dwconv_ln_tail_checked(h, dtype, B, L, C, k, dil, x, x_rows, w, bias, g, b, seqlen, tail, T, rf, y, y_rows, form, form_cap, grid_cap);
+                 else dwconv_ln_ex_checked(h, dtype, B, L, C, k, dil, x, x_rows, w, bias, g, b, seqlen, packed, 0, y, y_rows, form, form_cap, grid_cap); })
 }
 int64_t stn_dbg_len_tables(int B, const int32_t* llen, int ve_rows, int with_pairs, int vo_form, int ccf, int T, int rf, int32_t* layout,
                            int32_t* out, int64_t out_n) {
diff --git a/supertonic_amd/csrc/engine.hpp b/supertonic_amd/csrc/engine.hpp
--- a/supertonic_amd/csrc/engine.hpp
+++ b/supertonic_amd/csrc/engine.hpp
@@ -455,7 +455,7 @@
                       const float* g, const float* b, float* y, const int* seqlen = nullptr );
     std::string op_dwconv_ln_ex(int dtype, int B, int L, int C, int k, int dil, const float* x, int64_t x_rows, const float* w, const float* bias,
                                 const float* g, const float* b, const int* seqlen, int packed, int ln_only, float* y, int64_t y_rows,
-                                const float* tail = nullptr, int T = 0, int rf = 0);
+                                const float* tail = nullptr, int T = 0, int rf = 0, int grid_cap = 0);
     void op_fold_ln(int dtype, int M, int C, int S, const float* part, const float* b2, const float* gamma, const float* rowvec, const int* row_b,
                     int nseq, const float* g, const float* b, float* x, float* y);
     void op_layout(int which, int dtype, const int* p, const float* a, int64_t a_n, const float* b, int64_t b_n, const float* c, int64_t c_n,
diff --git a/supertonic_amd/csrc/engine_ops.cpp b/supertonic_amd/csrc/engine_ops.cpp
--- a/supertonic_amd/csrc/engine_ops.cpp
+++ b/supertonic_amd/csrc/engine_ops.cpp
@@ -558,7 +558,7 @@
 
 std::string Engine::op_dwconv_ln_ex(int dtype, int B, int L, int C, int k, int dil, const float* x, int64_t x_rows, const float* w,
                                     const float* bias, const float* g, const float* b, const int* seqlen, int packed, int ln_only, float* y,
-                                    int64_t y_rows, const float* tail, int T, int rf) {
+                                    int64_t y_rows, const float* tail, int T, int rf, int grid_cap) {
     STN_HIP(hipSetDevice(device_));
     ar_.reset();
     const int* dlen = seqlen ? up(ar_, s_, seqlen, (size_t)B) : nullptr;
@@ -582,7 +582,7 @@
         DwconvTail tl;
         if (tail) { tl.tail = up(ar_, s_, tail, (size_t)(rf + 1) * C); tl.T = T; tl.rf = rf; }
         form = dwconv_ln_form(dtype, B, L, C, k, packed != 0).str();
-        launch_dwconv_ln(s_, dtype, dx, B, L, C, dw, db, k, dil, dg, dbt, 1e-6f, dy, dlen, off, tl);
+        launch_dwconv_ln(s_, dtype, dx, B, L, C, dw, db, k, dil, dg, dbt, 1e-6f, dy, dlen, off, tl, grid_cap);
     }
     STN_HIP(hipGetLastError());
     down_as(ar_, s_, dtype, dy, y, (size_t)y_rows * C);
diff --git a/supertonic_amd/csrc/kernels.hpp b/supertonic_amd/csrc/kernels.hpp
--- a/supertonic_amd/csrc/kernels.hpp
+++ b/supertonic_amd/csrc/kernels.hpp
@@ -179,9 +179,10 @@
     const float* tail = nullptr;
     int T = 0, rf = 0;
 };
+constexpr int DWCONV_WALK_WGS = 4096;
 void launch_dwconv_ln(hipStream_t s, int out_dtype, const float* x, int B, int L, int C, const float* w_t,
                       const float* bias, int k, int dil, const float* ln_g, const float* ln_b, float eps, void* y,
-                      const int* seqlen = nullptr, const int* row_off = nullptr, const DwconvTail& tl = DwconvTail());
+                      const int* seqlen = nullptr, const int* row_off = nullptr, const DwconvTail& tl = DwconvTail(), int grid_cap = 0);
 enum DwconvLnKernel : int { DW_V3 = 0, DW_V2 = 1, DW_GENERIC = 2 };
 struct DwconvLnForm {
     int out_dtype = F32;
diff --git a/supertonic_amd/csrc/kernels_dwconv_ln.hip b/supertonic_amd/csrc/kernels_dwconv_ln.hip
--- a/supertonic_amd/csrc/kernels_dwconv_ln.hip
+++ b/supertonic_amd/csrc/kernels_dwconv_ln.hip
@@ -174,112 +174,143 @@
                                                            const int* __restrict__ seqlen, const int* __restrict__ row_off, int xcd_runs,
                                                            const float* __restrict__ tail = nullptr, int T = 0, int rf = 0) {
     const int lane = threadIdx.x & 63;
+    const int C4 = C >> 2;
+    constexpr int PV = 128;
+    __shared__ float4 prm[(K + 3) * PV];
     int bid = blockIdx.x;
     if (xcd_runs) {
         const int nb = gridDim.x, q = nb >> 3, rr = nb & 7, xcd = bid & 7, idx = bid >> 3;
         bid = xcd * q + (xcd < rr ? xcd : rr) + idx;
     }
-    const int64_t wid = (int64_t)bid * 4 + (threadIdx.x >> 6);
-    if (wid >= (int64_t)nseq * wps) return;
-    const int b = (int)(wid / wps), rem = (int)(wid % wps);
-    const int t0 = (rem / dil) * (R * dil) + (rem % dil);
-    const int Lv = seqlen ? seqlen[b] : L;
     constexpr int HALF = (K - 1) / 2, NWIN = R + K - 1;
-    const int C4 = C >> 2;
-    const int64_t row0 = row_off ? (int64_t)row_off[b] : (int64_t)b * L;
-    if (t0 >= Lv) {
-        if (row_off) return;
+    const int64_t nwid = (int64_t)nseq * wps, step = (int64_t)gridDim.x * 4;
+    const int wave = __builtin_amdgcn_readfirstlane((int)(threadIdx.x >> 6));
+    struct Comb { int t0, Lv; int64_t row0; };
+    auto comb_of = [&](int64_t wid) {
+        const int b = (int)(wid / wps), rem = (int)(wid % wps);
+        Comb c;
+        c.t0 = (rem / dil) * (R * dil) + (rem % dil);
+        c.Lv = seqlen ? seqlen[b] : L;
+        c.row0 = row_off ? (int64_t)row_off[b] : (int64_t)b * L;
+        return c;
+    };
+    int64_t wid = (int64_t)bid * 4 + wave;
+    float4 st[K + 3];
+    const bool stager = (int)threadIdx.x < C4;
+    {
+        const int sc = stager ? (int)threadIdx.x : 0;
+        const float4* w4 = reinterpret_cast<const float4*>(w_t);
+#pragma unroll
+        for (int j = 0; j < K; ++j) st[j] = w4[j * C4 + sc];
+        st[K] = reinterpret_cast<const float4*>(bias)[sc];
+        st[K + 1] = reinterpret_cast<const float4*>(g)[sc];
+        st[K + 2] = reinterpret_cast<const float4*>(bt)[sc];
+    }
+    Comb nx = comb_of(wid < nwid ? wid : 0);
+    if (stager) {
+#pragma unroll
+        for (int j = 0; j < K + 3; ++j) prm[j * PV + threadIdx.x] = st[j];
+    }
+    __syncthreads();
+    while (wid < nwid) {
+        const Comb cb = nx;
+        wid += step;
+        if (wid < nwid) nx = comb_of(wid);
+        asm volatile("" ::: "memory");
+        const int t0 = cb.t0, Lv = cb.Lv;
+        const int64_t row0 = cb.row0;
+        if (t0 >= Lv) {
+            if (row_off) continue;
+#pragma unroll
+            for (int r = 0; r < R; ++r) {
+                const int t = t0 + r * dil;
+                if (t >= L) break;
+#pragma unroll
+                for (int i = 0; i < 2; ++i)
+                    if (lane + 64 * i < C4) store4(y + (row0 + t) * C + (lane + 64 * i) * 4, 0.f, 0.f, 0.f, 0.f);
+            }
+            continue;
+        }
+        const float4* x4 = reinterpret_cast<const float4*>(x) + row0 * C4;
+        float4 h[R][2];
+#pragma unroll
+        for (int i = 0; i < 2; ++i) {
+            const int c4 = lane + 64 * i;
+            const bool act = c4 < C4;
+            const int cc = act ? c4 : 0;
+            float4 win[NWIN];
+#pragma unroll
+            for (int q = 0; q < NWIN; ++q) {
+                const int tt = t0 + (q - HALF) * dil;
+                const int hi_ = row_off ? Lv : L;
+                const int tc = tt < 0 ? 0 : (tt >= hi_ ? hi_ - 1 : tt);
+                if constexpr (TAIL) {
+                    const float4* src = x4 + (int64_t)tc * C4;
+                    bool keep = tt >= 0 && tt < Lv;
+                    if (tt >= Lv && tt < T) {
+                        const int j = T - 1 - tt;
+                        src = reinterpret_cast<const float4*>(tail) + (int64_t)(j < rf ? j : rf) * C4;
+                        keep = true;
+                    }
+                    const float4 v = src[cc];
+                    win[q] = keep ? v : make_float4(0.f, 0.f, 0.f, 0.f);
+                } else {
+                    const float4 v = x4[(int64_t)tc * C4 + cc];
+                    win[q] = (tt >= 0 && tt < Lv) ? v : make_float4(0.f, 0.f, 0.f, 0.f);
+                }
+            }
+            float4 a[R];
+            const float4 bv = prm[K * PV + cc];
+#pragma unroll
+            for (int r = 0; r < R; ++r) a[r] = bv;
+#pragma unroll
+            for (int j = 0; j < K; ++j) {
+                const float4 wv = prm[j * PV + cc];
+#pragma unroll
+                for (int r = 0; r < R; ++r) {
+                    a[r].x = fmaf(wv.x, win[r + j].x, a[r].x); a[r].y = fmaf(wv.y, win[r + j].y, a[r].y);
+                    a[r].z = fmaf(wv.z, win[r + j].z, a[r].z); a[r].w = fmaf(wv.w, win[r + j].w, a[r].w);
+                }
+            }
+#pragma unroll
+            for (int r = 0; r < R; ++r) h[r][i] = act ? a[r] : make_float4(0.f, 0.f, 0.f, 0.f);
+        }
+        float4 gg[2], bb[2];
+#pragma unroll
+        for (int i = 0; i < 2; ++i) {
+            const int c4 = lane + 64 * i;
+            gg[i] = prm[(K + 1) * PV + (c4 < C4 ? c4 : 0)];
+            bb[i] = prm[(K + 2) * PV + (c4 < C4 ? c4 : 0)];
+        }
 #pragma unroll
         for (int r = 0; r < R; ++r) {
             const int t = t0 + r * dil;
-            if (t >= L) break;
+            const float s = (h[r][0].x + h[r][0].y) + (h[r][0].z + h[r][0].w) + (h[r][1].x + h[r][1].y) + (h[r][1].z + h[r][1].w);
+            const float mean = wave_sum(s) / (float)C;
+            float v = 0.f;
 #pragma unroll
             for (int i = 0; i < 2; ++i)
-                if (lane + 64 * i < C4) store4(y + (row0 + t) * C + (lane + 64 * i) * 4, 0.f, 0.f, 0.f, 0.f);
-        }
-        return;
-    }
-    const float4* x4 = reinterpret_cast<const float4*>(x) + row0 * C4;
-    const float4* w4 = reinterpret_cast<const float4*>(w_t);
-    const float4* b4 = reinterpret_cast<const float4*>(bias);
-    float4 h[R][2];
-#pragma unroll
-    for (int i = 0; i < 2; ++i) {
-        const int c4 = lane + 64 * i;
-        const bool act = c4 < C4;
-        const int cc = act ? c4 : 0;
-        float4 win[NWIN], wv[K];
-#pragma unroll
-        for (int j = 0; j < K; ++j) wv[j] = w4[(int64_t)j * C4 + cc];
-#pragma unroll
-        for (int q = 0; q < NWIN; ++q) {
-            const int tt = t0 + (q - HALF) * dil;
-            const int hi_ = row_off ? Lv : L;
-            const int tc = tt < 0 ? 0 : (tt >= hi_ ? hi_ - 1 : tt);
-            if constexpr (TAIL) {
-                const float4* src = x4 + (int64_t)tc * C4;
-                bool keep = tt >= 0 && tt < Lv;
-                if (tt >= Lv && tt < T) {
-                    const int j = T - 1 - tt;
-                    src = reinterpret_cast<const float4*>(tail) + (int64_t)(j < rf ? j : rf) * C4;
-                    keep = true;
+                if (lane + 64 * i < C4) {
+                    const float dx = h[r][i].x - mean, dy = h[r][i].y - mean, dz = h[r][i].z - mean, dw = h[r][i].w - mean;
+                    v += (dx * dx + dy * dy) + (dz * dz + dw * dw);
                 }
-                const float4 v = src[cc];
-                win[q] = keep ? v : make_float4(0.f, 0.f, 0.f, 0.f);
-            } else {
-                const float4 v = x4[(int64_t)tc * C4 + cc];
-                win[q] = (tt >= 0 && tt < Lv) ? v : make_float4(0.f, 0.f, 0.f, 0.f);
-            }
-        }
-        const float4 bv = b4[cc];
-#pragma unroll
-        for (int r = 0; r < R; ++r) {
-            float4 a = bv;
-#pragma unroll
-            for (int j = 0; j < K; ++j) {
-                a.x = fmaf(wv[j].x, win[r + j].x, a.x); a.y = fmaf(wv[j].y, win[r + j].y, a.y);
-                a.z = fmaf(wv[j].z, win[r + j].z, a.z); a.w = fmaf(wv[j].w, win[r + j].w, a.w);
-            }
-            h[r][i] = act ? a : make_float4(0.f, 0.f, 0.f, 0.f);
-        }
-    }
-    const float4* g4 = reinterpret_cast<const float4*>(g);
-    const float4* bt4 = reinterpret_cast<const float4*>(bt);
-    float4 gg[2], bb[2];
-#pragma unroll
-    for (int i = 0; i < 2; ++i) {
-        const int c4 = lane + 64 * i;
-        gg[i] = g4[c4 < C4 ? c4 : 0];
-        bb[i] = bt4[c4 < C4 ? c4 : 0];
-    }
-#pragma unroll
-    for (int r = 0; r < R; ++r) {
-        const int t = t0 + r * dil;
-        const float s = (h[r][0].x + h[r][0].y) + (h[r][0].z + h[r][0].w) + (h[r][1].x + h[r][1].y) + (h[r][1].z + h[r][1].w);
-        const float mean = wave_sum(s) / (float)C;
-        float v = 0.f;
-#pragma unroll
-        for (int i = 0; i < 2; ++i)
-            if (lane + 64 * i < C4) {
-                const float dx = h[r][i].x - mean, dy = h[r][i].y - mean, dz = h[r][i].z - mean, dw = h[r][i].w - mean;
-                v += (dx * dx + dy * dy) + (dz * dz + dw * dw);
-            }
-        const float rstd = rsqrtf(wave_sum(v) / (float)C + eps);
-        if (t >= L) continue;
-        if (t >= Lv) {
-            if (row_off) continue;
-#pragma unroll
-            for (int i = 0; i < 2; ++i)
-                if (lane + 64 * i < C4) store4(y + (row0 + t) * C + (lane + 64 * i) * 4, 0.f, 0.f, 0.f, 0.f);
-            continue;
-        }
-#pragma unroll
-        for (int i = 0; i < 2; ++i) {
-            const int c4 = lane + 64 * i;
-            if (c4 < C4)
-                store4(y + (row0 + t) * C + c4 * 4, (h[r][i].x - mean) * rstd * gg[i].x + bb[i].x,
-                       (h[r][i].y - mean) * rstd * gg[i].y + bb[i].y, (h[r][i].z - mean) * rstd * gg[i].z + bb[i].z,
-                       (h[r][i].w - mean) * rstd * gg[i].w + bb[i].w);
+            const float rstd = rsqrtf(wave_sum(v) / (float)C + eps);
+            if (t >= L) continue;
+            if (t >= Lv) {
+                if (row_off) continue;
+#pragma unroll
+                for (int i = 0; i < 2; ++i)
+                    if (lane + 64 * i < C4) store4(y + (row0 + t) * C + (lane + 64 * i) * 4, 0.f, 0.f, 0.f, 0.f);
+                continue;
+            }
+#pragma unroll
+            for (int i = 0; i < 2; ++i) {
+                const int c4 = lane + 64 * i;
+                if (c4 < C4)
+                    store4(y + (row0 + t) * C + c4 * 4, (h[r][i].x - mean) * rstd * gg[i].x + bb[i].x,
+                           (h[r][i].y - mean) * rstd * gg[i].y + bb[i].y, (h[r][i].z - mean) * rstd * gg[i].z + bb[i].z,
+                           (h[r][i].w - mean) * rstd * gg[i].w + bb[i].w);
+            }
         }
     }
 }
@@ -317,32 +348,35 @@
 template <typename OutT, int K, int R>
 static void launch_dwconv_ln_v3_kr(hipStream_t s, bool occ4, const float* x, int nseq, int L, int C, const float* w_t, const float* bias,
                                    int dil, const float* g, const float* b, float eps, OutT* y, const int* seqlen, const int* row_off,
-                                   const DwconvTail& tl) {
+                                   const DwconvTail& tl, int grid_cap) {
     const int wps = ((L + R * dil - 1) / (R * dil)) * dil;
     const int64_t nw = (int64_t)nseq * wps;
     static const int xcd_runs = [] { const char* e = stn::dev_env("STN_DWCONV_XCD"); return e ? atoi(e) : 1; }();
+    static const int walk_wgs = [] { const char* e = stn::dev_env("STN_DWCONV_WGS"); const int v = e ? atoi(e) : 0; return v > 0 ? v : DWCONV_WALK_WGS; }();
+    const int64_t cap = grid_cap > 0 ? grid_cap : walk_wgs, need = (nw + 3) / 4;
+    const dim3 grid((unsigned)(need < cap ? need : cap));
     if (tl.tail) {
         if constexpr (K == 7 && R == 4 && !std::is_same<OutT, f16_t>::value) {
             if (occ4) {
-                STN_KLAUNCH((dwconv_ln_v3_tail_occ4_kernel<OutT, K, R>), dim3((unsigned)((nw + 3) / 4)), dim3(256), 0, s, x, nseq, L, C, w_t, bias,
+                STN_KLAUNCH((dwconv_ln_v3_tail_occ4_kernel<OutT, K, R>), grid, dim3(256), 0, s, x, nseq, L, C, w_t, bias,
                                    dil, wps, g, b, eps, y, seqlen, row_off, xcd_runs, tl.tail, tl.T, tl.rf);
                 return;
             }
         }
         if (occ4) throw std::logic_error("dwconv_ln: no occ4 kernel for this form");
-        STN_KLAUNCH((dwconv_ln_v3_tail_kernel<OutT, K, R>), dim3((unsigned)((nw + 3) / 4)), dim3(256), 0, s, x, nseq, L, C, w_t, bias,
+        STN_KLAUNCH((dwconv_ln_v3_tail_kernel<OutT, K, R>), grid, dim3(256), 0, s, x, nseq, L, C, w_t, bias,
                            dil, wps, g, b, eps, y, seqlen, row_off, xcd_runs, tl.tail, tl.T, tl.rf);
         return;
     }
     if constexpr (K == 7 && R == 4 && !std::is_same<OutT, f16_t>::value) {
         if (occ4) {
-            STN_KLAUNCH((dwconv_ln_v3_occ4_kernel<OutT, K, R>), dim3((unsigned)((nw + 3) / 4)), dim3(256), 0, s, x, nseq, L, C, w_t, bias,
+            STN_KLAUNCH((dwconv_ln_v3_occ4_kernel<OutT, K, R>), grid, dim3(256), 0, s, x, nseq, L, C, w_t, bias,
                                dil, wps, g, b, eps, y, seqlen, row_off, xcd_runs);
             return;
         }
     }
     if (occ4) throw std::logic_error("dwconv_ln: no occ4 kernel for this form");
-    STN_KLAUNCH((dwconv_ln_v3_kernel<OutT, K, R>), dim3((unsigned)((nw + 3) / 4)), dim3(256), 0, s, x, nseq, L, C, w_t, bias,
+    STN_KLAUNCH((dwconv_ln_v3_kernel<OutT, K, R>), grid, dim3(256), 0, s, x, nseq, L, C, w_t, bias,
                        dil, wps, g, b, eps, y, seqlen, row_off, xcd_runs);
 }
 
@@ -386,13 +420,13 @@
 template <typename OutT>
 static void launch_dwconv_ln_t(hipStream_t s, const DwconvLnForm& f, const float* x, int B, int L, int C, const float* w_t, const float* bias,
                                int k, int dil, const float* g, const float* b, float eps, OutT* y, const int* seqlen, const int* row_off,
-                               const DwconvTail& tl) {
+                               const DwconvTail& tl, int grid_cap) {
     const int64_t M = (int64_t)B * L;
     if (f.kernel == DW_V3) {
-        if (f.K == 5 && f.R == 2) launch_dwconv_ln_v3_kr<OutT, 5, 2>(s, f.occ4, x, B, L, C, w_t, bias, dil, g, b, eps, y, seqlen, row_off, tl);
-        else if (f.K == 5 && f.R == 4) launch_dwconv_ln_v3_kr<OutT, 5, 4>(s, f.occ4, x, B, L, C, w_t, bias, dil, g, b, eps, y, seqlen, row_off, tl);
-        else if (f.K == 5 && f.R == 8) launch_dwconv_ln_v3_kr<OutT, 5, 8>(s, f.occ4, x, B, L, C, w_t, bias, dil, g, b, eps, y, seqlen, row_off, tl);
-        else if (f.K == 7 && f.R == 4) launch_dwconv_ln_v3_kr<OutT, 7, 4>(s, f.occ4, x, B, L, C, w_t, bias, dil, g, b, eps, y, seqlen, row_off, tl);
+        if (f.K == 5 && f.R == 2) launch_dwconv_ln_v3_kr<OutT, 5, 2>(s, f.occ4, x, B, L, C, w_t, bias, dil, g, b, eps, y, seqlen, row_off, tl, grid_cap);
+        else if (f.K == 5 && f.R == 4) launch_dwconv_ln_v3_kr<OutT, 5, 4>(s, f.occ4, x, B, L, C, w_t, bias, dil, g, b, eps, y, seqlen, row_off, tl, grid_cap);
+        else if (f.K == 5 && f.R == 8) launch_dwconv_ln_v3_kr<OutT, 5, 8>(s, f.occ4, x, B, L, C, w_t, bias, dil, g, b, eps, y, seqlen, row_off, tl, grid_cap);
+        else if (f.K == 7 && f.R == 4) launch_dwconv_ln_v3_kr<OutT, 7, 4>(s, f.occ4, x, B, L, C, w_t, bias, dil, g, b, eps, y, seqlen, row_off, tl, grid_cap);
         else throw std::logic_error("dwconv_ln: no v3 kernel for form " + f.str());
     } else if (f.kernel == DW_V2) {
         constexpr int R = 2;
@@ -408,7 +442,7 @@
 
 void launch_dwconv_ln(hipStream_t s, int out_dtype, const float* x, int B, int L, int C, const float* w_t,
                       const float* bias, int k, int dil, const float* ln_g, const float* ln_b, float eps, void* y,
-                      const int* seqlen, const int* row_off, const DwconvTail& tl) {
+                      const int* seqlen, const int* row_off, const DwconvTail& tl, int grid_cap) {
     check_ln_shape(C);
     if ((int64_t)B * L == 0) return;
     if (row_off && !seqlen) { throw std::invalid_argument("packed dwconv_ln needs lengths, C <= 512, k in {5,7}"); }
@@ -416,7 +450,7 @@
     const DwconvLnForm f = dwconv_ln_form(out_dtype, B, L, C, k, row_off != nullptr);
     with_out_type(f.out_dtype, [&](auto* tag) {
         using T = std::remove_pointer_t<decltype(tag)>;
-        launch_dwconv_ln_t(s, f, x, B, L, C, w_t, bias, k, dil, ln_g, ln_b, eps, static_cast<T*>(y), seqlen, row_off, tl);
+        launch_dwconv_ln_t(s, f, x, B, L, C, w_t, bias, k, dil, ln_g, ln_b, eps, static_cast<T*>(y), seqlen, row_off, tl, grid_cap);
     });
 }
 
```

Measured after the change: 48310 (median of 6 runs). Within noise of the previous version (+0.5%).
